# AssemblyAI-Community/MinImagen

Hardware: AMD Instinct MI355X
Metric: denoising-steps/sec (images/sec x T), base 64^2 + SR 64->256 cascade (higher is better)
Workload: dtype f32; 1 GPU; cascade64_256: unet_0 params @64x64 + unet_1 params (lowres_cond) @256x256, T=100/stage, cond_scale=3.0 (2 U-Net evals/step), dynamic thresholding 0.9, fp32 storage / accumulate / softmax / statistics, contractions as 3-term fp16-split (hi*hi + hi*lo + lo*hi) MFMA products; per_gpu_batch=32, global_batch=32, parallelism=dp1

## Files before the change

### include/minimagen_hip.h

```cpp
#ifndef MINIMAGEN_HIP_H
#define MINIMAGEN_HIP_H

#include <stdint.h>

#ifdef __cplusplus
extern "C" {
#endif

#define MI_ABI_VERSION 12

enum mi_status {
    MI_OK = 0,
    MI_ERR_INVALID = -1,
    MI_ERR_LAUNCH = -2,
    MI_ERR_UNSUPPORTED = -3
};

int mi_abi_version(void);
const char* mi_last_error(void);
const char* mi_backend(void);
int mi_struct_size(int which);

typedef struct mi_act {
    const float* data;
    int C;
    const double* stats;
    int nt;
    float scale;
    int bmod;
    int st;
} mi_act;

typedef struct mi_conv_params {
    int B, H, W;
    mi_act in0, in1;
    int Cout;
    int ksize, stride, up2;
    const float* w;
    const float* bias;
    int gn_groups;
    const float* gn_gamma;
    const float* gn_beta;
    float gn_eps;
    const float* scale_shift;
    int ss_stride, ss_off;
    mi_act res0, res1;
    const float* res_w;
    const float* res_b;
    float* out;
    int out_st;
    double* out_stats;
    int tile_cfg;
    const void* w_rp;
    const void* res_w_rp;
    int w_rp_exp, res_w_rp_exp;
    float* gn_coef;
    int* gn_exps;
    void* act_prep; long long act_prep_bytes;
} mi_conv_params;
#define MI_CONV_SPLIT16 0x100
#define MI_CONV_SPLIT8  0x800
#define MI_CONV_HALF    0x400
#define MI_CONV_REVERSE 0x200
#define MI_CONV_RP_FIRST 6

int mi_conv_tile_shape(int tile_cfg, int* th, int* tw);
int mi_conv_stripe_rows(const mi_conv_params* p);
int mi_conv_prep_fwd(const mi_conv_params* p, void* stream);
long long mi_conv_prep_bytes(int B, int Cin, int Cres, int H, int W);
int mi_conv_cout_tile(int Cout);
int mi_conv_fwd(const mi_conv_params* p, void* stream);
int mi_gn_coef_fwd(const mi_conv_params* p, void* stream);

typedef struct mi_crossembed_params {
    int B, H, W;
    const float* in0; int C0;
    const float* in1; int C1;
    int in1_batch_mod;
    int in0_batch_mod;
    int n_kernels;
    int ksize[3];
    int cout[3];
    const float* w[3];
    const float* bias[3];
    float* out; double* out_stats;
    int out_st;
    int tile_cfg;
    const float* addend;
    const void* w_mfma;
    int w_mfma_exp[3];
} mi_crossembed_params;
int mi_crossembed_fwd(const mi_crossembed_params* p, void* stream);

typedef struct mi_init_down_params {
    int B, H, W;
    const float* in0; int C0;
    const float* in1; int C1;
    int in0_batch_mod;
    int n_kernels;
    int ksize[3];
    int cout[3];
    int Cout;
    const void* w_tab;
    int w_exp;
    const float* bias9;
    float* out; double* out_stats;
    int out_st;
    int tile_cfg;
    const float* addend;
} mi_init_down_params;
int mi_init_down_tiles(int tile_cfg, int H, int W);
int mi_init_down_fwd(const mi_init_down_params* p, void* stream);

typedef struct mi_linear {
    const float* w; const float* b; int in, out;
} mi_linear;

typedef struct mi_text_cond_params {
    int B2, B, L, E, cd, tcd, max_len;
    const float* text_embeds;
    const uint8_t* text_mask;
    const uint8_t* keep;
    mi_linear text_to_cond;
    const float* null_text_embed;
    const float* ln_w; const float* ln_b;
    mi_linear h1, h2;
    const float* null_text_hidden;
    const float* norm_w; const float* norm_b;
    float* c_text;
    float* text_hiddens;
} mi_text_cond_params;
int mi_text_cond_fwd(const mi_text_cond_params* p, void* stream);

typedef struct mi_cond_step_params {
    int B2, B, dim, cd, tcd, ntok;
    const int64_t* time;
    const int64_t* lowres_time;
    const float* freq;
    mi_linear th, tc, tt;
    mi_linear lth, ltc, ltt;
    const float* text_hiddens;
    const float* norm_w; const float* norm_b;
    mi_linear time_mlps;
    float* ss;
    float* c_time;
    float* t_out;
    float* silu_out;
} mi_cond_step_params;
int mi_cond_step_fwd(const mi_cond_step_params* p, void* stream);

#define MI_ATTN_MAX_BLOCKS 8
typedef struct mi_attn_fold_params {
    int B2, C, cd, heads, JT;
    const float* c_rows;
    int c_stride_b;
    int row0, nrows;
    int write_null;
    int frag_f16;
    int n_blocks;
    struct {
        const float* mg;
        const float* mv;
        const float* g0;
        const float* v0;
        float* gv;
        float* table;
        int g_exp, v_exp;
    } blk[MI_ATTN_MAX_BLOCKS];
    int mode;
    const int* t_state;
    int t_off;
    const float* ss_all; float* ss; int ss_n;
} mi_attn_fold_params;
int mi_attn_fold_rows(const mi_attn_fold_params* p, void* stream);
int mi_attn_fragment_floats(int C);

typedef struct mi_cross_attn_params {
    int B2, C, HW, heads, J;
    mi_act x;
    const float* gv;
    const float* n1_g; const float* n1_b;
    const float* n2_g; const float* n2_b;
    float* out; double* out_stats;
    int out_st;
    int x_exp, g_exp, v_exp;
    int variant;
} mi_cross_attn_params;
int mi_cross_attn_fwd(const mi_cross_attn_params* p, void* stream);
#define MI_ATTN_TOKENS_PER_WG 128

typedef struct mi_cfg_x0_params {
    int B, n;
    const float* pred2;
    int two;
    float cond_scale;
    const float* x_t;
    const float* coef; const int* t_state;
    float* pred_out;
    float* x0;
    unsigned* hist0;
    int t_off;
} mi_cfg_x0_params;
int mi_cfg_x0_fwd(const mi_cfg_x0_params* p, void* stream);

#define MI_Q_BINS 2048
typedef struct mi_quantile_params {
    int B, n;
    const float* x0;
    int k_lo, k_hi; float w;
    unsigned* hist;
    float* s_out;
    float* v_out;
    int pass0_done;
    int self_cleaning;
} mi_quantile_params;
int mi_quantile_fwd(const mi_quantile_params* p, void* stream);

typedef struct mi_posterior_params {
    int B, n, T;
    const float* x0; const float* s_q;
    float* x;
    const float* coef; const int* t_state;
    const float* noise;
    uint64_t seed; int sample0; int stream_base;
    const uint64_t* seed_dev;
    int t_off;
} mi_posterior_params;
int mi_posterior_fwd(const mi_posterior_params* p, void* stream);

#define MI_SAMPLER_SMALL_N 16384
int mi_sampler_step_small_fwd(const mi_cfg_x0_params* c, const mi_quantile_params* q, const mi_posterior_params* pp, void* stream);

int mi_sampler_group_size(int n);
long long mi_sampler_group_sync_bytes(int B, int n);
int mi_sampler_step_group_fwd(const mi_cfg_x0_params* c, const mi_quantile_params* q, const mi_posterior_params* pp, void* sync, void* stream);

int mi_step_advance(int* t_state, int64_t* times, int B, void* stream);
int mi_step_advance_by(int* t_state, int64_t* times, int B, int n, void* stream);
int mi_step_set(int* t_state, int64_t* times, int B, int value, void* stream);

typedef struct mi_sampler_ext_params {
    const int* t_map;
    float* x0_prev;
    long long reserved[2];
} mi_sampler_ext_params;
int mi_posterior_ext_fwd(const mi_posterior_params* p, const mi_sampler_ext_params* e, void* stream);
int mi_sampler_step_small_ext_fwd(const mi_cfg_x0_params* c, const mi_quantile_params* q, const mi_posterior_params* pp, const mi_sampler_ext_params* e, void* stream);
int mi_sampler_step_group_ext_fwd(const mi_cfg_x0_params* c, const mi_quantile_params* q, const mi_posterior_params* pp, const mi_sampler_ext_params* e, void* sync,
                                  void* stream);
int mi_step_set_mapped(int* t_state, int64_t* times, int B, int value, const mi_sampler_ext_params* e, void* stream);
int mi_step_advance_mapped(int* t_state, int64_t* times, int B, const mi_sampler_ext_params* e, void* stream);
int mi_step_advance_by_mapped(int* t_state, int64_t* times, int B, int n, const mi_sampler_ext_params* e, void* stream);

typedef struct mi_inpaint_params {
    const float* known;
    const unsigned char* mask;
    int hw;
    int known_stream;
    const float* known_noise;
    long long reserved[2];
} mi_inpaint_params;
int mi_posterior_inpaint_fwd(const mi_posterior_params* p, const mi_sampler_ext_params* e, const mi_inpaint_params* ip, void* stream);
int mi_sampler_step_small_inpaint_fwd(const mi_cfg_x0_params* c, const mi_quantile_params* q, const mi_posterior_params* pp, const mi_sampler_ext_params* e,
                                      const mi_inpaint_params* ip, void* stream);
int mi_sampler_step_group_inpaint_fwd(const mi_cfg_x0_params* c, const mi_quantile_params* q, const mi_posterior_params* pp, const mi_sampler_ext_params* e,
                                      const mi_inpaint_params* ip, void* sync, void* stream);
int mi_inpaint_blend0_fwd(float* x, int B, int n, const mi_inpaint_params* ip, float a, float b, uint64_t seed, int sample0, void* stream);
int mi_inpaint_prepare_fwd(const float* img, float* known, int B, int n, int normalize, const unsigned char* mask_in, int Hin, int Win, unsigned char* mask_out,
                           int size, void* stream);

int mi_randn_fill(float* out, int B, int n, uint64_t seed, int sample0, int stream_id, void* stream);

int mi_finalize_images(const float* x, float* out, int64_t total, int unnormalize, void* stream);

typedef struct mi_resize_params {
    int planes, Hin, Win, Hout, Wout, KH, KW;
    const float* in; float* out;
    const int* idx_h; const float* w_h;
    const int* idx_w; const float* w_w;
} mi_resize_params;
int mi_resize_fwd(const mi_resize_params* p, void* stream);

int mi_lowres_augment(const float* img, const float* noise, float* out, int64_t total, float a, float b, int normalize, void* stream);

int mi_ln_tokens_fwd(const mi_act* x, int B, int HW, const float* gamma, const float* beta, float* out, void* stream);
typedef struct mi_self_attn_params {
    int B2, C, HW, heads, J;
    mi_act x;
    const float* gv;
    const float* n1_g; const float* n1_b;
    const float* n2_g; const float* n2_b;
    float* out; double* out_stats;
} mi_self_attn_params;
int mi_self_attn_fwd(const mi_self_attn_params* p, void* stream);
typedef struct mi_chan_ff_params {
    int B, C, Chid, HW;
    mi_act x;
    const float* g1; const float* w1;
    const float* g2; const float* w2;
    float* out; double* out_stats;
} mi_chan_ff_params;
int mi_chan_ff_fwd(const mi_chan_ff_params* p, void* stream);

typedef struct mi_flash_attn_params {
    int B, HW, heads, kv_heads;
    const float* q; float q_scale;
    const float* null_k; const float* null_v;
    const float* k0; const float* v0; int n0, ld0; long long bs0;
    const float* k1; const float* v1; int n1, ld1; long long bs1;
    float* out;
    void* kv_prep; long long kv_prep_bytes;
} mi_flash_attn_params;
int mi_flash_attn_fwd(const mi_flash_attn_params* p, void* stream);
long long mi_flash_kv_prep_bytes(int B, int J);
typedef struct mi_tokens_to_nchw_params {
    int B, HW, C;
    const float* tokens;
    const float* gamma; const float* beta; float eps;
    mi_act res;
    float* out; double* out_stats;
} mi_tokens_to_nchw_params;
int mi_tokens_to_nchw_fwd(const mi_tokens_to_nchw_params* p, void* stream);
int mi_ln_rows_fwd(const float* x, const float* gamma, const float* beta, float* y, int rows, int dim, float eps, void* stream);

int mi_gemm_f32(const float* A, const float* W, const float* gate, const float* R, float* Cout, int M, int N, int K, int act, void* stream);
int mi_gemm_rms_f32(const float* A, const float* W, const float* gate, const float* R, float* Cout, int M, int N, int K, int act,
                    const float* rowsq_in, int nparts, float eps, float* rowsq_out, void* stream);
int mi_rmsnorm(const float* x, const float* w, float* y, int rows, int dim, float eps, const uint8_t* zero_mask, void* stream);
int mi_embed_rows(const int64_t* ids, const float* table, float* out, int rows, int dim, void* stream);
int mi_embed_rows_sq(const int64_t* ids, const float* table, float* out, float* rowsq, int nparts, int rows, int dim, void* stream);
int mi_t5_attention(const float* qkv, const float* bias_tab, const uint8_t* key_mask, float* ctx, int B, int L, int heads, void* stream);

typedef struct mi_conv_wgrad_params {
    int B, Cin, Cout, H, W;
    const float* a;
    const float* dy;
    float* dw;
    float* db;
    float* partial; int nwg;
    const double* a_stats; int a_nt;
    const float* gamma; const float* beta; int groups; float eps;
    const float* ss; int ss_stride, ss_off;
} mi_conv_wgrad_params;
long long mi_conv_wgrad_workspace(int Cin, int Cout, int nwg);
int mi_conv_wgrad(const mi_conv_wgrad_params* p, void* stream);

typedef struct mi_block_bwd_params {
    int B, C, HW, groups, nt, nchunk;
    float eps;
    const float* x; const float* da;
    const double* x_stats;
    const float* gamma; const float* beta;
    const float* ss; int ss_stride, ss_off;
    float* uv;
    float* dx;
    float* dgamma; float* dbeta;
    float* dss;
    double* dx_stats;
} mi_block_bwd_params;
int mi_block_bwd(const mi_block_bwd_params* p, void* stream);
int mi_chan_stats_fwd(const float* x, double* stats, int rows, int HW, void* stream);
int mi_layernorm_fwd(const float* x, const float* gamma, const float* beta, float* y, float* stat, int rows, int dim, float eps, void* stream);
int mi_layernorm_bwd_nwg(int rows, int dim);
int mi_layernorm_bwd(const float* dy, const float* x, const float* gamma, const float* stat, float* dx, float* partial, float* dgamma, float* dbeta,
                     int rows, int dim, void* stream);
long long mi_pack_conv3_floats(int Cout, int Cin, int adjoint, int cout_pad, int which);
int mi_pack_conv3(const float* w, int Cout, int Cin, int adjoint, int exp, void* frag, float* generic, int cout_pad, void* stream);
typedef struct mi_pack_conv3_desc {
    const float* w; void* frag; float* generic;
    int Cout, Cin, adjoint, exp, cout_pad, reserved;
} mi_pack_conv3_desc;
int mi_pack_conv3_multi(const mi_pack_conv3_desc* descs, int n, int blocks, void* stream);

typedef struct mi_crossembed_wgrad_params {
    int B, Cin, H, W;
    const float* x;
    const float* dy;
    int n_kernels; int ksize[3]; int cout[3];
    float* dw[3];
    float* db[3];
    float* partial; int nwg;
} mi_crossembed_wgrad_params;
long long mi_crossembed_wgrad_workspace(int Cin, int kmax, int nwg);
int mi_crossembed_wgrad(const mi_crossembed_wgrad_params* p, void* stream);

typedef struct mi_folded_attn_params {
    int B, n, H, J, C, nchunk;
    const float* q;
    const float* kf; const float* vf;
    const uint8_t* mask;
    float* out;
    float* lse;
    const float* dout;
    float* dsum;
    float* dq;
    float* dkf; float* dvf;
    float* oh;
} mi_folded_attn_params;
int mi_folded_attn_fwd(const mi_folded_attn_params* p, void* stream);
int mi_folded_attn_bwd(const mi_folded_attn_params* p, void* stream);

typedef struct mi_flash_attn_train_params {
    int B, n, heads, kv_heads, J;
    const float* q; float q_scale;
    const float* k; const float* v;
    const uint8_t* mask;
    float* out;
    float* lse;
    const float* dout;
    float* dq;
    float* dk; float* dv;
    void* work; long long work_bytes;
} mi_flash_attn_train_params;
int mi_flash_attn_train_fwd(const mi_flash_attn_train_params* p, void* stream);
int mi_flash_attn_train_bwd(const mi_flash_attn_train_params* p, void* stream);
long long mi_flash_attn_train_workspace(int B, int n, int heads, int kv_heads, int J, int backward);

typedef struct { float* p; const float* g; float* m; float* v; long long n; } mi_adam_tensor;
typedef struct {
    const mi_adam_tensor* tensors;
    const int* chunk_tensor; const int* chunk_off;
    int nchunks, chunk;
    float lr, beta1, beta2, eps, weight_decay, bias_correction1, bias_correction2;
    float one_minus_beta1, one_minus_beta2;
    const float* grad_scale;
} mi_adam_params;
int mi_adam_step(const mi_adam_params* p, void* stream);

int mi_graph_begin(void* stream);
int mi_graph_end(void* stream, void** graph_exec);
int mi_graph_launch(void* graph_exec, void* stream);
int mi_graph_destroy(void* graph_exec);

#ifdef __cplusplus
}
#endif
#endif
```

### minimagen_amd/_lib.py

```python
from __future__ import annotations

import ctypes as C
import os

import torch

_HERE = os.path.dirname(os.path.abspath(__file__))
DEFAULT_LIB = os.environ.get("MINIMAGEN_HIP_LIB") or os.path.join(_HERE, "libminimagen_hip.so")

c_float_p = C.c_void_p


class MiAct(C.Structure):
    _fields_ = [("data", C.c_void_p), ("C", C.c_int), ("stats", C.c_void_p), ("nt", C.c_int), ("scale", C.c_float), ("bmod", C.c_int),
                ("st", C.c_int)]


class MiConvParams(C.Structure):
    _fields_ = [
        ("B", C.c_int), ("H", C.c_int), ("W", C.c_int),
        ("in0", MiAct), ("in1", MiAct),
        ("Cout", C.c_int), ("ksize", C.c_int), ("stride", C.c_int), ("up2", C.c_int),
        ("w", C.c_void_p), ("bias", C.c_void_p),
        ("gn_groups", C.c_int), ("gn_gamma", C.c_void_p), ("gn_beta", C.c_void_p), ("gn_eps", C.c_float),
        ("scale_shift", C.c_void_p), ("ss_stride", C.c_int), ("ss_off", C.c_int),
        ("res0", MiAct), ("res1", MiAct), ("res_w", C.c_void_p), ("res_b", C.c_void_p),
        ("out", C.c_void_p), ("out_st", C.c_int), ("out_stats", C.c_void_p), ("tile_cfg", C.c_int),
        ("w_rp", C.c_void_p), ("res_w_rp", C.c_void_p), ("w_rp_exp", C.c_int), ("res_w_rp_exp", C.c_int),
        ("gn_coef", C.c_void_p), ("gn_exps", C.c_void_p),
        ("act_prep", C.c_void_p), ("act_prep_bytes", C.c_longlong),
    ]


class MiCrossEmbedParams(C.Structure):
    _fields_ = [
        ("B", C.c_int), ("H", C.c_int), ("W", C.c_int),
        ("in0", C.c_void_p), ("C0", C.c_int), ("in1", C.c_void_p), ("C1", C.c_int),
        ("in1_batch_mod", C.c_int), ("in0_batch_mod", C.c_int), ("n_kernels", C.c_int),
        ("ksize", C.c_int * 3), ("cout", C.c_int * 3), ("w", C.c_void_p * 3), ("bias", C.c_void_p * 3),
        ("out", C.c_void_p), ("out_stats", C.c_void_p), ("out_st", C.c_int), ("tile_cfg", C.c_int), ("addend", C.c_void_p),
        ("w_mfma", C.c_void_p), ("w_mfma_exp", C.c_int * 3),
    ]


class MiInitDownParams(C.Structure):
    _fields_ = [
        ("B", C.c_int), ("H", C.c_int), ("W", C.c_int),
        ("in0", C.c_void_p), ("C0", C.c_int), ("in1", C.c_void_p), ("C1", C.c_int),
        ("in0_batch_mod", C.c_int), ("n_kernels", C.c_int), ("ksize", C.c_int * 3), ("cout", C.c_int * 3), ("Cout", C.c_int),
        ("w_tab", C.c_void_p), ("w_exp", C.c_int), ("bias9", C.c_void_p),
        ("out", C.c_void_p), ("out_stats", C.c_void_p), ("out_st", C.c_int), ("tile_cfg", C.c_int), ("addend", C.c_void_p),
    ]


class MiLinear(C.Structure):
    _fields_ = [("w", C.c_void_p), ("b", C.c_void_p), ("in_", C.c_int), ("out", C.c_int)]


class MiTextCondParams(C.Structure):
    _fields_ = [
        ("B2", C.c_int), ("B", C.c_int), ("L", C.c_int), ("E", C.c_int), ("cd", C.c_int), ("tcd", C.c_int), ("max_len", C.c_int),
        ("text_embeds", C.c_void_p), ("text_mask", C.c_void_p), ("keep", C.c_void_p),
        ("text_to_cond", MiLinear), ("null_text_embed", C.c_void_p), ("ln_w", C.c_void_p), ("ln_b", C.c_void_p),
        ("h1", MiLinear), ("h2", MiLinear), ("null_text_hidden", C.c_void_p), ("norm_w", C.c_void_p), ("norm_b", C.c_void_p),
        ("c_text", C.c_void_p), ("text_hiddens", C.c_void_p),
    ]


class MiCondStepParams(C.Structure):
    _fields_ = [
        ("B2", C.c_int), ("B", C.c_int), ("dim", C.c_int), ("cd", C.c_int), ("tcd", C.c_int), ("ntok", C.c_int),
        ("time", C.c_void_p), ("lowres_time", C.c_void_p), ("freq", C.c_void_p),
        ("th", MiLinear), ("tc", MiLinear), ("tt", MiLinear), ("lth", MiLinear), ("ltc", MiLinear), ("ltt", MiLinear),
        ("text_hiddens", C.c_void_p), ("norm_w", C.c_void_p), ("norm_b", C.c_void_p), ("time_mlps", MiLinear),
        ("ss", C.c_void_p), ("c_time", C.c_void_p), ("t_out", C.c_void_p), ("silu_out", C.c_void_p),
    ]


class MiAttnFoldBlk(C.Structure):
    _fields_ = [("mg", C.c_void_p), ("mv", C.c_void_p), ("g0", C.c_void_p), ("v0", C.c_void_p), ("gv", C.c_void_p), ("table", C.c_void_p),
                ("g_exp", C.c_int), ("v_exp", C.c_int)]


class MiAttnFoldParams(C.Structure):
    _fields_ = [
        ("B2", C.c_int), ("C", C.c_int), ("cd", C.c_int), ("heads", C.c_int), ("JT", C.c_int),
        ("c_rows", C.c_void_p), ("c_stride_b", C.c_int), ("row0", C.c_int), ("nrows", C.c_int), ("write_null", C.c_int), ("frag_f16", C.c_int),
        ("n_blocks", C.c_int), ("blk", MiAttnFoldBlk * 8),
        ("mode", C.c_int), ("t_state", C.c_void_p), ("t_off", C.c_int), ("ss_all", C.c_void_p), ("ss", C.c_void_p), ("ss_n", C.c_int),
    ]


class MiCrossAttnParams(C.Structure):
    _fields_ = [
        ("B2", C.c_int), ("C", C.c_int), ("HW", C.c_int), ("heads", C.c_int), ("J", C.c_int),
        ("x", MiAct), ("gv", C.c_void_p), ("n1_g", C.c_void_p), ("n1_b", C.c_void_p), ("n2_g", C.c_void_p), ("n2_b", C.c_void_p),
        ("out", C.c_void_p), ("out_stats", C.c_void_p), ("out_st", C.c_int), ("x_exp", C.c_int), ("g_exp", C.c_int), ("v_exp", C.c_int), ("variant", C.c_int),
    ]


class MiSelfAttnParams(C.Structure):
    _fields_ = [("B2", C.c_int), ("C", C.c_int), ("HW", C.c_int), ("heads", C.c_int), ("J", C.c_int), ("x", MiAct), ("gv", C.c_void_p),
                ("n1_g", C.c_void_p), ("n1_b", C.c_void_p), ("n2_g", C.c_void_p), ("n2_b", C.c_void_p), ("out", C.c_void_p), ("out_stats", C.c_void_p)]


class MiChanFFParams(C.Structure):
    _fields_ = [("B", C.c_int), ("C", C.c_int), ("Chid", C.c_int), ("HW", C.c_int), ("x", MiAct), ("g1", C.c_void_p), ("w1", C.c_void_p),
                ("g2", C.c_void_p), ("w2", C.c_void_p), ("out", C.c_void_p), ("out_stats", C.c_void_p)]


class MiFlashAttnParams(C.Structure):
    _fields_ = [("B", C.c_int), ("HW", C.c_int), ("heads", C.c_int), ("kv_heads", C.c_int), ("q", C.c_void_p), ("q_scale", C.c_float),
                ("null_k", C.c_void_p), ("null_v", C.c_void_p),
                ("k0", C.c_void_p), ("v0", C.c_void_p), ("n0", C.c_int), ("ld0", C.c_int), ("bs0", C.c_longlong),
                ("k1", C.c_void_p), ("v1", C.c_void_p), ("n1", C.c_int), ("ld1", C.c_int), ("bs1", C.c_longlong), ("out", C.c_void_p),
                ("kv_prep", C.c_void_p), ("kv_prep_bytes", C.c_longlong)]


class MiTokensToNchwParams(C.Structure):
    _fields_ = [("B", C.c_int), ("HW", C.c_int), ("C", C.c_int), ("tokens", C.c_void_p), ("gamma", C.c_void_p), ("beta", C.c_void_p),
                ("eps", C.c_float), ("res", MiAct), ("out", C.c_void_p), ("out_stats", C.c_void_p)]


class MiCfgX0Params(C.Structure):
    _fields_ = [("B", C.c_int), ("n", C.c_int), ("pred2", C.c_void_p), ("two", C.c_int), ("cond_scale", C.c_float),
                ("x_t", C.c_void_p), ("coef", C.c_void_p), ("t_state", C.c_void_p), ("pred_out", C.c_void_p), ("x0", C.c_void_p),
                ("hist0", C.c_void_p), ("t_off", C.c_int)]


class MiQuantileParams(C.Structure):
    _fields_ = [("B", C.c_int), ("n", C.c_int), ("x0", C.c_void_p), ("k_lo", C.c_int), ("k_hi", C.c_int), ("w", C.c_float),
                ("hist", C.c_void_p), ("s_out", C.c_void_p), ("v_out", C.c_void_p), ("pass0_done", C.c_int), ("self_cleaning", C.c_int)]


class MiPosteriorParams(C.Structure):
    _fields_ = [("B", C.c_int), ("n", C.c_int), ("T", C.c_int), ("x0", C.c_void_p), ("s_q", C.c_void_p), ("x", C.c_void_p),
                ("coef", C.c_void_p), ("t_state", C.c_void_p), ("noise", C.c_void_p),
                ("seed", C.c_uint64), ("sample0", C.c_int), ("stream_base", C.c_int), ("seed_dev", C.c_void_p), ("t_off", C.c_int)]


class MiSamplerExtParams(C.Structure):
    _fields_ = [("t_map", C.c_void_p), ("x0_prev", C.c_void_p), ("reserved", C.c_longlong * 2)]


class MiInpaintParams(C.Structure):
    _fields_ = [("known", C.c_void_p), ("mask", C.c_void_p), ("hw", C.c_int), ("known_stream", C.c_int), ("known_noise", C.c_void_p),
                ("reserved", C.c_longlong * 2)]


class MiResizeParams(C.Structure):
    _fields_ = [("planes", C.c_int), ("Hin", C.c_int), ("Win", C.c_int), ("Hout", C.c_int), ("Wout", C.c_int), ("KH", C.c_int), ("KW", C.c_int),
                ("in_", C.c_void_p), ("out", C.c_void_p), ("idx_h", C.c_void_p), ("w_h", C.c_void_p), ("idx_w", C.c_void_p), ("w_w", C.c_void_p)]


class MiConvWgradParams(C.Structure):
    _fields_ = [("B", C.c_int), ("Cin", C.c_int), ("Cout", C.c_int), ("H", C.c_int), ("W", C.c_int), ("a", C.c_void_p), ("dy", C.c_void_p),
                ("dw", C.c_void_p), ("db", C.c_void_p), ("partial", C.c_void_p), ("nwg", C.c_int),
                ("a_stats", C.c_void_p), ("a_nt", C.c_int), ("gamma", C.c_void_p), ("beta", C.c_void_p), ("groups", C.c_int), ("eps", C.c_float),
                ("ss", C.c_void_p), ("ss_stride", C.c_int), ("ss_off", C.c_int)]


class MiBlockBwdParams(C.Structure):
    _fields_ = [("B", C.c_int), ("C", C.c_int), ("HW", C.c_int), ("groups", C.c_int), ("nt", C.c_int), ("nchunk", C.c_int), ("eps", C.c_float),
                ("x", C.c_void_p), ("da", C.c_void_p), ("x_stats", C.c_void_p), ("gamma", C.c_void_p), ("beta", C.c_void_p),
                ("ss", C.c_void_p), ("ss_stride", C.c_int), ("ss_off", C.c_int), ("uv", C.c_void_p), ("dx", C.c_void_p),
                ("dgamma", C.c_void_p), ("dbeta", C.c_void_p), ("dss", C.c_void_p), ("dx_stats", C.c_void_p)]


class MiCrossEmbedWgradParams(C.Structure):
    _fields_ = [("B", C.c_int), ("Cin", C.c_int), ("H", C.c_int), ("W", C.c_int), ("x", C.c_void_p), ("dy", C.c_void_p),
                ("n_kernels", C.c_int), ("ksize", C.c_int * 3), ("cout", C.c_int * 3), ("dw", C.c_void_p * 3), ("db", C.c_void_p * 3),
                ("partial", C.c_void_p), ("nwg", C.c_int)]


class MiFoldedAttnParams(C.Structure):
    _fields_ = [("B", C.c_int), ("n", C.c_int), ("H", C.c_int), ("J", C.c_int), ("C", C.c_int), ("nchunk", C.c_int), ("q", C.c_void_p),
                ("kf", C.c_void_p), ("vf", C.c_void_p), ("mask", C.c_void_p), ("out", C.c_void_p), ("lse", C.c_void_p), ("dout", C.c_void_p),
                ("dsum", C.c_void_p), ("dq", C.c_void_p), ("dkf", C.c_void_p), ("dvf", C.c_void_p), ("oh", C.c_void_p)]


class MiFlashAttnTrainParams(C.Structure):
    _fields_ = [("B", C.c_int), ("n", C.c_int), ("heads", C.c_int), ("kv_heads", C.c_int), ("J", C.c_int), ("q", C.c_void_p), ("q_scale", C.c_float),
                ("k", C.c_void_p), ("v", C.c_void_p), ("mask", C.c_void_p), ("out", C.c_void_p), ("lse", C.c_void_p), ("dout", C.c_void_p),
                ("dq", C.c_void_p), ("dk", C.c_void_p), ("dv", C.c_void_p), ("work", C.c_void_p), ("work_bytes", C.c_longlong)]


class MiAdamTensor(C.Structure):
    _fields_ = [("p", C.c_void_p), ("g", C.c_void_p), ("m", C.c_void_p), ("v", C.c_void_p), ("n", C.c_longlong)]


class MiAdamParams(C.Structure):
    _fields_ = [("tensors", C.c_void_p), ("chunk_tensor", C.c_void_p), ("chunk_off", C.c_void_p), ("nchunks", C.c_int), ("chunk", C.c_int),
                ("lr", C.c_float), ("beta1", C.c_float), ("beta2", C.c_float), ("eps", C.c_float), ("weight_decay", C.c_float),
                ("bias_correction1", C.c_float), ("bias_correction2", C.c_float), ("one_minus_beta1", C.c_float), ("one_minus_beta2", C.c_float),
                ("grad_scale", C.c_void_p)]


class MiPackConv3Desc(C.Structure):
    _fields_ = [("w", C.c_void_p), ("frag", C.c_void_p), ("generic", C.c_void_p), ("Cout", C.c_int), ("Cin", C.c_int), ("adjoint", C.c_int),
                ("exp", C.c_int), ("cout_pad", C.c_int), ("reserved", C.c_int)]


_STRUCTS = {0: MiAct, 1: MiConvParams, 2: MiCrossEmbedParams, 3: MiLinear, 4: MiTextCondParams, 5: MiCondStepParams,
            6: MiAttnFoldParams, 7: MiCrossAttnParams, 8: MiCfgX0Params, 9: MiQuantileParams, 10: MiPosteriorParams,
            11: MiResizeParams, 12: MiSelfAttnParams, 13: MiChanFFParams, 14: MiFlashAttnParams, 15: MiTokensToNchwParams, 16: MiConvWgradParams, 17: MiBlockBwdParams, 18: MiCrossEmbedWgradParams, 19: MiFoldedAttnParams, 20: MiAdamTensor, 21: MiAdamParams, 22: MiPackConv3Desc,
            23: MiFlashAttnTrainParams, 24: MiSamplerExtParams, 25: MiInpaintParams, 26: MiInitDownParams}

_lib = None
_backend = None


class MinImagenHipError(RuntimeError):
    pass


def _bind(lib):
    lib.mi_abi_version.restype = C.c_int
    lib.mi_last_error.restype = C.c_char_p
    lib.mi_backend.restype = C.c_char_p
    lib.mi_struct_size.argtypes = [C.c_int]
    vp, i32, i64, u64, f32 = C.c_void_p, C.c_int, C.c_int64, C.c_uint64, C.c_float
    for name in ("mi_conv_fwd", "mi_gn_coef_fwd", "mi_crossembed_fwd", "mi_text_cond_fwd", "mi_cond_step_fwd", "mi_attn_fold_rows", "mi_cross_attn_fwd",
                 "mi_cfg_x0_fwd", "mi_quantile_fwd", "mi_posterior_fwd", "mi_resize_fwd", "mi_self_attn_fwd", "mi_chan_ff_fwd",
                 "mi_flash_attn_fwd", "mi_conv_prep_fwd", "mi_tokens_to_nchw_fwd", "mi_conv_wgrad", "mi_block_bwd", "mi_crossembed_wgrad", "mi_folded_attn_fwd", "mi_folded_attn_bwd", "mi_adam_step",
                 "mi_flash_attn_train_fwd", "mi_flash_attn_train_bwd", "mi_init_down_fwd"):
        getattr(lib, name).argtypes = [vp, vp]
        getattr(lib, name).restype = i32
    lib.mi_conv_prep_bytes.argtypes = [i32, i32, i32, i32, i32]
    lib.mi_conv_prep_bytes.restype = C.c_longlong
    lib.mi_flash_kv_prep_bytes.argtypes = [i32, i32]
    lib.mi_flash_kv_prep_bytes.restype = C.c_longlong
    lib.mi_flash_attn_train_workspace.argtypes = [i32, i32, i32, i32, i32, i32]
    lib.mi_flash_attn_train_workspace.restype = C.c_longlong
    lib.mi_step_advance.argtypes = [vp, vp, i32, vp]
    lib.mi_step_advance_by.argtypes = [vp, vp, i32, i32, vp]
    lib.mi_sampler_step_small_fwd.argtypes = [vp, vp, vp, vp]
    lib.mi_sampler_step_small_fwd.restype = i32
    lib.mi_sampler_step_group_fwd.argtypes = [vp, vp, vp, vp, vp]
    lib.mi_sampler_step_group_fwd.restype = i32
    lib.mi_sampler_group_size.argtypes = [i32]
    lib.mi_sampler_group_sync_bytes.argtypes = [i32, i32]
    lib.mi_sampler_group_sync_bytes.restype = C.c_longlong
    lib.mi_step_set.argtypes = [vp, vp, i32, i32, vp]
    lib.mi_posterior_ext_fwd.argtypes = [vp, vp, vp]
    lib.mi_sampler_step_small_ext_fwd.argtypes = [vp, vp, vp, vp, vp]
    lib.mi_sampler_step_group_ext_fwd.argtypes = [vp, vp, vp, vp, vp, vp]
    lib.mi_step_set_mapped.argtypes = [vp, vp, i32, i32, vp, vp]
    lib.mi_step_advance_mapped.argtypes = [vp, vp, i32, vp, vp]
    lib.mi_step_advance_by_mapped.argtypes = [vp, vp, i32, i32, vp, vp]
    lib.mi_posterior_inpaint_fwd.argtypes = [vp, vp, vp, vp]
    lib.mi_sampler_step_small_inpaint_fwd.argtypes = [vp, vp, vp, vp, vp, vp]
    lib.mi_sampler_step_group_inpaint_fwd.argtypes = [vp, vp, vp, vp, vp, vp, vp]
    lib.mi_inpaint_blend0_fwd.argtypes = [vp, i32, i32, vp, f32, f32, u64, i32, vp]
    lib.mi_inpaint_prepare_fwd.argtypes = [vp, vp, i32, i32, i32, vp, i32, i32, vp, i32, vp]
    lib.mi_randn_fill.argtypes = [vp, i32, i32, u64, i32, i32, vp]
    lib.mi_finalize_images.argtypes = [vp, vp, i64, i32, vp]
    lib.mi_lowres_augment.argtypes = [vp, vp, vp, i64, f32, f32, i32, vp]
    lib.mi_gemm_f32.argtypes = [vp, vp, vp, vp, vp, i32, i32, i32, i32, vp]
    lib.mi_rmsnorm.argtypes = [vp, vp, vp, i32, i32, f32, vp, vp]
    lib.mi_embed_rows.argtypes = [vp, vp, vp, i32, i32, vp]
    lib.mi_embed_rows_sq.argtypes = [vp, vp, vp, vp, i32, i32, i32, vp]
    lib.mi_gemm_rms_f32.argtypes = [vp, vp, vp, vp, vp, i32, i32, i32, i32, vp, i32, f32, vp, vp]
    lib.mi_t5_attention.argtypes = [vp, vp, vp, vp, i32, i32, i32, vp]
    lib.mi_ln_tokens_fwd.argtypes = [vp, i32, i32, vp, vp, vp, vp]
    lib.mi_ln_rows_fwd.argtypes = [vp, vp, vp, vp, i32, i32, f32, vp]
    lib.mi_graph_begin.argtypes = [vp]
    lib.mi_graph_end.argtypes = [vp, C.POINTER(vp)]
    lib.mi_graph_launch.argtypes = [vp, vp]
    lib.mi_graph_destroy.argtypes = [vp]
    lib.mi_conv_tile_shape.argtypes = [i32, C.POINTER(i32), C.POINTER(i32)]
    lib.mi_conv_stripe_rows.argtypes = [vp]
    lib.mi_conv_stripe_rows.restype = i32
    lib.mi_conv_cout_tile.argtypes = [i32]
    lib.mi_init_down_tiles.argtypes = [i32, i32, i32]
    lib.mi_init_down_tiles.restype = i32
    lib.mi_conv_wgrad_workspace.argtypes = [i32, i32, i32]
    lib.mi_conv_wgrad_workspace.restype = C.c_longlong
    lib.mi_crossembed_wgrad_workspace.argtypes = [i32, i32, i32]
    lib.mi_crossembed_wgrad_workspace.restype = C.c_longlong
    lib.mi_chan_stats_fwd.argtypes = [vp, vp, i32, i32, vp]
    lib.mi_layernorm_fwd.argtypes = [vp, vp, vp, vp, vp, i32, i32, C.c_float, vp]
    lib.mi_layernorm_bwd_nwg.argtypes = [i32, i32]
    lib.mi_layernorm_bwd_nwg.restype = i32
    lib.mi_layernorm_bwd.argtypes = [vp, vp, vp, vp, vp, vp, vp, vp, i32, i32, vp]
    lib.mi_pack_conv3_floats.argtypes = [i32, i32, i32, i32, i32]
    lib.mi_pack_conv3_floats.restype = C.c_longlong
    lib.mi_pack_conv3.argtypes = [vp, i32, i32, i32, i32, vp, vp, i32, vp]
    lib.mi_pack_conv3_multi.argtypes = [vp, i32, i32, vp]
    lib.mi_attn_fragment_floats.argtypes = [i32]
    for which, st in _STRUCTS.items():
        n = lib.mi_struct_size(which)
        if n != C.sizeof(st):
            raise MinImagenHipError(f"ABI mismatch: struct {st.__name__} is {n} bytes in the library, {C.sizeof(st)} in the binding")
    return lib


def use_library(path: str):
    global _lib, _backend
    if not os.path.exists(path):
        raise MinImagenHipError(f"{path} not found -- build it first (python -c 'import __graft_entry__ as g; g.build()')")
    _lib = _bind(C.CDLL(path))
    _backend = _lib.mi_backend().decode()
    return _lib


def lib():
    global _lib
    if _lib is None:
        use_library(DEFAULT_LIB)
    return _lib


def backend() -> str:
    lib()
    return _backend


def require_device(*tensors):
    be = backend()
    for t in tensors:
        if t is None:
            continue
        if t.dtype not in (torch.float32, torch.int64, torch.int32, torch.uint8, torch.bool, torch.float64):
            raise MinImagenHipError(f"unsupported dtype {t.dtype}")
        if not t.is_contiguous():
            raise MinImagenHipError("tensor must be contiguous")
        if be == "hip-gfx950" and not t.is_cuda:
            raise MinImagenHipError("minimagen_amd has no CPU path: tensor is not on the GPU")
        if be == "hipemu" and t.is_cuda:
            raise MinImagenHipError("emulator build needs host tensors")


def ptr(t) -> int:
    return 0 if t is None else t.data_ptr()


_RAW_STREAM = getattr(torch._C, "_cuda_getCurrentRawStream", None)


def current_stream() -> int:
    if backend() == "hip-gfx950":
        if _RAW_STREAM is not None:
            return _RAW_STREAM(torch.cuda.current_device())
        return torch.cuda.current_stream().cuda_stream
    return 0


def check(rc: int, what: str = ""):
    if rc != 0:
        raise MinImagenHipError(f"{what} failed ({rc}): {lib().mi_last_error().decode()}")
```

### minimagen_amd/csrc/attention.hip

```cpp
#include "common.hip.h"

namespace {

typedef _Float16 f16x4 __attribute__((ext_vector_type(4)));
typedef _Float16 f16x8 __attribute__((ext_vector_type(8)));
#ifndef ATTN_QPF
#define ATTN_QPF 1
#endif
#ifndef ATTN_QK32
#define ATTN_QK32 2
#endif

__device__ __forceinline__ void split_f16(const float (&x)[4], f16x4& hi, f16x4& lo) { mi_split_f16(x, hi, lo); }

template <int C, int JT, int WPS, bool HALF, int NWV>
__global__ __launch_bounds__(64 * NWV, WPS) void cross_attn_f16x3_kernel(const mi_cross_attn_params p) {
    constexpr int KC = (C + 15) / 16, MT = (C + 15) / 16, FRH = 8 * KC + 8 * MT, TOK_WG = 16 * NWV;
    constexpr int JP = (JT + 1) / 2;
    __shared__ double red[NWV][2 * 16 * MT];
    constexpr int QC = KC + MT, JTS = (JT + 1) & ~1, ROWS = JTS * QC;
    __shared__ __attribute__((aligned(16))) uint4 frag[2][ROWS * 64];
    const int tid = threadIdx.x, wave = tid >> 6, lane = tid & 63, lq = lane & 15, lg = lane >> 4;
    const int tiles = (p.HW + TOK_WG - 1) / TOK_WG;
    int b, tile;
    if ((p.B2 & 7) == 0) {
        const int L = blockIdx.x, k = L >> 3;
        b = (L & 7) + 8 * (k / tiles);
        tile = k % tiles;
    } else {
        b = blockIdx.x / tiles;
        tile = blockIdx.x % tiles;
    }
    const int bx = mi_row_of(b, p.x.bmod);
    const int i = (tile * NWV + wave) * 16 + lq;
    const bool ok = i < p.HW;
    const float* xb = p.x.data + (size_t)bx * C * p.HW;
    const bool x16 = HALF && p.x.st != 0, o16 = HALF && p.out_st != 0;
    auto ldx = [&](int a) -> float {
        if (x16) return mi_bf16_to_f32(reinterpret_cast<const unsigned short*>(p.x.data)[((size_t)bx * C + a) * p.HW + i]);
        return xb[(size_t)a * p.HW + i];
    };

    f16x4 xhi[KC], xlo[KC];
    {
        float xf[KC][4];
        float s = 0.0f;
#pragma unroll
        for (int kc = 0; kc < KC; ++kc)
#pragma unroll
            for (int e = 0; e < 4; ++e) {
                const int a = 16 * kc + 4 * lg + e;
                xf[kc][e] = (ok && a < C) ? ldx(a) * p.x.scale : 0.0f;
                s += xf[kc][e];
            }
        s += __shfl_xor(s, 16); s += __shfl_xor(s, 32);
        const float mean = s / (float)C;
        float v = 0.0f;
#pragma unroll
        for (int kc = 0; kc < KC; ++kc)
#pragma unroll
            for (int e = 0; e < 4; ++e) { const float d = (16 * kc + 4 * lg + e < C) ? xf[kc][e] - mean : 0.0f; v = fmaf(d, d, v); }
        v += __shfl_xor(v, 16); v += __shfl_xor(v, 32);
        const float rstd = 1.0f / sqrtf(v / (float)C + 1e-5f);
#pragma unroll
        for (int kc = 0; kc < KC; ++kc) {
            float xn[4];
#pragma unroll
            for (int e = 0; e < 4; ++e) {
                const int a = 16 * kc + 4 * lg + e;
                xn[e] = (a < C) ? ldexpf((xf[kc][e] - mean) * rstd * p.n1_g[a] + p.n1_b[a], p.x_exp) : 0.0f;
            }
            split_f16(xn, xhi[kc], xlo[kc]);
        }
    }
    f32x4 oacc[MT];
#pragma unroll
    for (int mt = 0; mt < MT; ++mt) oacc[mt] = (f32x4){0.f, 0.f, 0.f, 0.f};
    const _Float16* gvb = reinterpret_cast<const _Float16*>(p.gv) + (size_t)b * p.heads * JTS * 64 * FRH;
    const int jlast = p.J - 1;
    auto issue_head = [&](int h, int buf) {
        const _Float16* gvh = gvb + (size_t)h * JTS * 64 * FRH;
        for (int r = wave; r < ROWS; r += NWV) {
            const int jt = r / QC, q = r % QC;
            const _Float16* src = gvh + ((size_t)(jt * 64 + lane) * QC + q) * 8;
#if defined(HIPEMU)
            frag[buf][r * 64 + lane] = *reinterpret_cast<const uint4*>(src);
#else
            __builtin_amdgcn_global_load_lds((const __attribute__((address_space(1))) void*)src,
                                             (__attribute__((address_space(3))) void*)&frag[buf][r * 64], 16, 0, 0);
#endif
        }
    };
    issue_head(0, 0);

    for (int h = 0; h < p.heads; ++h) {
        const int hb = h & 1;
#if !defined(HIPEMU)
        asm volatile("s_waitcnt vmcnt(0)" ::: "memory");
#endif
        __syncthreads();
        if (h + 1 < p.heads) issue_head(h + 1, hb ^ 1);
        f32x4 s[JT];
        uint4 gq[2];
        constexpr bool QPF = !HALF && KC == 1 && ATTN_QPF;
        if constexpr (QPF) gq[0] = frag[hb][lane];
#pragma unroll
        for (int jt = 0; jt < JT; ++jt) {
            f32x4 acc = (f32x4){0.f, 0.f, 0.f, 0.f};
            if constexpr (QPF) {
                if (jt + 1 < JT) gq[(jt + 1) & 1] = frag[hb][((jt + 1) * QC) * 64 + lane];
                __builtin_amdgcn_sched_barrier(0);
            }
#pragma unroll
            for (int kc = 0; kc < KC; ++kc) {
                union { uint4 u; f16x4 h2[2]; uint2 u2; } g;
                if constexpr (HALF) g.u2 = reinterpret_cast<const uint2*>(&frag[hb][0])[2 * ((jt * QC + kc) * 64 + lane)];
                else if constexpr (QPF) g.u = gq[jt & 1];
                else g.u = frag[hb][(jt * QC + kc) * 64 + lane];
                const f16x4 ghi = g.h2[0];
                if constexpr (!HALF) {
#if ATTN_QK32 == 2
                    const f16x4 z4 = {(_Float16)0, (_Float16)0, (_Float16)0, (_Float16)0};
                    const f16x8 xhh = __builtin_shufflevector(xhi[kc], xhi[kc], 0, 1, 2, 3, 4, 5, 6, 7);
                    const f16x8 xl0 = __builtin_shufflevector(xlo[kc], z4, 0, 1, 2, 3, 4, 5, 6, 7);
                    acc = __builtin_amdgcn_mfma_f32_16x16x32_f16(__builtin_bit_cast(f16x8, g.u), xl0, acc, 0, 0, 0);
                    acc = __builtin_amdgcn_mfma_f32_16x16x32_f16(__builtin_bit_cast(f16x8, g.u), xhh, acc, 0, 0, 0);
#elif ATTN_QK32
                    const f16x8 xhh = __builtin_shufflevector(xhi[kc], xhi[kc], 0, 1, 2, 3, 4, 5, 6, 7);
                    acc = __builtin_amdgcn_mfma_f32_16x16x16f16(ghi, xlo[kc], acc, 0, 0, 0);
                    acc = __builtin_amdgcn_mfma_f32_16x16x32_f16(__builtin_bit_cast(f16x8, g.u), xhh, acc, 0, 0, 0);
#else
                    acc = __builtin_amdgcn_mfma_f32_16x16x16f16(g.h2[1], xhi[kc], acc, 0, 0, 0);
                    acc = __builtin_amdgcn_mfma_f32_16x16x16f16(ghi, xlo[kc], acc, 0, 0, 0);
                    acc = __builtin_amdgcn_mfma_f32_16x16x16f16(ghi, xhi[kc], acc, 0, 0, 0);
#endif
                } else {
                    acc = __builtin_amdgcn_mfma_f32_16x16x16f16(ghi, xhi[kc], acc, 0, 0, 0);
                }
            }
            s[jt] = acc;
            if constexpr (HALF) { if ((jt & 3) == 3) __builtin_amdgcn_sched_barrier(0); }
        }
        float m = -INFINITY;
#pragma unroll
        for (int jt = 0; jt < JT; ++jt)
#pragma unroll
            for (int r = 0; r < 4; ++r) {
                if (jt == JT - 1 && (16 * jt + 4 * lg + r) > jlast) s[jt][r] = -INFINITY;
                m = fmaxf(m, s[jt][r]);
            }
        m = fmaxf(m, __shfl_xor(m, 16));
        m = fmaxf(m, __shfl_xor(m, 32));
        const float sc = ldexpf(1.0f, -(p.x_exp + p.g_exp)), msc = -m * sc;
        mi_f32x2 l2 = {0.0f, 0.0f};
        const mi_f32x2 sc2 = {sc, sc}, msc2 = {msc, msc};
        f32x4 oh[MT];
#pragma unroll
        for (int mt = 0; mt < MT; ++mt) oh[mt] = (f32x4){0.f, 0.f, 0.f, 0.f};
#pragma unroll
        for (int jp = 0; jp < JP; ++jp) {
            f16x4 ph[2], pl[2];
#pragma unroll
            for (int ts = 0; ts < 2; ++ts) {
                const int jt = 2 * jp + ts;
                float pe[4] = {0.f, 0.f, 0.f, 0.f};
                if (jt < JT) {
                    const f32x4 sv = s[jt < JT ? jt : 0];
                    const mi_f32x2 a01 = mi_pk_fma((mi_f32x2){sv[0], sv[1]}, sc2, msc2), a23 = mi_pk_fma((mi_f32x2){sv[2], sv[3]}, sc2, msc2);
                    pe[0] = __builtin_amdgcn_exp2f(a01[0]); pe[1] = __builtin_amdgcn_exp2f(a01[1]);
                    pe[2] = __builtin_amdgcn_exp2f(a23[0]); pe[3] = __builtin_amdgcn_exp2f(a23[1]);
                    l2 = mi_pk_add(l2, (mi_f32x2){pe[0], pe[1]});
                    l2 = mi_pk_add(l2, (mi_f32x2){pe[2], pe[3]});
                }
                if constexpr (HALF) {
#pragma unroll
                    for (int r = 0; r < 4; ++r) ph[ts][r] = (_Float16)pe[r];
                } else {
                    split_f16(pe, ph[ts], pl[ts]);
                }
            }
            const f16x8 phi = __builtin_shufflevector(ph[0], ph[1], 0, 1, 2, 3, 4, 5, 6, 7);
#pragma unroll
            for (int mt = 0; mt < MT; ++mt) {
                const f16x8 vhi = __builtin_bit_cast(f16x8, frag[hb][((2 * jp) * QC + KC + mt) * 64 + lane]);
                if constexpr (!HALF) {
                    const f16x8 plo = __builtin_shufflevector(pl[0], pl[1], 0, 1, 2, 3, 4, 5, 6, 7);
                    const f16x8 vlo = __builtin_bit_cast(f16x8, frag[hb][((2 * jp + 1) * QC + KC + mt) * 64 + lane]);
                    oh[mt] = __builtin_amdgcn_mfma_f32_16x16x32_f16(vlo, phi, oh[mt], 0, 0, 0);
                    oh[mt] = __builtin_amdgcn_mfma_f32_16x16x32_f16(vhi, plo, oh[mt], 0, 0, 0);
                }
                oh[mt] = __builtin_amdgcn_mfma_f32_16x16x32_f16(vhi, phi, oh[mt], 0, 0, 0);
            }
        }
        float l = l2[0] + l2[1];
        l += __shfl_xor(l, 16);
        l += __shfl_xor(l, 32);
        const float linv = ldexpf(1.0f / l, -p.v_exp);
#pragma unroll
        for (int mt = 0; mt < MT; ++mt)
#pragma unroll
            for (int r = 0; r < 4; ++r) oacc[mt][r] = fmaf(oh[mt][r], linv, oacc[mt][r]);
    }

    float yv[4 * MT];
#pragma unroll
    for (int e = 0; e < 4 * MT; ++e) yv[e] = 0.0f;
    {
        float s1 = 0.0f;
#pragma unroll
        for (int mt = 0; mt < MT; ++mt)
#pragma unroll
            for (int r = 0; r < 4; ++r) s1 += oacc[mt][r];
        s1 += __shfl_xor(s1, 16); s1 += __shfl_xor(s1, 32);
        const float mean = s1 / (float)C;
        float v = 0.0f;
#pragma unroll
        for (int mt = 0; mt < MT; ++mt)
#pragma unroll
            for (int r = 0; r < 4; ++r) { const int a = 16 * mt + 4 * lg + r; const float d = (a < C) ? oacc[mt][r] - mean : 0.0f; v = fmaf(d, d, v); }
        v += __shfl_xor(v, 16); v += __shfl_xor(v, 32);
        const float rstd = 1.0f / sqrtf(v / (float)C + 1e-5f);
#pragma unroll
        for (int mt = 0; mt < MT; ++mt)
#pragma unroll
            for (int r = 0; r < 4; ++r) {
                const int a = 16 * mt + 4 * lg + r;
                if (a < C && ok) {
                    const float y = (oacc[mt][r] - mean) * rstd * p.n2_g[a] + p.n2_b[a] + ldx(a) * p.x.scale;
                    if (o16) reinterpret_cast<unsigned short*>(p.out)[((size_t)b * C + a) * p.HW + i] = (unsigned short)(mi_f32_to_bf16x2(y, 0.0f) & 0xffffu);
                    else p.out[((size_t)b * C + a) * p.HW + i] = y;
                    yv[4 * mt + r] = y;
                }
            }
    }
    if (p.out_stats) {
#pragma unroll
        for (int mt = 0; mt < MT; ++mt)
#pragma unroll
            for (int r = 0; r < 4; ++r) {
                const int a = 16 * mt + 4 * lg + r;
                double S, Q;
                mi_stat_reduce16(yv[4 * mt + r], a < C && ok, lane, S, Q);
                if (lq == 0) { red[wave][2 * a] = S; red[wave][2 * a + 1] = Q; }
            }
        __syncthreads();
        const int nt64 = (p.HW + 63) / 64;
        for (int sub = 0; sub < NWV / 4; ++sub) {
            const int st = tile * (NWV / 4) + sub;
            if (tid < 2 * C && st < nt64)
                p.out_stats[((size_t)(b * C + (tid >> 1)) * nt64 + st) * 2 + (tid & 1)] =
                    red[4 * sub][tid] + red[4 * sub + 1][tid] + red[4 * sub + 2][tid] + red[4 * sub + 3][tid];
        }
    }
}

}

extern "C" int mi_cross_attn_fwd(const mi_cross_attn_params* pp, void* stream) {
    const mi_cross_attn_params& p = *pp;
    hipStream_t st = (hipStream_t)stream;
    const int JT = (p.J + 15) / 16;
    if (JT != 17 && JT != 1) { mi_set_error("mi_cross_attn_fwd: context of %d rows (%d tiles) not instantiated (MinImagen: 1 + time tokens [+ 256])", p.J, JT); return MI_ERR_UNSUPPORTED; }
    if (p.B2 <= 0 || p.HW <= 0) { mi_set_error("mi_cross_attn_fwd: empty problem"); return MI_ERR_INVALID; }
    if ((p.x.st || p.out_st) && p.variant != 7) { mi_set_error("mi_cross_attn_fwd: bf16 activation storage is variant 7 only"); return MI_ERR_UNSUPPORTED; }
    if (p.variant == 6 || p.variant == 7) {
        static const int force_nwv = getenv("MI_ATTN_WAVES") ? atoi(getenv("MI_ATTN_WAVES")) : 0;
        const int nwv = (force_nwv == 8 || force_nwv == 16) ? force_nwv : (p.HW <= 1024 ? 16 : 8);
        const dim3 g6(((p.HW + 16 * nwv - 1) / (16 * nwv)) * p.B2);
#define MI_ATTN16_LAUNCH(CC) \
        if (JT == 1) { \
            if (p.variant == 6) hipLaunchKernelGGL(HIP_KERNEL_NAME(cross_attn_f16x3_kernel<CC, 1, (CC <= 16 ? 4 : 2), false, 8>), dim3(((p.HW + 127) / 128) * p.B2), dim3(512), 0, st, p); \
            else hipLaunchKernelGGL(HIP_KERNEL_NAME(cross_attn_f16x3_kernel<CC, 1, (CC <= 16 ? 4 : 2), true, 8>), dim3(((p.HW + 127) / 128) * p.B2), dim3(512), 0, st, p); \
        } else \
        if (p.variant == 6 && nwv == 8) hipLaunchKernelGGL(HIP_KERNEL_NAME(cross_attn_f16x3_kernel<CC, 17, (CC <= 16 ? 4 : 2), false, 8>), g6, dim3(512), 0, st, p); \
        else if (p.variant == 6) hipLaunchKernelGGL(HIP_KERNEL_NAME(cross_attn_f16x3_kernel<CC, 17, (CC <= 16 ? 4 : 2), false, 16>), g6, dim3(1024), 0, st, p); \
        else if (nwv == 8) hipLaunchKernelGGL(HIP_KERNEL_NAME(cross_attn_f16x3_kernel<CC, 17, (CC <= 16 ? 4 : 2), true, 8>), g6, dim3(512), 0, st, p); \
        else hipLaunchKernelGGL(HIP_KERNEL_NAME(cross_attn_f16x3_kernel<CC, 17, (CC <= 16 ? 4 : 2), true, 16>), g6, dim3(1024), 0, st, p);
        switch (p.C) {
            case 8: MI_ATTN16_LAUNCH(8) break;
            case 16: MI_ATTN16_LAUNCH(16) break;
            case 32: MI_ATTN16_LAUNCH(32) break;
            default: mi_set_error("mi_cross_attn_fwd: folded path instantiated for C in {8,16,32}, got %d", p.C); return MI_ERR_UNSUPPORTED;
        }
#undef MI_ATTN16_LAUNCH
        return mi_check_launch("cross_attn_f16x3_kernel");
    }
    mi_set_error("mi_cross_attn_fwd: variant %d (6 = 3-term fp16 split, fp32-grade; 7 = single fp16 term: the reduced-precision configuration)", p.variant);
    return MI_ERR_UNSUPPORTED;
}

namespace {

__global__ __launch_bounds__(256) void ln_tokens_kernel(const mi_act x, int HW, const float* gamma, const float* beta, float* out) {
    __shared__ float part[4][64];
    __shared__ float sMean[64], sRstd[64];
    __shared__ float T[64 * 65];
    const int tid = threadIdx.x, tl = tid & 63, cq = tid >> 6;
    const int b = blockIdx.y, C = x.C;
    const int bx = mi_row_of(b, x.bmod);
    const int tok0 = blockIdx.x * 64, tok = tok0 + tl;
    const bool ok = tok < HW;
    const float* xb = x.data + (size_t)bx * C * HW + (ok ? tok : HW - 1);
    float s = 0.0f;
    for (int c = cq; c < C; c += 4) s += xb[(size_t)c * HW] * x.scale;
    part[cq][tl] = s;
    __syncthreads();
    if (cq == 0) sMean[tl] = ((part[0][tl] + part[1][tl]) + (part[2][tl] + part[3][tl])) / (float)C;
    __syncthreads();
    const float mean = sMean[tl];
    float v = 0.0f;
    for (int c = cq; c < C; c += 4) { const float d = xb[(size_t)c * HW] * x.scale - mean; v = fmaf(d, d, v); }
    part[cq][tl] = v;
    __syncthreads();
    if (cq == 0) sRstd[tl] = 1.0f / sqrtf(((part[0][tl] + part[1][tl]) + (part[2][tl] + part[3][tl])) / (float)C + 1e-5f);
    __syncthreads();
    const float rstd = sRstd[tl];
    const int orow = tid >> 2, oseg = (tid & 3) * 16;
    const int nblk = (C + 63) / 64, per = (nblk + (int)gridDim.z - 1) / (int)gridDim.z;
    const int c_lo = (int)blockIdx.z * per * 64, c_hi = c_lo + per * 64 < C ? c_lo + per * 64 : C;
    for (int c0 = c_lo; c0 < c_hi; c0 += 64) {
        for (int cc = cq; cc < 64; cc += 4) {
            const int c = c0 + cc;
            if (c < C) T[tl * 65 + cc] = (xb[(size_t)c * HW] * x.scale - mean) * rstd * gamma[c] + beta[c];
        }
        __syncthreads();
        if (tok0 + orow < HW) {
            float* o = out + ((size_t)b * HW + tok0 + orow) * C + c0 + oseg;
            if (c0 + oseg + 16 <= C && (C & 3) == 0) {
#pragma unroll
                for (int i = 0; i < 16; i += 4)
                    *reinterpret_cast<float4*>(o + i) = make_float4(T[orow * 65 + oseg + i], T[orow * 65 + oseg + i + 1], T[orow * 65 + oseg + i + 2], T[orow * 65 + oseg + i + 3]);
            } else {
                for (int i = 0; i < 16; ++i) if (c0 + oseg + i < C) o[i] = T[orow * 65 + oseg + i];
            }
        }
        __syncthreads();
    }
}

template <int C, int JTC>
__global__ __launch_bounds__(256) void self_attn_folded_kernel(const mi_self_attn_params p, const int JT) {
    constexpr int KK = C / 4, NGP = KK < 4 ? 4 : KK, MT = (C + 15) / 16, FR = NGP + 4 * MT;
    __shared__ double red[4][2 * 16 * MT];
    const int tid = threadIdx.x, wave = tid >> 6, lane = tid & 63, lq = lane & 15, lg = lane >> 4;
    const int tiles = (p.HW + 63) / 64;
    const int b = blockIdx.x / tiles, tile = blockIdx.x % tiles;
    const int bx = mi_row_of(b, p.x.bmod);
    const int i = (tile * 4 + wave) * 16 + lq;
    const bool ok = i < p.HW;
    const float* xb = p.x.data + (size_t)bx * C * p.HW;
    float xh[KK];
    {
        float s = 0.0f;
#pragma unroll
        for (int kk = 0; kk < KK; ++kk) { xh[kk] = ok ? xb[(size_t)(4 * kk + lg) * p.HW + i] * p.x.scale : 0.0f; s += xh[kk]; }
        s += __shfl_xor(s, 16); s += __shfl_xor(s, 32);
        const float mean = s / (float)C;
        float v = 0.0f;
#pragma unroll
        for (int kk = 0; kk < KK; ++kk) { const float d = xh[kk] - mean; v = fmaf(d, d, v); }
        v += __shfl_xor(v, 16); v += __shfl_xor(v, 32);
        const float rstd = 1.0f / sqrtf(v / (float)C + 1e-5f);
#pragma unroll
        for (int kk = 0; kk < KK; ++kk) { const int a = 4 * kk + lg; xh[kk] = (xh[kk] - mean) * rstd * p.n1_g[a] + p.n1_b[a]; }
    }
    f32x4 oacc[MT];
#pragma unroll
    for (int mt = 0; mt < MT; ++mt) oacc[mt] = (f32x4){0.f, 0.f, 0.f, 0.f};
    const float* gvb = p.gv + (size_t)b * p.heads * JT * 64 * FR + (size_t)lane * FR;
    const int jlast = p.J - 1;
    for (int h = 0; h < p.heads; ++h) {
        const float* gvh = gvb + (size_t)h * JT * 64 * FR;
        f32x4 oh[MT];
#pragma unroll
        for (int mt = 0; mt < MT; ++mt) oh[mt] = (f32x4){0.f, 0.f, 0.f, 0.f};
        float m = -INFINITY, l = 0.0f;
        for (int jt0 = 0; jt0 < JT; jt0 += JTC) {
            f32x4 s[JTC];
#pragma unroll
            for (int t = 0; t < JTC; ++t) {
                f32x4 acc = (f32x4){0.f, 0.f, 0.f, 0.f};
                if (jt0 + t < JT) {
                    float g[NGP];
#pragma unroll
                    for (int v4 = 0; v4 < NGP / 4; ++v4) {
                        const float4 q4 = *reinterpret_cast<const float4*>(gvh + (size_t)(jt0 + t) * 64 * FR + 4 * v4);
                        g[4 * v4] = q4.x; g[4 * v4 + 1] = q4.y; g[4 * v4 + 2] = q4.z; g[4 * v4 + 3] = q4.w;
                    }
#pragma unroll
                    for (int kk = 0; kk < KK; ++kk) acc = __builtin_amdgcn_mfma_f32_16x16x4f32(g[kk], xh[kk], acc, 0, 0, 0);
                }
                s[t] = acc;
            }
            float cm = -INFINITY;
#pragma unroll
            for (int t = 0; t < JTC; ++t)
#pragma unroll
                for (int r = 0; r < 4; ++r) {
                    if (16 * (jt0 + t) + 4 * lg + r > jlast) s[t][r] = -INFINITY;
                    cm = fmaxf(cm, s[t][r]);
                }
            cm = fmaxf(cm, __shfl_xor(cm, 16));
            cm = fmaxf(cm, __shfl_xor(cm, 32));
            const float mn = fmaxf(m, cm);
            const float alpha = __builtin_amdgcn_exp2f(m - mn);
            float cl = 0.0f;
#pragma unroll
            for (int t = 0; t < JTC; ++t)
#pragma unroll
                for (int r = 0; r < 4; ++r) { const float e = __builtin_amdgcn_exp2f(s[t][r] - mn); s[t][r] = e; cl += e; }
            cl += __shfl_xor(cl, 16);
            cl += __shfl_xor(cl, 32);
            l = l * alpha + cl;
            m = mn;
#pragma unroll
            for (int mt = 0; mt < MT; ++mt)
#pragma unroll
                for (int r = 0; r < 4; ++r) oh[mt][r] *= alpha;
#pragma unroll
            for (int t = 0; t < JTC; ++t) {
                if (jt0 + t < JT) {
                    float vw[4 * MT];
#pragma unroll
                    for (int mt = 0; mt < MT; ++mt) {
                        const float4 q4 = *reinterpret_cast<const float4*>(gvh + (size_t)(jt0 + t) * 64 * FR + NGP + 4 * mt);
                        vw[4 * mt] = q4.x; vw[4 * mt + 1] = q4.y; vw[4 * mt + 2] = q4.z; vw[4 * mt + 3] = q4.w;
                    }
#pragma unroll
                    for (int mt = 0; mt < MT; ++mt)
#pragma unroll
                        for (int r = 0; r < 4; ++r) oh[mt] = __builtin_amdgcn_mfma_f32_16x16x4f32(vw[4 * mt + r], s[t][r], oh[mt], 0, 0, 0);
                }
            }
        }
        const float linv = 1.0f / l;
#pragma unroll
        for (int mt = 0; mt < MT; ++mt)
#pragma unroll
            for (int r = 0; r < 4; ++r) oacc[mt][r] = fmaf(oh[mt][r], linv, oacc[mt][r]);
    }
    float yv[4 * MT];
#pragma unroll
    for (int e = 0; e < 4 * MT; ++e) yv[e] = 0.0f;
    {
        float s1 = 0.0f;
#pragma unroll
        for (int mt = 0; mt < MT; ++mt)
#pragma unroll
            for (int r = 0; r < 4; ++r) s1 += oacc[mt][r];
        s1 += __shfl_xor(s1, 16); s1 += __shfl_xor(s1, 32);
        const float mean = s1 / (float)C;
        float v = 0.0f;
#pragma unroll
        for (int mt = 0; mt < MT; ++mt)
#pragma unroll
            for (int r = 0; r < 4; ++r) { const int a = 16 * mt + 4 * lg + r; const float d = (a < C) ? oacc[mt][r] - mean : 0.0f; v = fmaf(d, d, v); }
        v += __shfl_xor(v, 16); v += __shfl_xor(v, 32);
        const float rstd = 1.0f / sqrtf(v / (float)C + 1e-5f);
#pragma unroll
        for (int mt = 0; mt < MT; ++mt)
#pragma unroll
            for (int r = 0; r < 4; ++r) {
                const int a = 16 * mt + 4 * lg + r;
                if (a < C && ok) {
                    const float y = (oacc[mt][r] - mean) * rstd * p.n2_g[a] + p.n2_b[a] + xb[(size_t)a * p.HW + i] * p.x.scale;
                    p.out[((size_t)b * C + a) * p.HW + i] = y;
                    yv[4 * mt + r] = y;
                }
            }
    }
    if (p.out_stats) {
#pragma unroll
        for (int mt = 0; mt < MT; ++mt)
#pragma unroll
            for (int r = 0; r < 4; ++r) {
                const int a = 16 * mt + 4 * lg + r;
                double S, Q;
                mi_stat_reduce16(yv[4 * mt + r], a < C && ok, lane, S, Q);
                if (lq == 0) { red[wave][2 * a] = S; red[wave][2 * a + 1] = Q; }
            }
        __syncthreads();
        if (tid < 2 * C) p.out_stats[((size_t)(b * C + (tid >> 1)) * tiles + tile) * 2 + (tid & 1)] = red[0][tid] + red[1][tid] + red[2][tid] + red[3][tid];
    }
}

__device__ __forceinline__ float gelu_erf(float x) { return 0.5f * x * (1.0f + erff(x * 0.70710678118654752440f)); }

template <int C, int CH>
__global__ __launch_bounds__(256) void chan_ff_kernel(const mi_chan_ff_params p, const float* __restrict__ w1, const float* __restrict__ w2,
                                                      const float* __restrict__ g1, const float* __restrict__ g2) {
    __shared__ double red[2 * C][4];
    const int b = blockIdx.y, tid = threadIdx.x;
    const int bx = mi_row_of(b, p.x.bmod);
    const int i = blockIdx.x * 256 + tid;
    const bool ok = i < p.HW;
    const float* xb = p.x.data + (size_t)bx * C * p.HW + (ok ? i : 0);
    float x[C], hdn[CH];
    float s = 0.0f;
#pragma unroll
    for (int c = 0; c < C; ++c) { x[c] = xb[(size_t)c * p.HW] * p.x.scale; s += x[c]; }
    float mean = s / (float)C, v = 0.0f;
#pragma unroll
    for (int c = 0; c < C; ++c) { const float d = x[c] - mean; v = fmaf(d, d, v); }
    float rs = 1.0f / sqrtf(v / (float)C + 1e-5f);
    float xn[C];
#pragma unroll
    for (int c = 0; c < C; ++c) xn[c] = (x[c] - mean) * rs * g1[c];
    s = 0.0f;
#pragma unroll
    for (int o = 0; o < CH; ++o) {
        float a = 0.0f;
#pragma unroll
        for (int c = 0; c < C; ++c) a = fmaf(w1[o * C + c], xn[c], a);
        hdn[o] = gelu_erf(a);
        s += hdn[o];
    }
    mean = s / (float)CH; v = 0.0f;
#pragma unroll
    for (int o = 0; o < CH; ++o) { const float d = hdn[o] - mean; v = fmaf(d, d, v); }
    rs = 1.0f / sqrtf(v / (float)CH + 1e-5f);
#pragma unroll
    for (int o = 0; o < CH; ++o) hdn[o] = (hdn[o] - mean) * rs * g2[o];
#pragma unroll
    for (int c = 0; c < C; ++c) {
        float a = 0.0f;
#pragma unroll
        for (int o = 0; o < CH; ++o) a = fmaf(w2[c * CH + o], hdn[o], a);
        const float y = a + x[c];
        if (ok) p.out[((size_t)b * C + c) * p.HW + i] = y;
        if (p.out_stats) {
            double ys, yq;
            mi_stat_reduce64(ok ? y : 0.0f, ok, ys, yq);
            if ((tid & 63) == 0) { red[2 * c][tid >> 6] = ys; red[2 * c + 1][tid >> 6] = yq; }
        }
    }
    if (p.out_stats) {
        __syncthreads();
        if (tid < 2 * C) p.out_stats[((size_t)(b * C + (tid >> 1)) * gridDim.x + blockIdx.x) * 2 + (tid & 1)] = red[tid][0] + red[tid][1] + red[tid][2] + red[tid][3];
    }
}

}

extern "C" int mi_ln_tokens_fwd(const mi_act* x, int B, int HW, const float* gamma, const float* beta, float* out, void* stream) {
    if (B <= 0 || HW <= 0) { mi_set_error("mi_ln_tokens_fwd: empty"); return MI_ERR_INVALID; }
    const int nt = (HW + 63) / 64, nblk = (x->C + 63) / 64;
    int split = 1;
    while (split < nblk && (long long)nt * B * split < 512) split *= 2;
    hipLaunchKernelGGL(ln_tokens_kernel, dim3(nt, B, split), dim3(256), 0, (hipStream_t)stream, *x, HW, gamma, beta, out);
    return mi_check_launch("ln_tokens_kernel");
}

extern "C" int mi_self_attn_fwd(const mi_self_attn_params* pp, void* stream) {
    const mi_self_attn_params& p = *pp;
    hipStream_t st = (hipStream_t)stream;
    if (p.B2 <= 0 || p.HW <= 0 || p.J != p.HW + 1) { mi_set_error("mi_self_attn_fwd: bad sizes (J must be HW+1)"); return MI_ERR_INVALID; }
    const int JT = (p.J + 15) / 16;
    const dim3 grid(((p.HW + 63) / 64) * p.B2);
    switch (p.C) {
        case 8: hipLaunchKernelGGL(HIP_KERNEL_NAME(self_attn_folded_kernel<8, 16>), grid, dim3(256), 0, st, p, JT); break;
        case 16: hipLaunchKernelGGL(HIP_KERNEL_NAME(self_attn_folded_kernel<16, 16>), grid, dim3(256), 0, st, p, JT); break;
        case 32: hipLaunchKernelGGL(HIP_KERNEL_NAME(self_attn_folded_kernel<32, 16>), grid, dim3(256), 0, st, p, JT); break;
        default: mi_set_error("mi_self_attn_fwd: folded path instantiated for C in {8,16,32}, got %d", p.C); return MI_ERR_UNSUPPORTED;
    }
    return mi_check_launch("self_attn_folded_kernel");
}

extern "C" int mi_chan_ff_fwd(const mi_chan_ff_params* pp, void* stream) {
    const mi_chan_ff_params& p = *pp;
    hipStream_t st = (hipStream_t)stream;
    if (p.B <= 0 || p.HW <= 0 || p.Chid != 2 * p.C) { mi_set_error("mi_chan_ff_fwd: bad sizes (hidden must be 2*C)"); return MI_ERR_INVALID; }
    const dim3 grid((p.HW + 255) / 256, p.B);
    switch (p.C) {
        case 8: hipLaunchKernelGGL(HIP_KERNEL_NAME(chan_ff_kernel<8, 16>), grid, dim3(256), 0, st, p, p.w1, p.w2, p.g1, p.g2); break;
        case 16: hipLaunchKernelGGL(HIP_KERNEL_NAME(chan_ff_kernel<16, 32>), grid, dim3(256), 0, st, p, p.w1, p.w2, p.g1, p.g2); break;
        case 32: hipLaunchKernelGGL(HIP_KERNEL_NAME(chan_ff_kernel<32, 64>), grid, dim3(256), 0, st, p, p.w1, p.w2, p.g1, p.g2); break;
        default: mi_set_error("mi_chan_ff_fwd: instantiated for C in {8,16,32}, got %d", p.C); return MI_ERR_UNSUPPORTED;
    }
    return mi_check_launch("chan_ff_kernel");
}
```

### minimagen_amd/csrc/capi.hip

```cpp
#include "common.hip.h"
#include <cstdarg>
#include <cstdio>

static thread_local char g_err[512] = "";

void mi_set_error(const char* fmt, ...) {
    va_list ap;
    va_start(ap, fmt);
    vsnprintf(g_err, sizeof(g_err), fmt, ap);
    va_end(ap);
}

int mi_check_launch(const char* what) {
    hipError_t e = hipGetLastError();
    if (e != hipSuccess) {
        mi_set_error("%s: %s", what, hipGetErrorString(e));
        return MI_ERR_LAUNCH;
    }
    return MI_OK;
}

extern "C" int mi_abi_version(void) { return MI_ABI_VERSION; }
extern "C" const char* mi_last_error(void) { return g_err; }
extern "C" const char* mi_backend(void) { return MI_BACKEND_STRING; }
extern "C" int mi_struct_size(int which) {
    switch (which) {
        case 0: return (int)sizeof(mi_act);
        case 1: return (int)sizeof(mi_conv_params);
        case 2: return (int)sizeof(mi_crossembed_params);
        case 3: return (int)sizeof(mi_linear);
        case 4: return (int)sizeof(mi_text_cond_params);
        case 5: return (int)sizeof(mi_cond_step_params);
        case 6: return (int)sizeof(mi_attn_fold_params);
        case 7: return (int)sizeof(mi_cross_attn_params);
        case 8: return (int)sizeof(mi_cfg_x0_params);
        case 9: return (int)sizeof(mi_quantile_params);
        case 10: return (int)sizeof(mi_posterior_params);
        case 11: return (int)sizeof(mi_resize_params);
        case 12: return (int)sizeof(mi_self_attn_params);
        case 13: return (int)sizeof(mi_chan_ff_params);
        case 14: return (int)sizeof(mi_flash_attn_params);
        case 15: return (int)sizeof(mi_tokens_to_nchw_params);
        case 16: return (int)sizeof(mi_conv_wgrad_params);
        case 17: return (int)sizeof(mi_block_bwd_params);
        case 18: return (int)sizeof(mi_crossembed_wgrad_params);
        case 19: return (int)sizeof(mi_folded_attn_params);
        case 20: return (int)sizeof(mi_adam_tensor);
        case 21: return (int)sizeof(mi_adam_params);
        case 22: return (int)sizeof(mi_pack_conv3_desc);
        case 23: return (int)sizeof(mi_flash_attn_train_params);
        case 24: return (int)sizeof(mi_sampler_ext_params);
        case 25: return (int)sizeof(mi_inpaint_params);
        case 26: return (int)sizeof(mi_init_down_params);
    }
    return -1;
}
```

### minimagen_amd/csrc/cond.hip

```cpp
#include "common.hip.h"

#define MI_MAX_TCD 4096
#define MI_MAX_CD 1024

namespace {

__device__ __forceinline__ float dot_row(const float* __restrict__ w, const float* __restrict__ x, int n) {
    float a0 = 0.0f, a1 = 0.0f, a2 = 0.0f, a3 = 0.0f;
    int k = 0;
    if ((n & 3) == 0 && ((reinterpret_cast<size_t>(w) | reinterpret_cast<size_t>(x)) & 15) == 0) {
        for (; k + 4 <= n; k += 4) {
            const float4 wv = *reinterpret_cast<const float4*>(w + k), xv = *reinterpret_cast<const float4*>(x + k);
            a0 = fmaf(wv.x, xv.x, a0);
            a1 = fmaf(wv.y, xv.y, a1);
            a2 = fmaf(wv.z, xv.z, a2);
            a3 = fmaf(wv.w, xv.w, a3);
        }
    }
    for (; k < n; ++k) a0 = fmaf(w[k], x[k], a0);
    return (a0 + a1) + (a2 + a3);
}

__device__ __forceinline__ void ln_stats(const float* v, int n, float& mean, float& rstd) {
    float s = 0.0f;
    for (int k = 0; k < n; ++k) s += v[k];
    mean = s / (float)n;
    float q = 0.0f;
    for (int k = 0; k < n; ++k) { const float d = v[k] - mean; q = fmaf(d, d, q); }
    rstd = 1.0f / sqrtf(q / (float)n + 1e-5f);
}

__global__ __launch_bounds__(256) void text_cond_kernel(const mi_text_cond_params p) {
    __shared__ __attribute__((aligned(16))) float pooled[MI_MAX_CD];
    __shared__ __attribute__((aligned(16))) float hid[MI_MAX_TCD];
    const int tid = threadIdx.x, NT = 256;
    const int bb = blockIdx.x, b = bb % p.B;
    const bool keep = p.keep[bb] != 0;
    float* crow = p.c_text + (size_t)bb * p.max_len * p.cd;
    for (int j = tid; j < p.max_len; j += NT) {
        const bool in_caption = j < p.L;
        const bool valid = keep && (p.text_mask == nullptr || (in_caption && p.text_mask[(size_t)b * p.L + j] != 0));
        const float* e = p.text_embeds + ((size_t)b * p.L + (in_caption ? j : 0)) * p.E;
        for (int o = 0; o < p.cd; ++o) {
            float v;
            if (valid) v = in_caption ? dot_row(p.text_to_cond.w + (size_t)o * p.E, e, p.E) + (p.text_to_cond.b ? p.text_to_cond.b[o] : 0.0f) : 0.0f;
            else v = p.null_text_embed[(size_t)j * p.cd + o];
            crow[(size_t)j * p.cd + o] = v;
        }
    }
    __syncthreads();
    for (int o = tid; o < p.cd; o += NT) {
        float s = 0.0f;
        for (int j = 0; j < p.max_len; ++j) s += crow[(size_t)j * p.cd + o];
        pooled[o] = s / (float)p.max_len;
    }
    __syncthreads();
    float mean, rstd;
    ln_stats(pooled, p.cd, mean, rstd);
    __syncthreads();
    for (int o = tid; o < p.cd; o += NT) pooled[o] = (pooled[o] - mean) * rstd * p.ln_w[o] + p.ln_b[o];
    __syncthreads();
    for (int o = tid; o < p.tcd; o += NT) hid[o] = mi_silu(dot_row(p.h1.w + (size_t)o * p.cd, pooled, p.cd) + p.h1.b[o]);
    __syncthreads();
    for (int o = tid; o < p.tcd; o += NT) {
        const float v = dot_row(p.h2.w + (size_t)o * p.tcd, hid, p.tcd) + p.h2.b[o];
        p.text_hiddens[(size_t)bb * p.tcd + o] = keep ? v : p.null_text_hidden[o];
    }
    for (int j = tid; j < p.max_len; j += NT) {
        float* r = crow + (size_t)j * p.cd;
        float s = 0.0f;
        for (int k = 0; k < p.cd; ++k) s += r[k];
        const float m = s / (float)p.cd;
        float q = 0.0f;
        for (int k = 0; k < p.cd; ++k) { const float d = r[k] - m; q = fmaf(d, d, q); }
        const float rs = 1.0f / sqrtf(q / (float)p.cd + 1e-5f);
        for (int k = 0; k < p.cd; ++k) r[k] = (r[k] - m) * rs * p.norm_w[k] + p.norm_b[k];
    }
}

__device__ void time_trio(const mi_linear& th, const mi_linear& tc, const mi_linear& tt, const float* freq, long long tval, int dim,
                          float* emb, float* hid, float* t_acc, float* tok, bool accumulate, int tid, int NT) {
    const int half = dim / 2;
    for (int j = tid; j < half; j += NT) {
        const float arg = (float)tval * freq[j];
        emb[j] = sinf(arg);
        emb[half + j] = cosf(arg);
    }
    __syncthreads();
    for (int o = tid; o < th.out; o += NT) hid[o] = mi_silu(dot_row(th.w + (size_t)o * th.in, emb, th.in) + th.b[o]);
    __syncthreads();
    for (int o = tid; o < tc.out; o += NT) {
        const float v = dot_row(tc.w + (size_t)o * tc.in, hid, tc.in) + tc.b[o];
        t_acc[o] = accumulate ? t_acc[o] + v : v;
    }
    for (int o = tid; o < tt.out; o += NT) tok[o] = dot_row(tt.w + (size_t)o * tt.in, hid, tt.in) + tt.b[o];
    __syncthreads();
}

__global__ __launch_bounds__(256) void cond_step_kernel(const mi_cond_step_params p) {
    __shared__ __attribute__((aligned(16))) float emb[MI_MAX_CD];
    __shared__ __attribute__((aligned(16))) float hid[MI_MAX_TCD];
    __shared__ __attribute__((aligned(16))) float tvec[MI_MAX_TCD];
    __shared__ __attribute__((aligned(16))) float tok[4 * MI_MAX_CD];
    const int tid = threadIdx.x, NT = 256;
    const int bb = blockIdx.x, b = bb % p.B;
    const bool lowres = p.lth.w != nullptr;
    time_trio(p.th, p.tc, p.tt, p.freq, (long long)p.time[b], p.dim, emb, hid, tvec, tok, false, tid, NT);
    if (lowres)
        time_trio(p.lth, p.ltc, p.ltt, p.freq, (long long)p.lowres_time[b], p.dim, emb, hid, tvec, tok + p.ntok * p.cd, true, tid, NT);
    const int ntot = p.ntok * (lowres ? 2 : 1);
    for (int o = tid; o < p.tcd; o += NT) {
        float v = tvec[o];
        if (p.text_hiddens) v += p.text_hiddens[(size_t)bb * p.tcd + o];
        if (p.t_out) p.t_out[(size_t)bb * p.tcd + o] = v;
        hid[o] = mi_silu(v);
        if (p.silu_out) p.silu_out[(size_t)bb * p.tcd + o] = hid[o];
    }
    for (int r = tid; r < ntot; r += NT) {
        const float* row = tok + r * p.cd;
        float s = 0.0f;
        for (int k = 0; k < p.cd; ++k) s += row[k];
        const float m = s / (float)p.cd;
        float q = 0.0f;
        for (int k = 0; k < p.cd; ++k) { const float d = row[k] - m; q = fmaf(d, d, q); }
        const float rs = 1.0f / sqrtf(q / (float)p.cd + 1e-5f);
        if (p.c_time)
            for (int k = 0; k < p.cd; ++k)
                p.c_time[((size_t)bb * ntot + r) * p.cd + k] = (row[k] - m) * rs * p.norm_w[k] + p.norm_b[k];
    }
    __syncthreads();
    if (p.ss)
        for (int r = tid; r < p.time_mlps.out; r += NT)
            p.ss[(size_t)bb * p.time_mlps.out + r] = dot_row(p.time_mlps.w + (size_t)r * p.tcd, hid, p.tcd) + p.time_mlps.b[r];
}

__global__ __launch_bounds__(256) void attn_fold_rows_kernel(const mi_attn_fold_params p) {
    const int bb = blockIdx.x, blk = blockIdx.y;
    if (blk == p.n_blocks) {
        const float* src = p.ss_all + ((size_t)(*p.t_state - p.t_off) * gridDim.x + bb) * p.ss_n;
        for (int i = threadIdx.x; i < p.ss_n; i += 256) p.ss[(size_t)bb * p.ss_n + i] = src[i];
        return;
    }
    const int C = p.C, NGP = (C / 4) < 4 ? 4 : (C / 4), MT = (C + 15) / 16, FR = NGP + 4 * MT;
    const float* mg = p.blk[blk].mg;
    const float* mv = p.blk[blk].mv;
    float* gv = p.blk[blk].gv + (size_t)bb * p.heads * p.JT * 64 * FR;
    const int first = p.write_null ? -1 : 0;
    const int total = (p.nrows - first) * p.heads * C;
    const size_t trow = p.mode == 2 ? (size_t)(*p.t_state - p.t_off) * gridDim.x + bb : (p.mode == 3 ? (size_t)(*p.t_state - p.t_off) : (size_t)bb);
    for (int idx = threadIdx.x; idx < total; idx += 256) {
        const int a = idx % C, h = (idx / C) % p.heads, r = idx / (C * p.heads) + first;
        float g, v;
        int j;
        if (r < 0) {
            j = 0;
            g = p.blk[blk].g0[h * C + a];
            v = p.blk[blk].v0[h * C + a];
        } else {
            j = p.row0 + r;
            float* tab = p.mode ? p.blk[blk].table + (((trow * p.nrows + r) * p.heads + h) * C + a) * 2 : nullptr;
            if (p.mode >= 2) {
                g = tab[0];
                v = tab[1];
            } else {
                const float* c = p.c_rows + (size_t)bb * p.c_stride_b + (size_t)r * p.cd;
                g = dot_row(mg + ((size_t)h * C + a) * p.cd, c, p.cd);
                v = dot_row(mv + ((size_t)h * C + a) * p.cd, c, p.cd);
                if (p.mode == 1) { tab[0] = g; tab[1] = v; continue; }
            }
        }
        const int jt = j >> 4, jm = j & 15;
        if (p.frag_f16) {
            const int KC = (C + 15) / 16, MTh = (C + 15) / 16, FRH = 8 * KC + 8 * MTh;
            const int JTS = (p.JT + 1) & ~1;
            _Float16* th = reinterpret_cast<_Float16*>(p.blk[blk].gv) + (((size_t)bb * p.heads + h) * JTS + jt) * 64 * FRH;
            g = ldexpf(g, p.blk[blk].g_exp);
            v = ldexpf(v, p.blk[blk].v_exp);
            const _Float16 ghi = (_Float16)g, glo = (_Float16)(g - (float)ghi);
            const _Float16 vhi = (_Float16)v, vlo = (_Float16)(v - (float)vhi);
            _Float16* lg = th + (size_t)(jm + 16 * ((a & 15) >> 2)) * FRH + 8 * (a >> 4);
            lg[a & 3] = ghi;
            lg[4 + (a & 3)] = glo;
            _Float16* tv = th - (size_t)(jt & 1) * 64 * FRH;
            _Float16* lv = tv + (size_t)((a & 15) + 16 * (jm >> 2)) * FRH + 8 * KC + 8 * (a >> 4) + 4 * (jt & 1);
            lv[jm & 3] = vhi;
            lv[(size_t)64 * FRH + (jm & 3)] = vlo;
            continue;
        }
        float* tilep = gv + ((size_t)h * p.JT + jt) * 64 * FR;
        tilep[(size_t)(jm + 16 * (a & 3)) * FR + (a >> 2)] = g;
        tilep[(size_t)((a & 15) + 16 * (jm >> 2)) * FR + NGP + 4 * (a >> 4) + (jm & 3)] = v;
    }
}

}

extern "C" int mi_attn_fragment_floats(int C) { return ((C / 4) < 4 ? 4 : (C / 4)) + 4 * ((C + 15) / 16); }

extern "C" int mi_text_cond_fwd(const mi_text_cond_params* p, void* stream) {
    if (p->cd > MI_MAX_CD || p->tcd > MI_MAX_TCD || p->B2 <= 0 || p->B <= 0) { mi_set_error("mi_text_cond_fwd: cd/tcd too large or empty batch"); return MI_ERR_INVALID; }
    hipLaunchKernelGGL(text_cond_kernel, dim3(p->B2), dim3(256), 0, (hipStream_t)stream, *p);
    return mi_check_launch("text_cond_kernel");
}

extern "C" int mi_cond_step_fwd(const mi_cond_step_params* p, void* stream) {
    if (p->cd > MI_MAX_CD || p->tcd > MI_MAX_TCD || p->dim > MI_MAX_CD || p->B2 <= 0 || p->ntok * p->cd > 2 * MI_MAX_CD) { mi_set_error("mi_cond_step_fwd: dims too large"); return MI_ERR_INVALID; }
    if ((p->lth.w != nullptr) && p->lowres_time == nullptr) { mi_set_error("mi_cond_step_fwd: lowres U-Net needs lowres_time"); return MI_ERR_INVALID; }
    hipLaunchKernelGGL(cond_step_kernel, dim3(p->B2), dim3(256), 0, (hipStream_t)stream, *p);
    return mi_check_launch("cond_step_kernel");
}

extern "C" int mi_attn_fold_rows(const mi_attn_fold_params* p, void* stream) {
    const bool stage = p->mode == 2 || p->mode == 3;
    if (p->n_blocks < (stage ? 0 : 1) || p->n_blocks > MI_ATTN_MAX_BLOCKS || (p->n_blocks && (p->C % 4) != 0) || p->B2 <= 0) { mi_set_error("mi_attn_fold_rows: bad n_blocks / C"); return MI_ERR_INVALID; }
    if (p->n_blocks && p->mode != 1 && p->row0 + p->nrows > p->JT * 16) { mi_set_error("mi_attn_fold_rows: rows beyond the padded context"); return MI_ERR_INVALID; }
    if (p->mode < 0 || p->mode > 3 || (p->mode && p->write_null) || (stage && (!p->t_state || (p->ss_n > 0 && (!p->ss_all || !p->ss))))) { mi_set_error("mi_attn_fold_rows: bad mode / table arguments"); return MI_ERR_INVALID; }
    for (int k = 0; k < p->n_blocks; ++k) if (p->mode && !p->blk[k].table) { mi_set_error("mi_attn_fold_rows: mode %d needs blk[].table", p->mode); return MI_ERR_INVALID; }
    hipLaunchKernelGGL(attn_fold_rows_kernel, dim3(p->B2, p->n_blocks + ((stage && p->ss_n > 0) ? 1 : 0)), dim3(256), 0, (hipStream_t)stream, *p);
    return mi_check_launch("attn_fold_rows_kernel");
}
```

### minimagen_amd/engine.py

```python
from __future__ import annotations

import ctypes as C
import os
from types import SimpleNamespace
from typing import List, Optional

import torch
from torch import nn

from . import _lib as L
from . import packing as P
from .layers import Attention, CrossAttention, EinopsToAndFrom, Identity, Parallel, ResnetBlock, TransformerBlock

MAX_TEXT_LEN = 256
CONV_SPLIT8 = int(os.environ.get("MINIMAGEN_CONV_SPLIT8", "64"))
CONV_RP = int(os.environ.get("MINIMAGEN_CONV_RP", "2"))
CONV_WIDE_GEMM = os.environ.get("MINIMAGEN_CONV_WIDE_GEMM", "1") != "0"
COND_GEMM = int(os.environ.get("MINIMAGEN_COND_GEMM", "2048"))
FLASH_KV_PREP = os.environ.get("MINIMAGEN_FLASH_KV_PREP", "1") != "0"
CE_MFMA = os.environ.get("MINIMAGEN_CE_MFMA", "1") != "0"
INIT_DOWN = os.environ.get("MINIMAGEN_INIT_DOWN", "1") != "0"
CONV_REVERSE = int(os.environ.get("MINIMAGEN_CONV_REVERSE", "1"))
RP_NTILE = int(os.environ.get("MINIMAGEN_RP_NTILE", "0"))
RP_NTILE_BY = {k: int(os.environ.get("MINIMAGEN_RP_NTILE_" + k, "0")) for k in ("L", "M", "S")}
RP_NTILE_PIPE = {k: int(os.environ.get("MINIMAGEN_RP_NTILE_PIPE_" + k, d)) for k, d in (("L", "0"), ("M", "4"), ("S", "2"))}
CONV_STRIPE = os.environ.get("MINIMAGEN_CONV_STRIPE", "LMS").upper().replace("0", "").replace("1", "LMS")
ST_NBLK = {k: int(os.environ.get("MINIMAGEN_ST_NBLK_" + k, "0")) for k in ("L", "M", "S")}
ST_NBLK_PIPE = {k: int(os.environ.get("MINIMAGEN_ST_NBLK_PIPE_" + k, d)) for k, d in (("L", "0"), ("M", "0"), ("S", "4"))}
WEIGHT_FINGERPRINT = os.environ.get("MINIMAGEN_WEIGHT_FINGERPRINT", "1") != "0"
JT = 17


class Act:
    __slots__ = ("t", "stats", "nt", "C", "H", "W", "batch", "uses", "rev")

    def __init__(self, t, stats, nt, C_, H, W, batch):
        self.t, self.stats, self.nt, self.C, self.H, self.W, self.batch = t, stats, nt, C_, H, W, batch
        self.uses = 0
        self.rev = False

    @property
    def st(self) -> int:
        return 1 if self.t.dtype == torch.bfloat16 else 0

    def c(self, consumer_batch: int, scale: float = 1.0) -> L.MiAct:
        bmod = self.batch if self.batch != consumer_batch else 0
        self.uses += 1
        return L.MiAct(L.ptr(self.t), self.C, L.ptr(self.stats), self.nt, scale, bmod, self.st)


class _Store16Unsupported(Exception):
    """raised while a launch plan is built with bf16 activation storage and a layer needs a kernel that only reads fp32"""


def _lin(m: Optional[nn.Linear]) -> L.MiLinear:
    if m is None:
        return L.MiLinear(0, 0, 0, 0)
    return L.MiLinear(L.ptr(m.weight), L.ptr(m.bias) if m.bias is not None else 0, m.in_features, m.out_features)


class Workspace:

    def __init__(self):
        self.sampler_state = {}
        self.step_tables = {}
        self.prog_stage = None
        self.prog_stage_off = {}
        self.resize_tabs = {}


def _close_workspace(ws):
    for st in ws.sampler_state.values():
        st.close(ws.dev)


class UnetEngine:
    def __init__(self, unet):
        self.unet = unet
        self._pack = None
        self._pack_key = None
        self._pack_fp = None
        self._ws = {}
        self.precision = os.environ.get("MINIMAGEN_PRECISION", "fp32")

    def _param_key(self):
        ts = self._tensors()
        return (str(ts[0].device), tuple(t.data_ptr() for t in ts), sum(t._version for t in ts))

    def _tensors(self):
        ts = self.__dict__.get("_tensor_list")
        if ts is None:
            ts = self._tensor_list = list(self.unet.parameters()) + list(self.unet.buffers())
        return ts

    def _fingerprint(self):
        ts = [t.detach() for t in self._tensors() if t.is_floating_point()]
        return torch.stack(torch._foreach_norm(ts, 1) + torch._foreach_norm(ts, 2))

    def invalidate(self):
        for ws in self._ws.values():
            _close_workspace(ws)
        self._ws = {}
        self._pack = self._pack_key = self._pack_fp = None
        self.__dict__.pop("_tensor_list", None)

    def _check_params(self):
        for name, t in list(self.unet.named_parameters()) + list(self.unet.named_buffers()):
            if t.dtype != torch.float32:
                raise L.MinImagenHipError(f"parameter {name} is {t.dtype}; the HIP path computes in fp32 like the reference")
            if not t.is_contiguous():
                raise L.MinImagenHipError(f"parameter {name} is not contiguous")
        L.require_device(next(self.unet.parameters()))

    def pack(self):
        key = self._param_key()
        if not WEIGHT_FINGERPRINT:
            if self._pack is not None and key == self._pack_key:
                return self._pack
            fp = None
        else:
            fp = self._fingerprint()
            if self._pack is not None and key == self._pack_key and torch.equal(fp, self._pack_fp):
                return self._pack
        return self._repack(key, fp)

    def pack_identity(self):
        if self._pack is None or self._param_key() != self._pack_key:
            self.pack()

    def pack_begin(self):
        fresh = list(self.unet.parameters()) + list(self.unet.buffers())
        cached = self._tensors()
        if len(fresh) != len(cached) or any(a is not b for a, b in zip(fresh, cached)):
            self.__dict__.pop("_tensor_list", None)
            return (None, None, None)
        if not WEIGHT_FINGERPRINT or self._pack is None or self._pack_fp is None:
            return None
        fp = self._fingerprint()
        flag = self.__dict__.get("_fp_flag")
        if flag is None or flag.device != torch.device("cpu"):
            flag = self._fp_flag = torch.zeros(1, dtype=torch.int32).pin_memory() if fp.is_cuda else torch.zeros(1, dtype=torch.int32)
        flag.copy_((fp != self._pack_fp).any().to(torch.int32).reshape(1), non_blocking=True)
        ev = torch.cuda.current_stream(fp.device).record_event() if fp.is_cuda else None
        return (flag, ev, fp)

    def pack_changed(self, token) -> bool:
        if token is None:
            return False
        flag, ev, _ = token
        if flag is None:
            return True
        if ev is not None:
            ev.synchronize()
        return bool(flag.item())

    def _repack(self, key, fp):
        self.invalidate()
        self._pack_fp = fp
        self._check_params()
        u = self.unet
        dev = next(u.parameters()).device
        lib = L.lib()
        pk = SimpleNamespace()
        pk.keep = []
        pk.freq = P.sinusoid_freq(u.dim, dev)
        pk.conv = {}
        pk.conv_rp = {}
        pk.conv_ig = {}
        pk.attn = {}
        pk.attn_exp = {}

        def conv_pack(mod: nn.Conv2d, w=None, b=None):
            w = mod.weight if w is None else w
            ct = lib.mi_conv_cout_tile(w.shape[0])
            wp = P.pack_conv_weight(w.to(dev), ct)
            pk.keep.append(wp)
            if w.shape[-1] in (3, 4) and w.shape[1] % 8 == 0:
                pk.conv_rp[id(wp)] = P.pack_conv_weight_rp(w.to(dev))
            if CONV_WIDE_GEMM and w.shape[-1] == 3 and w.shape[1] % 32 == 0 and w.shape[0] % 64 == 0:
                pk.conv_ig[id(wp)] = P.pack_conv_weight_ig(w.to(dev))
            return wp

        resblocks: List[ResnetBlock] = [m for m in u.modules() if isinstance(m, ResnetBlock)]
        rows, biases, off = [], [], 0
        pk.ss_off = {}
        for rb in resblocks:
            if rb.time_mlp is not None:
                lin = rb.time_mlp[1]
                pk.ss_off[id(rb)] = off
                rows.append(lin.weight.detach())
                biases.append(lin.bias.detach())
                off += lin.out_features
        pk.R = off
        pk.tm_w = torch.cat(rows, 0).contiguous() if rows else torch.zeros(1, u.time_cond_dim, device=dev)
        pk.tm_b = torch.cat(biases, 0).contiguous() if rows else torch.zeros(1, device=dev)
        for rb in resblocks:
            pk.conv[id(rb.block1.project)] = conv_pack(rb.block1.project)
            pk.conv[id(rb.block2.project)] = conv_pack(rb.block2.project)
            if isinstance(rb.res_conv, nn.Conv2d):
                ct = lib.mi_conv_cout_tile(rb.res_conv.weight.shape[0])
                rw = P.pack_conv_weight(rb.res_conv.weight, ct).reshape(rb.res_conv.weight.shape[1], -1).contiguous()
                pk.keep.append(rw)
                if rb.res_conv.weight.shape[1] % 8 == 0:
                    pk.conv_rp[id(rw)] = P.pack_conv_weight_rp(rb.res_conv.weight)
                if CONV_WIDE_GEMM and rb.res_conv.weight.shape[1] % 32 == 0 and rb.res_conv.weight.shape[0] % 64 == 0:
                    pk.conv_ig[id(rw)] = P.pack_conv_weight_ig(rb.res_conv.weight)
                pk.conv[id(rb.res_conv)] = rw
            if rb.cross_attn is not None:
                ca: CrossAttention = rb.cross_attn.fn
                Cc = ca.to_q.in_features
                if ca.dim_head != 64:
                    raise NotImplementedError("cross-attention with dim_head != 64")
                if Cc not in (8, 16, 32):
                    if Cc % 16 or u.cond_dim % 16:
                        raise NotImplementedError(f"cross-attention over {Cc} channels / {u.cond_dim}-wide context: the wide path needs multiples of 16")
                    continue
                if not isinstance(ca.norm_context, Identity):
                    raise NotImplementedError("norm_context=True cross-attention is not on the MinImagen hot path")
                mg, mv, g0, v0 = P.fold_cross_attention(ca.to_q.weight, ca.to_kv.weight, ca.to_out[0].weight, ca.null_kv, ca.heads, ca.dim_head)
                pk.attn[id(ca)] = (mg, mv, g0, v0)
                pk.attn_exp[id(ca)] = P.attn_f16_exponents(mg, mv, g0, v0, cmax=P.layernorm_bound(u.norm_cond.weight, u.norm_cond.bias, u.cond_dim),
                                                           xmax=P.layernorm_bound(ca.norm.gamma, ca.norm.beta, Cc))
        for m in u.modules():
            if isinstance(m, Attention):
                Cc = m.to_q.in_features
                dh = m.to_kv.out_features // 2
                if dh != 64:
                    raise NotImplementedError("self-attention with dim_head != 64")
                if Cc not in (8, 16, 32):
                    if Cc % 16:
                        raise NotImplementedError(f"self-attention over {Cc} channels: the wide path needs a multiple of 16")
                    continue
                kv = m.to_kv.weight.detach()
                kv_full = torch.cat((kv[:dh].repeat(m.heads, 1), kv[dh:].repeat(m.heads, 1)), 0)
                pk.attn[id(m)] = P.fold_cross_attention(m.to_q.weight, kv_full, m.to_out[0].weight, m.null_kv, m.heads, dh)
        for level in u.downs:
            pre, _, _, _, post = level
            if isinstance(pre, nn.Conv2d):
                pk.conv[id(pre)] = conv_pack(pre)
            if isinstance(post, nn.Conv2d):
                pk.conv[id(post)] = conv_pack(post)
            elif isinstance(post, Parallel):
                w, b = P.fold_parallel_1x1(post.fns[0].weight, post.fns[0].bias, post.fns[1].weight, post.fns[1].bias)
                b = b.contiguous()
                pk.keep.append(b)
                pk.conv[id(post)] = (conv_pack(None, w=w), b)
        for level in u.ups:
            up = level[3]
            if isinstance(up, nn.Sequential):
                pk.conv[id(up[1])] = conv_pack(up[1])
        pk.conv[id(u.final_conv)] = conv_pack(u.final_conv)
        pk.ce_w = [c.weight.detach().permute(1, 2, 3, 0).contiguous() for c in u.init_conv.convs]
        pk.ce_mfma = {}
        cvs = u.init_conv.convs
        if CE_MFMA and [c.kernel_size[0] for c in cvs] == [3, 7, 15] and [c.out_channels for c in cvs] == [4, 2, 2] and u.channels <= 4:
            for chan0 in range(0, cvs[0].in_channels, u.channels):
                pk.ce_mfma[chan0] = P.pack_crossembed_mfma([c.weight for c in cvs], chan0, u.channels)
        pk.init_down = {}
        pre0 = u.downs[0][0]
        pk.init_down_ok = INIT_DOWN and CE_MFMA and isinstance(pre0, nn.Conv2d) and pre0.kernel_size == (4, 4) and pre0.stride == (2, 2) \
            and pre0.padding == (1, 1) and pre0.out_channels == 8 and len(cvs) <= 3 and all(c.kernel_size[0] % 2 == 1 and c.kernel_size[0] <= 15 for c in cvs) \
            and sum(c.out_channels for c in cvs) <= 16 and u.channels <= 4 and not u.init_conv_to_final_conv_residual
        self._pack, self._pack_key = pk, key
        return pk

    def _init_down_tables(self, pk):
        if not pk.init_down:
            u = self.unet
            cvs, pre0 = u.init_conv.convs, u.downs[0][0]
            dev = pre0.weight.device
            for chan0 in range(0, cvs[0].in_channels, u.channels):
                x_half = chan0 == 0
                w9, b9 = P.compose_init_down([c.weight for c in cvs], [c.bias for c in cvs] if x_half else None, pre0.weight, pre0.bias, chan0, u.channels)
                tab, exp, b32 = P.pack_init_down_mfma(w9, b9)
                pk.init_down[chan0] = (tab.to(dev), exp, b32.to(dev) if x_half else None)
        return pk.init_down

    def packed(self):
        return self._pack if self._pack is not None else self.pack()

    def workspace(self, B: int, B2: int, H: int, W: int, precision: Optional[str] = None, has_text: bool = True, lane: int = 0,
                  pipelined: bool = False) -> Workspace:
        pk = self.packed()
        dev = next(self.unet.parameters()).device
        precision = self.precision if precision is None else precision
        assert precision in ("fp32", "half"), precision
        key = (B, B2, H, W, str(dev), precision, has_text) + ((lane,) if lane else ()) + (("pipe",) if pipelined else ())
        ws = self._ws.get(key)
        if ws is not None:
            return ws
        u = self.unet
        ws = Workspace()
        ws.B, ws.B2, ws.H, ws.W, ws.dev = B, B2, H, W, dev
        ws.pipelined = pipelined
        ws.half = precision == "half"
        f = lambda *shape: torch.zeros(*shape, dtype=torch.float32, device=dev)
        ws.x = f(B, u.channels, H, W)
        ws.lowres = f(B, u.channels, H, W) if u.lowres_cond else None
        ws.times = torch.zeros(B, dtype=torch.int64, device=dev)
        ws.lowres_times = torch.zeros(B, dtype=torch.int64, device=dev) if u.lowres_cond else None
        ws.keep = torch.ones(B2, dtype=torch.uint8, device=dev)
        ws.c_text = f(B2, MAX_TEXT_LEN, u.cond_dim)
        ws.text_hiddens = f(B2, u.time_cond_dim)
        ws.ntot = u.num_time_tokens * (2 if u.lowres_cond else 1)
        ws.has_text = has_text
        ws.J = 1 + ws.ntot + (MAX_TEXT_LEN if has_text else 0)
        ws.JT = -(-ws.J // 16)
        ws.ss = f(B2, max(pk.R, 1))
        ws.c_time = f(B2, ws.ntot, u.cond_dim)
        ws.t_out = f(B2, u.time_cond_dim)
        ws.gv = {}
        ws.tensors = []
        ws.text_L = None
        for store16 in ((True, False) if ws.half else (False,)):
            ws.store16 = store16
            ws.gv, ws.tensors, ws.prog, ws.prog_text, ws.wide_attn = {}, [], [], [], False
            ws.ig_convs = []
            try:
                self._build_program(ws, pk)
                break
            except _Store16Unsupported:
                continue
        if ws.ig_convs:
            nbytes = max(n for _, n in ws.ig_convs)
            ws.ig_prep = torch.empty((nbytes + 3) // 4, dtype=torch.float32, device=dev)
            for p_, _ in ws.ig_convs:
                p_.act_prep, p_.act_prep_bytes = L.ptr(ws.ig_prep), nbytes
        self._ws[key] = ws
        return ws

    def _tile_cfg(self, H, W, batch=None, cz=1):
        lib = L.lib()
        best = 0 if (W >= 64 and H * W > 64 * 64) else 2
        th, tw = C.c_int(), C.c_int()
        lib.mi_conv_tile_shape(best, C.byref(th), C.byref(tw))
        return best, -(-H // th.value) * -(-W // tw.value)

    def _stripe_rows(self, batch, Ho, Wo, in0, in1, Cout, gn, res, up2=0, ksize=3, stride=1) -> int:
        q = L.MiConvParams()
        q.B, q.H, q.W, q.Cout, q.ksize, q.stride, q.up2 = batch, Ho, Wo, Cout, ksize, stride, int(bool(up2))
        q.in0 = L.MiAct(1, in0.C, 1 if in0.stats is not None else 0, in0.nt, 1.0, 0)
        if in1 is not None:
            q.in1 = L.MiAct(1, in1.C, 1 if in1.stats is not None else 0, in1.nt, 1.0, 0)
        q.w_rp = 1
        if gn is not None:
            q.gn_groups = gn.num_groups
        if res is not None:
            r0, r1, rw, _ = res
            q.res0 = L.MiAct(1, r0.C, 1 if r0.stats is not None else 0, r0.nt, 1.0, 0)
            if r1 is not None:
                q.res1 = L.MiAct(1, r1.C, 1 if r1.stats is not None else 0, r1.nt, 1.0, 0)
            if rw is not None:
                q.res_w, q.res_w_rp = 1, 1
        return int(L.lib().mi_conv_stripe_rows(C.byref(q)))

    def _new_act(self, ws, batch, Cc, H, W, nt, fp32: bool = False) -> Act:
        t = torch.empty(batch, Cc, H, W, dtype=torch.float32 if (fp32 or not ws.store16) else torch.bfloat16, device=ws.dev)
        st = torch.zeros(batch, Cc, max(nt, 1), 2, dtype=torch.float64, device=ws.dev) if nt else None
        ws.tensors += [t, st]
        return Act(t, st, nt, Cc, H, W, batch)

    def _emit_conv(self, ws, pk, in0: Act, in1: Optional[Act], *, wpack, bias, Cout, ksize=3, stride=1, up2=0,
                   gn: Optional[nn.GroupNorm] = None, ss_off: Optional[int] = None, res=None, conditioned=False,
                   want_stats=True, skip_scale=1.0, out_fp32=False) -> Act:
        lib = L.lib()
        Ho = in0.H * 2 if up2 else in0.H // stride
        Wo = in0.W * 2 if up2 else in0.W // stride
        if stride == 2 and ((in0.H | in0.W) & 1):
            raise NotImplementedError("stride-2 conv on an odd-sized image")
        ins = [a for a in (in0, in1) if a is not None] + ([r for r in res[:2] if r is not None] if res else [])
        batch = ws.B2 if (conditioned or any(a.batch == ws.B2 for a in ins)) else ws.B
        ct = lib.mi_conv_cout_tile(Cout)
        cfg, nt = self._tile_cfg(Ho, Wo, batch, -(-Cout // ct))
        cin_tot = in0.C + (in1.C if in1 is not None else 0)
        cres = 0 if (res is None or res[2] is None) else res[0].C + (res[1].C if res[1] is not None else 0)
        rp = bool(CONV_RP) and ((ksize == 3 and stride == 1) or (ksize == 4 and stride == 2 and not up2 and CONV_RP >= 2)) \
            and (not up2 or CONV_RP >= 2) and Wo % 4 == 0 and id(wpack) in pk.conv_rp \
            and in0.C % 8 == 0 and (in1 is None or in1.C % 8 == 0) \
            and (res is None or res[2] is None or (id(res[2]) in pk.conv_rp and res[0].C % 8 == 0 and (res[1] is None or res[1].C % 8 == 0)))
        narrow = cin_tot <= 64 and cres <= 64 and Cout <= (16 if stride == 2 else (8 if up2 else 32))
        wide = rp and not narrow
        stripe = False
        if rp:
            cfg = 6
            if Ho * Wo <= 64 * 64 and (Wo <= 32 or Cout <= 8):
                cfg = 7
            if Cout > 16:
                cfg = 7
            if up2:
                cfg = 6
            if stride == 2 or wide:
                cfg = 7
            if wide and stride == 1 and not up2 and Wo % 64 == 0 and Cout >= 32 and not ws.half:
                cfg = 6
            if wide and stride == 1 and not up2 and Wo <= 16 and Ho > 8 and Cout >= 32 and not ws.half:
                cfg = 10
            gemm = wide and ksize == 3 and stride == 1 and (not up2 or res is None) and not ws.half and cin_tot % 32 == 0 and cres % 32 == 0 and Cout % 64 == 0 \
                and id(wpack) in pk.conv_ig and (cres == 0 or id(res[2]) in pk.conv_ig)
            if gemm:
                cfg = 11
            th, tw = {6: (8, 64), 7: (8, 32), 10: (16, 16), 11: (8, 16)}[cfg]
            nt = -(-Ho // th) * -(-Wo // tw)
            cls = "L" if Ho * Wo > 128 * 128 else ("M" if Ho * Wo > 64 * 64 else "S")
            if narrow and ((ksize == 3 and stride == 1) or (ksize == 4 and stride == 2)) and not ws.half and cls in CONV_STRIPE:
                rows = self._stripe_rows(batch, Ho, Wo, in0, in1, Cout, gn, res, up2, ksize, stride)
                if rows:
                    cfg, nt, stripe = 12, Ho // rows, True
        if ws.store16 and (not rp or wide):
            raise _Store16Unsupported()
        out = self._new_act(ws, batch, Cout, Ho, Wo, nt if want_stats else 0, fp32=out_fp32)
        p = L.MiConvParams()
        p.B, p.H, p.W = batch, Ho, Wo
        p.in0 = in0.c(batch)
        if in1 is not None:
            p.in1 = in1.c(batch, skip_scale)
        p.Cout, p.ksize, p.stride, p.up2 = Cout, ksize, stride, up2
        p.w, p.bias = L.ptr(wpack), L.ptr(bias)
        if gn is not None:
            p.gn_groups, p.gn_gamma, p.gn_beta, p.gn_eps = gn.num_groups, L.ptr(gn.weight), L.ptr(gn.bias), gn.eps
            if ss_off is not None:
                p.scale_shift, p.ss_stride, p.ss_off = L.ptr(ws.ss), ws.ss.shape[1], ss_off
        if res is not None:
            r0, r1, rw, rb = res
            p.res0 = r0.c(batch)
            if r1 is not None:
                p.res1 = r1.c(batch, skip_scale)
            p.res_w, p.res_b = L.ptr(rw), L.ptr(rb)
        p.out_st = out.st
        p.out, p.out_stats, p.tile_cfg = L.ptr(out.t), L.ptr(out.stats), cfg | 0x100 | (0x400 if ws.half else 0) | (0x800 if (CONV_SPLIT8 and Ho * Wo <= CONV_SPLIT8 * CONV_SPLIT8) else 0)
        if wide:
            coef = torch.zeros(batch, cin_tot, 4, dtype=torch.float32, device=ws.dev)
            exps = torch.zeros(batch, 2, dtype=torch.int32, device=ws.dev)
            ws.tensors += [coef, exps]
            p.gn_coef, p.gn_exps = L.ptr(coef), L.ptr(exps)
        if rp:
            out.rev = bool(CONV_REVERSE) and batch % 8 == 0 and not in0.rev
            if out.rev:
                p.tile_cfg |= 0x200
            cls = "L" if Ho * Wo > 128 * 128 else ("M" if Ho * Wo > 64 * 64 else "S")
            nt_knob = RP_NTILE_BY[cls] or RP_NTILE
            if not nt_knob and ws.pipelined and RP_NTILE_PIPE[cls] and batch * nt // RP_NTILE_PIPE[cls] >= 256:
                nt_knob = RP_NTILE_PIPE[cls]
            if stripe:
                nt_knob = ST_NBLK[cls]
                if ws.pipelined and ST_NBLK_PIPE[cls] and nt % ST_NBLK_PIPE[cls] == 0 and batch * nt // ST_NBLK_PIPE[cls] >= 128 \
                        and self.unet.lowres_cond:
                    nt_knob = ST_NBLK_PIPE[cls]
                if nt_knob and (nt % nt_knob or nt_knob > 15):
                    nt_knob = 0
            p.tile_cfg |= (nt_knob & 0xf) << 12
            frags = pk.conv_ig if gemm else pk.conv_rp
            frag, p.w_rp_exp = frags[id(wpack)]
            p.w_rp = L.ptr(frag)
            if res is not None and res[2] is not None:
                rfrag, p.res_w_rp_exp = frags[id(res[2])]
                p.res_w_rp = L.ptr(rfrag)
        if wide:
            ws.prog.append((lib.mi_gn_coef_fwd, p, "gn_coef"))
            if gemm:
                ws.ig_convs.append((p, lib.mi_conv_prep_bytes(batch, cin_tot, cres, Ho, Wo)))
                ws.prog.append((lib.mi_conv_prep_fwd, p, "conv_prep"))
        ws.prog.append((lib.mi_conv_fwd, p, "conv"))
        return out

    def _emit_resnet(self, ws, pk, rb: ResnetBlock, in0: Act, in1: Optional[Act]) -> Act:
        u = self.unet
        s = u.skip_connect_scale
        Cout = rb.block1.project.out_channels
        has_cross = rb.cross_attn is not None
        h = self._emit_conv(ws, pk, in0, in1, wpack=pk.conv[id(rb.block1.project)], bias=rb.block1.project.bias, Cout=Cout,
                            gn=rb.block1.groupnorm, want_stats=not has_cross, skip_scale=s)
        if has_cross:
            h = self._emit_cross_attn(ws, pk, rb.cross_attn.fn, h)
        ss_off = pk.ss_off.get(id(rb))
        if isinstance(rb.res_conv, nn.Conv2d):
            res = (in0, in1, pk.conv[id(rb.res_conv)], rb.res_conv.bias)
        else:
            assert in1 is None
            res = (in0, None, None, None)
        return self._emit_conv(ws, pk, h, None, wpack=pk.conv[id(rb.block2.project)], bias=rb.block2.project.bias, Cout=Cout,
                               gn=rb.block2.groupnorm, ss_off=ss_off, res=res, conditioned=ss_off is not None, skip_scale=s)

    @staticmethod
    def _call(fn, name, *args):
        return (lambda _p, st, fn=fn, args=args: fn(*args, st)), None, name

    def _buf(self, ws, *shape):
        t = torch.empty(*shape, dtype=torch.float32, device=ws.dev)
        ws.tensors.append(t)
        return t

    def _emit_tokens_out(self, ws, tokens, batch, Cc, H, W, ln, res: Act, want_stats: bool) -> Act:
        if ws.store16:
            raise _Store16Unsupported()
        lib = L.lib()
        HW = H * W
        out = self._new_act(ws, batch, Cc, H, W, -(-HW // 64) if want_stats else 0)
        p = L.MiTokensToNchwParams()
        p.B, p.HW, p.C, p.tokens = batch, HW, Cc, L.ptr(tokens)
        if ln is not None:
            p.gamma, p.beta, p.eps = L.ptr(ln.gamma), L.ptr(ln.beta), 1e-5
        p.res = res.c(batch)
        p.out, p.out_stats = L.ptr(out.t), L.ptr(out.stats)
        ws.prog.append((lib.mi_tokens_to_nchw_fwd, p, "tokens_to_nchw"))
        return out

    def _emit_cross_attn_wide(self, ws, ca: CrossAttention, h: Act) -> Act:
        if ws.store16:
            raise _Store16Unsupported()
        lib, u = L.lib(), self.unet
        Cc, HW, B2, inner = h.C, h.H * h.W, ws.B2, ca.heads * 64
        xh, q, o, t = self._buf(ws, B2, HW, Cc), self._buf(ws, B2, HW, inner), self._buf(ws, B2, HW, inner), self._buf(ws, B2, HW, Cc)
        kv_time = self._buf(ws, B2, ws.ntot, 2 * inner)
        kv_text = self._buf(ws, B2, MAX_TEXT_LEN, 2 * inner) if ws.has_text else None
        xa = h.c(B2)
        ws.tensors.append(xa)
        ws.prog.append(self._call(lib.mi_ln_tokens_fwd, "ln_tokens", C.byref(xa), B2, HW, L.ptr(ca.norm.gamma), L.ptr(ca.norm.beta), L.ptr(xh)))
        ws.prog.append(self._call(lib.mi_gemm_f32, "gemm_q", L.ptr(xh), L.ptr(ca.to_q.weight), 0, 0, L.ptr(q), B2 * HW, inner, Cc, 0))
        ws.prog.append(self._call(lib.mi_gemm_f32, "gemm_kv_time", L.ptr(ws.c_time), L.ptr(ca.to_kv.weight), 0, 0, L.ptr(kv_time), B2 * ws.ntot, 2 * inner, u.cond_dim, 0))
        if ws.has_text:
            ws.prog_text.append(self._call(lib.mi_gemm_f32, "gemm_kv_text", L.ptr(ws.c_text), L.ptr(ca.to_kv.weight), 0, 0, L.ptr(kv_text), B2 * MAX_TEXT_LEN, 2 * inner, u.cond_dim, 0))
        p = L.MiFlashAttnParams()
        p.B, p.HW, p.heads, p.kv_heads, p.q, p.q_scale = B2, HW, ca.heads, ca.heads, L.ptr(q), 64 ** -0.5 * P.LOG2E
        p.null_k, p.null_v = L.ptr(ca.null_kv), L.ptr(ca.null_kv) + 4 * 64
        p.k0, p.v0, p.n0, p.ld0, p.bs0 = L.ptr(kv_time), L.ptr(kv_time) + 4 * inner, ws.ntot, 2 * inner, ws.ntot * 2 * inner
        if ws.has_text:
            p.k1, p.v1, p.n1, p.ld1, p.bs1 = L.ptr(kv_text), L.ptr(kv_text) + 4 * inner, MAX_TEXT_LEN, 2 * inner, MAX_TEXT_LEN * 2 * inner
        p.out = L.ptr(o)
        if FLASH_KV_PREP:
            nbytes = lib.mi_flash_kv_prep_bytes(B2 * ca.heads, 1 + ws.ntot + (MAX_TEXT_LEN if ws.has_text else 0))
            prep = self._buf(ws, (nbytes + 3) // 4)
            p.kv_prep, p.kv_prep_bytes = L.ptr(prep), nbytes
        ws.prog.append((lib.mi_flash_attn_fwd, p, "flash_attn"))
        ws.prog.append(self._call(lib.mi_gemm_f32, "gemm_out", L.ptr(o), L.ptr(ca.to_out[0].weight), 0, 0, L.ptr(t), B2 * HW, Cc, inner, 0))
        ws.wide_attn = True
        return self._emit_tokens_out(ws, t, B2, Cc, h.H, h.W, ca.to_out[1], h, True)

    def _emit_self_attn_wide(self, ws, at: Attention, x: Act, want_stats: bool) -> Act:
        if ws.store16:
            raise _Store16Unsupported()
        lib = L.lib()
        Cc, HW, batch, inner = x.C, x.H * x.W, x.batch, at.heads * 64
        xh, q, kv = self._buf(ws, batch, HW, Cc), self._buf(ws, batch, HW, inner), self._buf(ws, batch, HW, 128)
        o, t = self._buf(ws, batch, HW, inner), self._buf(ws, batch, HW, Cc)
        xa = x.c(batch)
        ws.tensors.append(xa)
        ws.prog.append(self._call(lib.mi_ln_tokens_fwd, "ln_tokens", C.byref(xa), batch, HW, L.ptr(at.norm.gamma), L.ptr(at.norm.beta), L.ptr(xh)))
        ws.prog.append(self._call(lib.mi_gemm_f32, "gemm_q", L.ptr(xh), L.ptr(at.to_q.weight), 0, 0, L.ptr(q), batch * HW, inner, Cc, 0))
        ws.prog.append(self._call(lib.mi_gemm_f32, "gemm_kv", L.ptr(xh), L.ptr(at.to_kv.weight), 0, 0, L.ptr(kv), batch * HW, 128, Cc, 0))
        p = L.MiFlashAttnParams()
        p.B, p.HW, p.heads, p.kv_heads, p.q, p.q_scale = batch, HW, at.heads, 1, L.ptr(q), 64 ** -0.5 * P.LOG2E
        p.null_k, p.null_v = L.ptr(at.null_kv), L.ptr(at.null_kv) + 4 * 64
        p.k0, p.v0, p.n0, p.ld0, p.bs0 = L.ptr(kv), L.ptr(kv) + 4 * 64, HW, 128, HW * 128
        p.out = L.ptr(o)
        if FLASH_KV_PREP and at.heads % 4 == 0:
            nbytes = lib.mi_flash_kv_prep_bytes(batch, HW + 1)
            prep = self._buf(ws, (nbytes + 3) // 4)
            p.kv_prep, p.kv_prep_bytes = L.ptr(prep), nbytes
        ws.prog.append((lib.mi_flash_attn_fwd, p, "flash_attn"))
        ws.prog.append(self._call(lib.mi_gemm_f32, "gemm_out", L.ptr(o), L.ptr(at.to_out[0].weight), 0, 0, L.ptr(t), batch * HW, Cc, inner, 0))
        return self._emit_tokens_out(ws, t, batch, Cc, x.H, x.W, at.to_out[1], x, want_stats)

    def _emit_chan_ff_wide(self, ws, tb: TransformerBlock, y: Act) -> Act:
        if ws.store16:
            raise _Store16Unsupported()
        lib = L.lib()
        Cc, HW, batch, Chid = y.C, y.H * y.W, y.batch, tb.ff[1].out_channels
        t0, h1, h2, t = self._buf(ws, batch, HW, Cc), self._buf(ws, batch, HW, Chid), self._buf(ws, batch, HW, Chid), self._buf(ws, batch, HW, Cc)
        zeros = torch.zeros(Cc, dtype=torch.float32, device=ws.dev)
        ya = y.c(batch)
        ws.tensors += [zeros, ya]
        ws.prog.append(self._call(lib.mi_ln_tokens_fwd, "ln_tokens", C.byref(ya), batch, HW, L.ptr(tb.ff[0].g), L.ptr(zeros), L.ptr(t0)))
        ws.prog.append(self._call(lib.mi_gemm_f32, "gemm_ff1", L.ptr(t0), L.ptr(tb.ff[1].weight), 0, 0, L.ptr(h1), batch * HW, Chid, Cc, 3))
        ws.prog.append(self._call(lib.mi_ln_rows_fwd, "ln_rows", L.ptr(h1), L.ptr(tb.ff[3].g), 0, L.ptr(h2), batch * HW, Chid, 1e-5))
        ws.prog.append(self._call(lib.mi_gemm_f32, "gemm_ff2", L.ptr(h2), L.ptr(tb.ff[4].weight), 0, 0, L.ptr(t), batch * HW, Cc, Chid, 0))
        return self._emit_tokens_out(ws, t, batch, Cc, y.H, y.W, None, y, True)

    def _emit_cross_attn(self, ws, pk, ca: CrossAttention, h: Act) -> Act:
        lib = L.lib()
        Cc, HW = h.C, h.H * h.W
        if Cc not in (8, 16, 32):
            return self._emit_cross_attn_wide(ws, ca, h)
        FR = lib.mi_attn_fragment_floats(Cc)
        jts = ws.JT + (ws.JT & 1)
        gv = torch.zeros(ws.B2, ca.heads, jts, 64, FR, dtype=torch.float32, device=ws.dev)
        ws.gv[id(ca)] = gv
        nt = -(-HW // 64)
        out = self._new_act(ws, ws.B2, Cc, h.H, h.W, nt)
        p = L.MiCrossAttnParams()
        p.B2, p.C, p.HW, p.heads, p.J = ws.B2, Cc, HW, ca.heads, ws.J
        p.x = h.c(ws.B2)
        p.gv = L.ptr(gv)
        p.n1_g, p.n1_b = L.ptr(ca.norm.gamma), L.ptr(ca.norm.beta)
        p.n2_g, p.n2_b = L.ptr(ca.to_out[1].gamma), L.ptr(ca.to_out[1].beta)
        p.out_st = out.st
        p.out, p.out_stats, p.variant = L.ptr(out.t), L.ptr(out.stats), (7 if ws.half else 6)
        p.x_exp, p.g_exp, p.v_exp = pk.attn_exp[id(ca)]
        ws.prog.append((lib.mi_cross_attn_fwd, p, "cross_attn"))
        return out

    def _emit_self_attn(self, ws, pk, at: Attention, x: Act, want_stats: bool) -> Act:
        if ws.store16:
            raise _Store16Unsupported()
        lib = L.lib()
        Cc, HW, batch = x.C, x.H * x.W, x.batch
        if Cc not in (8, 16, 32):
            return self._emit_self_attn_wide(ws, at, x, want_stats)
        xh = torch.empty(batch, HW, Cc, dtype=torch.float32, device=ws.dev)
        J = HW + 1
        jt = -(-J // 16)
        FR = lib.mi_attn_fragment_floats(Cc)
        gv = torch.zeros(batch, at.heads, jt, 64, FR, dtype=torch.float32, device=ws.dev)
        ws.tensors += [xh, gv]
        xa = x.c(batch)
        ws.tensors.append(xa)

        def ln_call(_p, st, xa=xa, xh=xh):
            return lib.mi_ln_tokens_fwd(C.byref(xa), batch, HW, L.ptr(at.norm.gamma), L.ptr(at.norm.beta), L.ptr(xh), st)
        ws.prog.append((lambda p_, st: ln_call(p_, st), None, "ln_tokens"))
        mg, mv, g0, v0 = pk.attn[id(at)]
        fp = L.MiAttnFoldParams()
        fp.B2, fp.C, fp.cd, fp.heads, fp.JT = batch, Cc, Cc, at.heads, jt
        fp.c_rows, fp.c_stride_b, fp.row0, fp.nrows, fp.write_null, fp.n_blocks = L.ptr(xh), HW * Cc, 1, HW, 1, 1
        fp.blk[0].mg, fp.blk[0].mv, fp.blk[0].g0, fp.blk[0].v0, fp.blk[0].gv = L.ptr(mg), L.ptr(mv), L.ptr(g0), L.ptr(v0), L.ptr(gv)
        ws.prog.append((lib.mi_attn_fold_rows, fp, "self_fold"))
        out = self._new_act(ws, batch, Cc, x.H, x.W, -(-HW // 64) if want_stats else 0)
        p = L.MiSelfAttnParams()
        p.B2, p.C, p.HW, p.heads, p.J = batch, Cc, HW, at.heads, J
        p.x, p.gv = xa, L.ptr(gv)
        p.n1_g, p.n1_b = L.ptr(at.norm.gamma), L.ptr(at.norm.beta)
        p.n2_g, p.n2_b = L.ptr(at.to_out[1].gamma), L.ptr(at.to_out[1].beta)
        p.out, p.out_stats = L.ptr(out.t), L.ptr(out.stats)
        ws.prog.append((lib.mi_self_attn_fwd, p, "self_attn"))
        return out

    def _emit_transformer_block(self, ws, pk, tb: TransformerBlock, x: Act) -> Act:
        if ws.store16:
            raise _Store16Unsupported()
        lib = L.lib()
        y = self._emit_self_attn(ws, pk, tb.attn.fn, x, want_stats=False)
        if y.C not in (8, 16, 32):
            return self._emit_chan_ff_wide(ws, tb, y)
        HW = y.H * y.W
        out = self._new_act(ws, y.batch, y.C, y.H, y.W, -(-HW // 256))
        p = L.MiChanFFParams()
        p.B, p.C, p.Chid, p.HW = y.batch, y.C, tb.ff[1].out_channels, HW
        p.x = y.c(y.batch)
        p.g1, p.w1, p.g2, p.w2 = L.ptr(tb.ff[0].g), L.ptr(tb.ff[1].weight), L.ptr(tb.ff[3].g), L.ptr(tb.ff[4].weight)
        p.out, p.out_stats = L.ptr(out.t), L.ptr(out.stats)
        ws.prog.append((lib.mi_chan_ff_fwd, p, "chan_ff"))
        return out

    def _fold_params(self, ws, pk, rows_t, stride_b, row0, nrows, write_null):
        lib = L.lib()
        calls = []
        cas = {id(m): m for m in self.unet.modules() if isinstance(m, CrossAttention)}
        by_c = {}
        for ca_id in ws.gv:
            if ca_id in cas:
                by_c.setdefault(cas[ca_id].to_q.in_features, []).append(ca_id)
        for _, ids in by_c.items():
            for i0 in range(0, len(ids), 8):
                chunk = ids[i0:i0 + 8]
                ca0 = cas[chunk[0]]
                p = L.MiAttnFoldParams()
                p.B2, p.C, p.cd, p.heads, p.JT = ws.B2, ca0.to_q.in_features, self.unet.cond_dim, ca0.heads, ws.JT
                p.c_rows, p.c_stride_b, p.row0, p.nrows, p.write_null = L.ptr(rows_t), stride_b, row0, nrows, write_null
                p.frag_f16 = 1
                p.n_blocks = len(chunk)
                for k, cid in enumerate(chunk):
                    mg, mv, g0, v0 = pk.attn[cid]
                    _, p.blk[k].g_exp, p.blk[k].v_exp = pk.attn_exp[cid]
                    p.blk[k].mg, p.blk[k].mv, p.blk[k].g0, p.blk[k].v0 = L.ptr(mg), L.ptr(mv), L.ptr(g0), L.ptr(v0)
                    p.blk[k].gv = L.ptr(ws.gv[cid])
                calls.append((lib.mi_attn_fold_rows, p, "fold"))
        return calls

    def _build_program(self, ws, pk):
        u = self.unet
        lib = L.lib()
        B, B2, H, W = ws.B, ws.B2, ws.H, ws.W
        cp = L.MiCondStepParams()
        cp.B2, cp.B, cp.dim, cp.cd, cp.tcd, cp.ntok = B2, B, u.dim, u.cond_dim, u.time_cond_dim, u.num_time_tokens
        cp.time, cp.lowres_time, cp.freq = L.ptr(ws.times), L.ptr(ws.lowres_times), L.ptr(pk.freq)
        cp.th, cp.tc, cp.tt = _lin(u.to_time_hiddens[1]), _lin(u.to_time_cond[0]), _lin(u.to_time_tokens[0])
        if u.lowres_cond:
            cp.lth, cp.ltc, cp.ltt = _lin(u.to_lowres_time_hiddens[1]), _lin(u.to_lowres_time_cond[0]), _lin(u.to_lowres_time_tokens[0])
        cp.text_hiddens = L.ptr(ws.text_hiddens) if ws.has_text else 0
        cp.norm_w, cp.norm_b = L.ptr(u.norm_cond.weight), L.ptr(u.norm_cond.bias)
        cp.time_mlps = L.MiLinear(L.ptr(pk.tm_w), L.ptr(pk.tm_b), u.time_cond_dim, pk.R)
        cp.ss, cp.c_time, cp.t_out = L.ptr(ws.ss), L.ptr(ws.c_time), L.ptr(ws.t_out)
        ws.cond_params = cp
        ws.prog_cond = [(lib.mi_cond_step_fwd, cp, "cond_step")]
        if COND_GEMM and pk.R >= COND_GEMM and u.time_cond_dim % 32 == 0:
            cg = L.MiCondStepParams.from_buffer_copy(cp)
            ws.silu_t = self._buf(ws, B2, u.time_cond_dim)
            ws.tm_bias = pk.tm_b.unsqueeze(0).expand(B2, -1).contiguous()
            ws.tensors.append(ws.tm_bias)
            cg.ss, cg.silu_out = 0, L.ptr(ws.silu_t)
            ws.prog_cond = [(lib.mi_cond_step_fwd, cg, "cond_step"),
                            self._call(lib.mi_gemm_f32, "gemm_time_mlps", L.ptr(ws.silu_t), L.ptr(pk.tm_w), 0, L.ptr(ws.tm_bias), L.ptr(ws.ss), B2, pk.R, u.time_cond_dim, 0)]

        cin = u.init_conv.convs[0].in_channels
        assert cin == u.channels * (2 if u.lowres_cond else 1)
        cfg, nt = self._tile_cfg(H, W, B)
        ce_mfma = bool(pk.ce_mfma) and W % 4 == 0
        if ws.store16 and not ce_mfma:
            raise _Store16Unsupported()
        if ce_mfma:
            cfg = 8 if H * W >= 128 * 128 else 9
            th, tw = C.c_int(), C.c_int()
            lib.mi_conv_tile_shape(cfg, C.byref(th), C.byref(tw))
            nt = -(-H // th.value) * -(-W // tw.value)
        ctot = sum(u.init_conv.dim_scales)
        if len(u.init_conv.convs) > 3:
            raise NotImplementedError("CrossEmbedLayer with more than 3 kernel sizes")
        init_down = pk.init_down_ok and not ws.half and not ws.store16 and H >= 4 and W >= 4 and H % 2 == 0 and W % 4 == 0

        def ce_params(src, chan0, with_bias, out_t, out_stats, addend):
            ce = L.MiCrossEmbedParams()
            ce.B, ce.H, ce.W = B, H, W
            ce.in0, ce.C0 = L.ptr(src), u.channels
            ce.n_kernels = len(u.init_conv.convs)
            for i, cv in enumerate(u.init_conv.convs):
                k, co = cv.kernel_size[0], cv.out_channels
                ce.ksize[i], ce.cout[i] = k, co
                ce.w[i] = L.ptr(pk.ce_w[i]) + 4 * chan0 * k * k * co
                ce.bias[i] = L.ptr(cv.bias) if with_bias else 0
            ce.out, ce.out_stats, ce.tile_cfg, ce.addend = L.ptr(out_t), L.ptr(out_stats), cfg, L.ptr(addend)
            ce.out_st = 1 if ws.store16 else 0
            if ce_mfma:
                tab, exps = pk.ce_mfma[chan0]
                ce.w_mfma, ce.tile_cfg = L.ptr(tab), cfg | (0x400 if ws.half else 0)
                for i in range(3):
                    ce.w_mfma_exp[i] = exps[i]
            return ce

        def id_params(src, chan0, out_t, out_stats, addend, id_cfg):
            q = L.MiInitDownParams()
            q.B, q.H, q.W = B, H, W
            q.in0, q.C0 = L.ptr(src), u.channels
            q.n_kernels = len(u.init_conv.convs)
            for i, cv in enumerate(u.init_conv.convs):
                q.ksize[i], q.cout[i] = cv.kernel_size[0], cv.out_channels
            tab, q.w_exp, b9 = pk.init_down[chan0]
            q.Cout, q.w_tab, q.bias9 = 8, L.ptr(tab), L.ptr(b9)
            q.out, q.out_stats, q.tile_cfg, q.addend = L.ptr(out_t), L.ptr(out_stats), id_cfg, L.ptr(addend)
            return q

        ws.prog_pre = []
        if init_down:
            self._init_down_tables(pk)
            id_cfg = 0 if W // 2 >= 64 else 1
            cur = self._new_act(ws, B, 8, H // 2, W // 2, lib.mi_init_down_tiles(id_cfg, H, W))
            fn = lib.mi_init_down_fwd
            if u.lowres_cond:
                ws.ce_lr = torch.zeros(B, 8, H // 2, W // 2, dtype=torch.float32, device=ws.dev)
                ws.prog_pre.append((fn, id_params(ws.lowres, u.channels, ws.ce_lr, None, None, id_cfg), "crossembed_lowres"))
            ws.prog.append((fn, id_params(ws.x, 0, cur.t, cur.stats, ws.ce_lr if u.lowres_cond else None, id_cfg), "crossembed"))
        else:
            cur = self._new_act(ws, B, ctot, H, W, nt)
            if u.lowres_cond:
                ws.ce_lr = torch.zeros(B, ctot, H, W, dtype=torch.bfloat16 if ws.store16 else torch.float32, device=ws.dev)
                ws.prog_pre.append((lib.mi_crossembed_fwd, ce_params(ws.lowres, u.channels, False, ws.ce_lr, None, None), "crossembed_lowres"))
                ws.prog.append((lib.mi_crossembed_fwd, ce_params(ws.x, 0, True, cur.t, cur.stats, ws.ce_lr), "crossembed"))
            else:
                ws.prog.append((lib.mi_crossembed_fwd, ce_params(ws.x, 0, True, cur.t, cur.stats, None), "crossembed"))

        hiddens: List[Act] = []
        for level, (pre, init_block, resnet_blocks, attn_block, post) in enumerate(u.downs):
            if isinstance(pre, nn.Conv2d) and not (init_down and level == 0):
                cur = self._emit_conv(ws, pk, cur, None, wpack=pk.conv[id(pre)], bias=pre.bias, Cout=pre.out_channels, ksize=4, stride=2)
            cur = self._emit_resnet(ws, pk, init_block, cur, None)
            for rb in resnet_blocks:
                cur = self._emit_resnet(ws, pk, rb, cur, None)
                hiddens.append(cur)
            if isinstance(attn_block, TransformerBlock):
                cur = self._emit_transformer_block(ws, pk, attn_block, cur)
            hiddens.append(cur)
            if isinstance(post, nn.Conv2d):
                cur = self._emit_conv(ws, pk, cur, None, wpack=pk.conv[id(post)], bias=post.bias, Cout=post.out_channels, ksize=4, stride=2)
            elif isinstance(post, Parallel):
                wp, bsum = pk.conv[id(post)]
                cur = self._emit_conv(ws, pk, cur, None, wpack=wp, bias=bsum, Cout=post.fns[0].out_channels)
        cur = self._emit_resnet(ws, pk, u.mid_block1, cur, None)
        if u.mid_attn is not None:
            cur = self._emit_self_attn(ws, pk, u.mid_attn.fn.fn, cur, want_stats=True)
        cur = self._emit_resnet(ws, pk, u.mid_block2, cur, None)
        for init_block, resnet_blocks, attn_block, upsample in u.ups:
            cur = self._emit_resnet(ws, pk, init_block, cur, hiddens.pop())
            for rb in resnet_blocks:
                cur = self._emit_resnet(ws, pk, rb, cur, hiddens.pop())
            if isinstance(attn_block, TransformerBlock):
                cur = self._emit_transformer_block(ws, pk, attn_block, cur)
            if isinstance(upsample, nn.Sequential):
                cv = upsample[1]
                cur = self._emit_conv(ws, pk, cur, None, wpack=pk.conv[id(cv)], bias=cv.bias, Cout=cv.out_channels, up2=1)
        cur = self._emit_resnet(ws, pk, u.final_res_block, cur, None)
        out = self._emit_conv(ws, pk, cur, None, wpack=pk.conv[id(u.final_conv)], bias=u.final_conv.bias, Cout=u.channels_out,
                              want_stats=False, conditioned=True, out_fp32=True)
        ws.pred = out.t
        if (out.H, out.W) != (H, W):
            raise L.MinImagenHipError(f"U-Net output is {out.H}x{out.W} for a {H}x{W} input (image size must be divisible by the down-sampling factor)")
        if ws.gv:
            ws.prog_cond += self._fold_params(ws, pk, ws.c_time, ws.ntot * u.cond_dim, 1, ws.ntot, 0)

    def set_text(self, ws, text_embeds: torch.Tensor, text_mask: Optional[torch.Tensor], keep: torch.Tensor):
        u, pk, lib = self.unet, self.packed(), L.lib()
        st = L.current_stream()
        if text_embeds is None:
            assert not ws.has_text, "workspace was built for a text-conditioned call"
            for fn, fp, name in self._fold_params(ws, pk, ws.c_time, ws.ntot * u.cond_dim, 1, 0, 1):
                L.check(fn(C.byref(fp), st), name)
            return
        assert ws.has_text, "workspace was built for a call without text"
        text_embeds = text_embeds.to(device=ws.dev, dtype=torch.float32).contiguous()
        assert text_embeds.shape[0] == ws.B and text_embeds.shape[-1] == u.text_embed_dim
        mask8 = None if text_mask is None else text_mask.to(device=ws.dev).to(torch.uint8).contiguous()
        k8 = keep.to(device='cpu', dtype=torch.uint8)
        if getattr(ws, "keep_host", None) is None or not torch.equal(ws.keep_host, k8):
            ws.keep.copy_(k8)
            ws.keep_host = k8.clone()
        ws.text_keepalive = (text_embeds, mask8)
        L.require_device(text_embeds, mask8)
        p = L.MiTextCondParams()
        p.B2, p.B, p.L, p.E, p.cd, p.tcd, p.max_len = ws.B2, ws.B, text_embeds.shape[1], u.text_embed_dim, u.cond_dim, u.time_cond_dim, MAX_TEXT_LEN
        p.text_embeds, p.text_mask, p.keep = L.ptr(text_embeds), L.ptr(mask8), L.ptr(ws.keep)
        p.text_to_cond = _lin(u.text_to_cond)
        p.null_text_embed = L.ptr(u.null_text_embed)
        ln = u.to_text_non_attn_cond[0]
        p.ln_w, p.ln_b = L.ptr(ln.weight), L.ptr(ln.bias)
        p.h1, p.h2 = _lin(u.to_text_non_attn_cond[1]), _lin(u.to_text_non_attn_cond[3])
        p.null_text_hidden = L.ptr(u.null_text_hidden)
        p.norm_w, p.norm_b = L.ptr(u.norm_cond.weight), L.ptr(u.norm_cond.bias)
        p.c_text, p.text_hiddens = L.ptr(ws.c_text), L.ptr(ws.text_hiddens)
        L.check(lib.mi_text_cond_fwd(C.byref(p), st), "mi_text_cond_fwd")
        for fn, fp, name in self._fold_params(ws, pk, ws.c_text, MAX_TEXT_LEN * u.cond_dim, 1 + ws.ntot, MAX_TEXT_LEN, 1):
            L.check(fn(C.byref(fp), st), name)
        for fn, fp, name in ws.prog_text:
            L.check(fn(None, st), name)

    def prepare_lowres(self, ws, stream=None):
        st = L.current_stream() if stream is None else stream
        for fn, p, name in ws.prog_pre:
            L.check(fn(C.byref(p), st), name)

    def prepare_step_tables(self, ws, T: int, t_state: torch.Tensor, stream=None, t_map=None):
        u, pk, lib = self.unet, self.packed(), L.lib()
        st = L.current_stream() if stream is None else stream
        B2, dev = ws.B2, ws.dev
        if ws.wide_attn:
            ws.prog_stage = ws.prog_cond
            return
        key = (T, t_state.data_ptr()) if t_map is None else (T, t_state.data_ptr(), tuple(int(v) for v in t_map))
        tb = ws.step_tables.get(key)
        if tb is None:
            tb = SimpleNamespace()
            steps_t = torch.arange(T, dtype=torch.int64, device=dev) if t_map is None else t_map.to(dev, torch.int64).contiguous()
            assert steps_t.numel() == T
            n = T * B2
            tb.times = steps_t.repeat_interleave(B2).contiguous()
            tb.lowres_times = torch.zeros(n, dtype=torch.int64, device=dev) if u.lowres_cond else None
            tb.text_hiddens = torch.empty(n, u.time_cond_dim, dtype=torch.float32, device=dev)
            tb.ss = torch.empty(n, max(pk.R, 1), dtype=torch.float32, device=dev)
            cp = L.MiCondStepParams.from_buffer_copy(ws.cond_params)
            cp.B2 = cp.B = n
            cp.time, cp.lowres_time = L.ptr(tb.times), L.ptr(tb.lowres_times)
            cp.text_hiddens, cp.ss, cp.c_time, cp.t_out = (L.ptr(tb.text_hiddens) if ws.has_text else 0), L.ptr(tb.ss), 0, 0
            tb.cond = cp
            tb.times_t = steps_t
            tb.lowres_t = torch.zeros(T, dtype=torch.int64, device=dev) if u.lowres_cond else None
            tb.c_time_t = torch.empty(T, ws.ntot, u.cond_dim, dtype=torch.float32, device=dev)
            ct = L.MiCondStepParams.from_buffer_copy(ws.cond_params)
            ct.B2 = ct.B = T
            ct.time, ct.lowres_time = L.ptr(tb.times_t), L.ptr(tb.lowres_t)
            ct.text_hiddens, ct.ss, ct.c_time, ct.t_out = 0, 0, L.ptr(tb.c_time_t), 0
            tb.cond_t = ct
            tb.fold, tb.tables = [], []
            stage_blocks = []
            for fn, fp, name in self._fold_params(ws, pk, tb.c_time_t, ws.ntot * u.cond_dim, 1, ws.ntot, 0):
                f1 = L.MiAttnFoldParams.from_buffer_copy(fp)
                f1.B2, f1.mode = T, 1
                for k in range(fp.n_blocks):
                    t = torch.empty(T, ws.ntot, fp.heads, fp.C, 2, dtype=torch.float32, device=dev)
                    tb.tables.append(t)
                    f1.blk[k].table = L.ptr(t)
                tb.fold.append(f1)
                f2 = L.MiAttnFoldParams.from_buffer_copy(f1)
                f2.B2, f2.mode, f2.t_state = B2, 3, L.ptr(t_state)
                stage_blocks.append(f2)
            if not stage_blocks:
                f2 = L.MiAttnFoldParams()
                f2.B2, f2.mode, f2.t_state, f2.n_blocks = B2, 3, L.ptr(t_state), 0
                stage_blocks.append(f2)
            stage_blocks[0].ss_all, stage_blocks[0].ss, stage_blocks[0].ss_n = L.ptr(tb.ss), L.ptr(ws.ss), ws.ss.shape[1]
            tb.stage = [(lib.mi_attn_fold_rows, f2, "stage_step") for f2 in stage_blocks]
            tb.keep = t_state
            ws.step_tables[key] = tb
        tb.text_hiddens.view(T, B2, -1).copy_(ws.text_hiddens.unsqueeze(0).expand(T, -1, -1))
        if u.lowres_cond:
            tb.lowres_times.view(T, B2)[:, :ws.B].copy_(ws.lowres_times.unsqueeze(0).expand(T, -1))
            if B2 != ws.B:
                tb.lowres_times.view(T, B2)[:, ws.B:].copy_(ws.lowres_times.unsqueeze(0).expand(T, -1))
            tb.lowres_t.copy_(ws.lowres_times[:1].expand(T))
        L.check(lib.mi_cond_step_fwd(C.byref(tb.cond), st), "mi_cond_step_fwd (all steps: scale/shift rows)")
        L.check(lib.mi_cond_step_fwd(C.byref(tb.cond_t), st), "mi_cond_step_fwd (all steps: time tokens)")
        for f1 in tb.fold:
            L.check(lib.mi_attn_fold_rows(C.byref(f1), st), "mi_attn_fold_rows (all steps)")
        ws.prog_stage = tb.stage

    def drop_step_tables(self, ws, t_state: torch.Tensor):
        for key in [k for k in ws.step_tables if k[1] == t_state.data_ptr()]:
            tb = ws.step_tables.pop(key)
            for k in [k for k in ws.prog_stage_off if k[0] == id(tb.stage)]:
                del ws.prog_stage_off[k]
            if ws.prog_stage is tb.stage:
                ws.prog_stage = ws.prog_cond

    def stage_prog(self, ws, t_off: int = 0):
        if t_off == 0:
            return ws.prog_stage
        assert ws.prog_stage is not ws.prog_cond, "the step-at-a-time conditioning cannot address a timestep offset"
        cache = ws.prog_stage_off
        key = (id(ws.prog_stage), t_off)
        if key not in cache:
            prog = []
            for fn, p, name in ws.prog_stage:
                q = L.MiAttnFoldParams.from_buffer_copy(p)
                q.t_off = t_off
                prog.append((fn, q, name))
            cache[key] = prog
        return cache[key]

    def step_offsets_supported(self, ws) -> bool:
        return ws.prog_stage is not ws.prog_cond

    def run_step(self, ws, stream=None, t_off: int = 0):
        st = L.current_stream() if stream is None else stream
        for fn, p, name in self.stage_prog(ws, t_off) + ws.prog:
            rc = fn(C.byref(p), st) if p is not None else fn(None, st)
            if rc != 0:
                L.check(rc, name)

    def run(self, ws, stream=None):
        st = L.current_stream() if stream is None else stream
        for fn, p, name in ws.prog_cond + ws.prog:
            rc = fn(C.byref(p), st) if p is not None else fn(None, st)
            if rc != 0:
                L.check(rc, name)

    def forward_once(self, x, time, *, lowres_cond_img, lowres_noise_times, text_embeds, text_mask, keep, cond_scale=None):
        u, lib = self.unet, L.lib()
        self.pack()
        L.require_device(x)
        B, Cc, H, W = x.shape
        assert Cc == u.channels
        two = cond_scale is not None
        ws = self.workspace(B, 2 * B if two else B, H, W, has_text=text_embeds is not None)
        ws.x.copy_(x)
        ws.times.copy_(time.to(torch.int64))
        if u.lowres_cond:
            ws.lowres.copy_(lowres_cond_img)
            ws.lowres_times.copy_(lowres_noise_times.to(torch.int64))
            self.prepare_lowres(ws)
        if two:
            keep = torch.cat((torch.ones(B, dtype=torch.bool), torch.zeros(B, dtype=torch.bool)))
        self.set_text(ws, text_embeds, text_mask, keep)
        self.run(ws)
        if not two:
            return ws.pred.clone()
        out = torch.empty(B, u.channels_out, H, W, dtype=torch.float32, device=ws.dev)
        p = L.MiCfgX0Params(B, u.channels_out * H * W, L.ptr(ws.pred), 1, float(cond_scale), 0, 0, 0, L.ptr(out), 0)
        L.check(lib.mi_cfg_x0_fwd(C.byref(p), L.current_stream()), "mi_cfg_x0_fwd")
        return out
```

### minimagen_amd/packing.py

```python
from __future__ import annotations

import math

import torch

LOG2E = 1.4426950408889634


def pack_conv_weight(w: torch.Tensor, cout_tile: int) -> torch.Tensor:
    cout = w.shape[0]
    pad = (cout + cout_tile - 1) // cout_tile * cout_tile
    out = torch.zeros(w.shape[1], w.shape[2], w.shape[3], pad, dtype=torch.float32, device=w.device)
    out[..., :cout] = w.detach().permute(1, 2, 3, 0)
    return out.contiguous()


def fold_parallel_1x1(w3: torch.Tensor, b3, w1: torch.Tensor, b1):
    w = w3.detach().clone()
    w[:, :, 1, 1] += w1.detach()[:, :, 0, 0]
    return w, (b3.detach() + b1.detach())


def fold_cross_attention(to_q, to_kv, to_out, null_kv, heads: int, dim_head: int = 64):
    dev = to_q.device
    H, D = heads, dim_head
    to_q, to_kv, to_out, null_kv = (t.detach().to('cpu') for t in (to_q, to_kv, to_out, null_kv))
    q = to_q.detach().double().reshape(H, D, -1)
    kv = to_kv.detach().double()
    k = kv[:H * D].reshape(H, D, -1)
    v = kv[H * D:].reshape(H, D, -1)
    o = to_out.detach().double().reshape(-1, H, D).permute(1, 0, 2)
    nk, nv = null_kv.detach().double().unbind(0)
    scale = D ** -0.5
    mg = torch.einsum('hda,hdb->hab', q, k) * (scale * LOG2E)
    mv = torch.einsum('had,hdb->hab', o, v)
    g0 = torch.einsum('hda,d->ha', q, nk) * (scale * LOG2E)
    v0 = torch.einsum('had,d->ha', o, nv)
    f = lambda t: t.float().contiguous().to(dev)
    return f(mg), f(mv), f(g0), f(v0)


def sinusoid_freq(dim: int, device) -> torch.Tensor:
    half = dim // 2
    k = math.log(10000) / (half - 1)
    return torch.exp(torch.arange(half) * -k).float().contiguous().to(device)


RP_PERM = (0, 2, 1, 3)


def rp_weight_exponent(mx: float) -> int:
    exp = 0 if (mx == 0.0 or not math.isfinite(mx)) else 7 - math.floor(math.log2(mx))
    return max(-100, min(100, exp))


def pack_conv_weight_rp(w: torch.Tensor, exp=None):
    cout, cin, kh, kw = w.shape
    assert (kh, kw) in ((3, 3), (1, 1), (4, 4))
    if exp is None:
        wd = w.detach().double().cpu()
        exp = rp_weight_exponent(float(wd.abs().max()))
    else:
        wd = w.detach().double()
    dev = wd.device
    ws = wd * (2.0 ** exp)
    if kh == 4:
        nj, ko = -(-cout // 16), -(-cin // 8)
        wp = torch.zeros(nj * 16, ko * 8, 4, 4, dtype=torch.float64, device=dev)
        wp[:cout, :cin] = ws
        lane = torch.arange(64, device=dev)
        lq, lg = lane & 15, lane >> 4
        co = 16 * torch.arange(nj, device=dev)[:, None] + lq[None, :]
        ci = 8 * torch.arange(ko, device=dev)[:, None] + torch.arange(8, device=dev)[None, :]
        out = wp[co[None, None, :, :, None], ci[:, None, None, None, :], lg[None, None, None, :, None], torch.arange(4, device=dev)[None, :, None, None, None]]
        hi = out.float().half()
        lo = (out - hi.double()).float().half()
        return torch.cat((hi, lo), dim=-1).contiguous().to(w.device), exp
    nj, ko, steps = -(-cout // 8), -(-cin // 8), kw
    wp = torch.zeros(nj * 8, ko * 8, 3, kw, dtype=torch.float64, device=dev)
    if kh == 3:
        wp[:cout, :cin] = ws
    else:
        wp[:cout, :cin, 1, :] = ws[:, :, 0, :]
    lane = torch.arange(64, device=dev)
    lq, lg = lane & 15, lane >> 4
    r = torch.tensor(RP_PERM, device=dev)[lg]
    ky = r - (lq >> 3)
    live = ((ky >= 0) & (ky <= 2)).double()
    kyc = ky.clamp(0, 2)
    co = (8 * torch.arange(nj, device=dev)[:, None] + (lq & 7)[None, :])
    ci = (8 * torch.arange(ko, device=dev)[:, None] + torch.arange(8, device=dev)[None, :])
    out = wp[co[None, None, :, :, None], ci[:, None, None, None, :], kyc[None, None, None, :, None], torch.arange(steps, device=dev)[None, :, None, None, None]]
    out = out * live[None, None, None, :, None]
    hi = out.float().half()
    lo = (out - hi.double()).float().half()
    return torch.cat((hi, lo), dim=-1).contiguous().to(w.device), exp


def pack_conv_weight_ig(w: torch.Tensor, exp=None):
    cout, cin, kh, kw = w.shape
    assert (kh, kw) in ((3, 3), (1, 1)) and cin % 32 == 0 and cout % 16 == 0
    wd = w.detach().double()
    if exp is None:
        exp = rp_weight_exponent(float(wd.abs().max()))
    ws = (wd * (2.0 ** exp)).reshape(cout // 16, 16, cin // 32, 4, 8, kh * kw)
    out = ws.permute(2, 5, 0, 3, 1, 4).reshape(cin // 32, kh * kw, cout // 16, 64, 8)
    hi = out.float().half()
    lo = (out - hi.double()).float().half()
    return torch.stack((hi, lo), dim=3).contiguous().to(w.device), exp


def attn_f16_exponents(mg, mv, g0, v0, cmax: float, xmax: float):
    def k(bound):
        bound = float(bound)
        if not math.isfinite(bound) or bound <= 0.0:
            return 0
        return max(-40, min(40, 12 - math.ceil(math.log2(bound))))
    gb = max(float(mg.abs().sum(-1).max()) * cmax, float(g0.abs().max()))
    vb = max(float(mv.abs().sum(-1).max()) * cmax, float(v0.abs().max()))
    return k(xmax), k(gb), k(vb)


def layernorm_bound(weight, bias, n: int) -> float:
    with torch.no_grad():
        if bias is not None:
            w, b = torch.stack((weight.detach().abs().max(), bias.detach().abs().max())).tolist()
        else:
            w, b = float(weight.detach().abs().max()), 0.0
    return w * math.sqrt(max(n - 1, 1)) + b


CE_TILES = ((0, 0), (0, 2), (1, 0), (2, 0))
CE_TABLE_ROWS = 32


def _crossembed_toeplitz(scaled, cin: int):
    tab = torch.zeros(CE_TABLE_ROWS, 2, 2, 2, 4, 8, dtype=torch.float64)
    w3, w7, w15 = scaled
    for lg in range(4):
        for dx in range(2):
            for h in range(2):
                kx = 2 * lg + dx + 8 * h
                if kx < 15:
                    tab[16:31, h, 0, :, lg, 4 * dx:4 * dx + cin] = w15[:, :, :, kx].permute(2, 0, 1)
                kx = 2 * lg + dx + 8 * h - 4
                if 0 <= kx < 7:
                    tab[8:15, h, 0, :, lg, 4 * dx:4 * dx + cin] = w7[:, :, :, kx].permute(2, 0, 1)
            kx = 2 * (lg & 1) + dx
            if kx < 3:
                for t in range(2):
                    for q in range(4):
                        ky = q - 1 + (lg >> 1)
                        if 0 <= ky < 3:
                            tab[4 * t + q, 0, 0, :, lg, 4 * dx:4 * dx + cin] = w3[2 * t:2 * t + 2, :, ky, kx]
    return tab


def pack_crossembed_mfma(ws, chan0: int, cin: int):
    assert cin <= 4 and len(ws) == 3 and [w.shape[-1] for w in ws] == [3, 7, 15] and [w.shape[0] for w in ws] == [4, 2, 2]
    exps, scaled = [], []
    for w in ws:
        wd = w.detach().double().cpu()[:, chan0:chan0 + cin]
        mx = float(wd.abs().max())
        e = 0 if (mx == 0.0 or not math.isfinite(mx)) else 7 - math.floor(math.log2(mx))
        e = max(-100, min(100, e))
        exps.append(e)
        scaled.append(wd * (2.0 ** e))
    tab = _crossembed_toeplitz(scaled, cin)
    hi = tab[:, :, 0].float().half()
    lo = (tab[:, :, 0] - hi.double()).float().half()
    out = torch.stack((hi, lo), dim=2)
    return out.reshape(CE_TABLE_ROWS, 256).contiguous().to(ws[0].device), exps


def crossembed_mfma_gather_index(shapes, chan0: int, cin: int):
    idx_w, off = [], 0
    for sh in shapes:
        n = 1
        for d in sh:
            n *= d
        idx_w.append((torch.arange(n, dtype=torch.float64) + (off + 1)).reshape(sh)[:, chan0:chan0 + cin])
        off += n
    tab = _crossembed_toeplitz(idx_w, cin)[:, :, 0]
    idx = tab.round().long() - 1
    idx[idx < 0] = off
    return idx.reshape(-1).contiguous()


def pack_crossembed_mfma_device(ws, idx: torch.Tensor, exps):
    flat = torch.cat([w.detach().reshape(-1) * (2.0 ** e) for w, e in zip(ws, exps)] + [ws[0].new_zeros(1)])
    t = flat[idx].reshape(CE_TABLE_ROWS, 2, 2, 4, 8)
    hi = t.half()
    lo = (t - hi.float()).half()
    return torch.stack((hi, lo), dim=2).reshape(CE_TABLE_ROWS, 256).contiguous()


ID_TAPS = 18
ID_ROWS = 3 * ID_TAPS + 1
ID_STEPS = 5


def compose_init_down(ce_ws, ce_bs, wd, bd, chan0: int, cin: int):
    ks = [w.shape[-1] for w in ce_ws]
    assert all(k % 2 == 1 and k <= 15 for k in ks) and tuple(wd.shape[2:]) == (4, 4)
    m_tot = sum(w.shape[0] for w in ce_ws)
    assert wd.shape[1] == m_tot
    wc = torch.zeros(m_tot, cin, 15, 15, dtype=torch.float64)
    m0 = 0
    for w, k in zip(ce_ws, ks):
        o = (15 - k) // 2
        wc[m0:m0 + w.shape[0], :, o:o + k, o:o + k] = w.detach().double().cpu()[:, chan0:chan0 + cin]
        m0 += w.shape[0]
    wdd = wd.detach().double().cpu()
    co = wdd.shape[0]
    with_bias = ce_bs is not None
    bc = torch.cat([b.detach().double().cpu() for b in ce_bs]) if with_bias else torch.zeros(m_tot, dtype=torch.float64)
    taps = ((1, 2, 3), (0, 1, 2, 3), (0, 1, 2))
    w9 = torch.zeros(3, 3, co, cin, ID_TAPS, ID_TAPS, dtype=torch.float64)
    b9 = torch.zeros(3, 3, co, dtype=torch.float64)
    for vy in range(3):
        for vx in range(3):
            for a in taps[vy]:
                for b in taps[vx]:
                    w9[vy, vx, :, :, a:a + 15, b:b + 15] += torch.einsum('om,mcyx->ocyx', wdd[:, :, a, b], wc)
                    b9[vy, vx] += wdd[:, :, a, b] @ bc
            if with_bias and bd is not None:
                b9[vy, vx] += bd.detach().double().cpu()
    return w9, b9


def pack_init_down_mfma(w9: torch.Tensor, b9: torch.Tensor):
    co, cin = w9.shape[2], w9.shape[3]
    assert co == 8 and cin <= 4 and tuple(w9.shape[4:]) == (ID_TAPS, ID_TAPS)
    wp = torch.zeros(3, 3, co, 4, ID_TAPS, 24, dtype=torch.float64)
    wp[:, :, :, :cin, :, :ID_TAPS] = w9
    exp = rp_weight_exponent(float(wp.abs().max()))
    wp = wp * (2.0 ** exp)
    tab = torch.zeros(ID_ROWS, ID_STEPS, co, 4, 2, 4, dtype=torch.float64)
    f = lambda t, n: t.reshape(3, co, 4, ID_TAPS, n, 4, 2).permute(0, 3, 4, 1, 5, 6, 2)
    main = tab[:3 * ID_TAPS].reshape(3, ID_TAPS, ID_STEPS, co, 4, 2, 4)
    main[:, :, 0:3] = f(wp[:, 1], 3)
    main[:, :, 3] = f((wp[:, 0] - wp[:, 1])[..., 8:16], 1)[:, :, 0]
    main[:, :, 4] = f((wp[:, 2] - wp[:, 1])[..., 2:10], 1)[:, :, 0]
    t = tab.reshape(ID_ROWS, ID_STEPS, co, 4, 8)
    hi = t.float().half()
    lo = (t - hi.double()).float().half()
    out = torch.stack((hi, lo), dim=2)
    return out.reshape(ID_ROWS, -1).contiguous(), exp, b9.float().contiguous()
```

Measured before the change: 50490 denoising-steps/s.

## Add cond-space cross-attention kernel sharing one context fragment across heads

Adds a cross-attention variant for narrow-channel blocks with 8 heads and small cond_dim. Instead of per-head folded key/value fragments built from the context each step, each token is projected into cond space through a per-head table. Attention then runs against one shared packed context fragment written by a new cond-rows kernel. This removes per-head fragment construction and storage and cuts the context data loaded per block. The cost is extra small MFMAs per head for the projection and new exponent-scaling logic that may hurt accuracy or fall back when bounds are large.

New measurement: 53040 denoising-steps/s, median of 6. 5.0% higher.

```diff
diff --git a/include/minimagen_hip.h b/include/minimagen_hip.h
--- a/include/minimagen_hip.h
+++ b/include/minimagen_hip.h
@@ -185,8 +185,24 @@
     int out_st;
     int x_exp, g_exp, v_exp;
     int variant;
+    const float* head_tab;
 } mi_cross_attn_params;
 int mi_cross_attn_fwd(const mi_cross_attn_params* p, void* stream);
+
+typedef struct mi_attn_cond_params {
+    int B2, cd, JT;
+    const float* c_rows;
+    int c_stride_b;
+    int row0, nrows;
+    int write_null;
+    int c_exp, i_exp;
+    float* frag;
+    const int* t_state; int t_off;
+    const float* ss_all; float* ss; int ss_n;
+} mi_attn_cond_params;
+int mi_attn_cond_rows(const mi_attn_cond_params* p, void* stream);
+int mi_attn_cond_frag_floats(int JT);
+int mi_attn_cond_head_floats(void);
 #define MI_ATTN_TOKENS_PER_WG 128
 
 typedef struct mi_cfg_x0_params {
diff --git a/minimagen_amd/_lib.py b/minimagen_amd/_lib.py
--- a/minimagen_amd/_lib.py
+++ b/minimagen_amd/_lib.py
@@ -96,6 +96,15 @@
         ("B2", C.c_int), ("C", C.c_int), ("HW", C.c_int), ("heads", C.c_int), ("J", C.c_int),
         ("x", MiAct), ("gv", C.c_void_p), ("n1_g", C.c_void_p), ("n1_b", C.c_void_p), ("n2_g", C.c_void_p), ("n2_b", C.c_void_p),
         ("out", C.c_void_p), ("out_stats", C.c_void_p), ("out_st", C.c_int), ("x_exp", C.c_int), ("g_exp", C.c_int), ("v_exp", C.c_int), ("variant", C.c_int),
+        ("head_tab", C.c_void_p),
+    ]
+
+
+class MiAttnCondParams(C.Structure):
+    _fields_ = [
+        ("B2", C.c_int), ("cd", C.c_int), ("JT", C.c_int), ("c_rows", C.c_void_p), ("c_stride_b", C.c_int), ("row0", C.c_int), ("nrows", C.c_int),
+        ("write_null", C.c_int), ("c_exp", C.c_int), ("i_exp", C.c_int), ("frag", C.c_void_p),
+        ("t_state", C.c_void_p), ("t_off", C.c_int), ("ss_all", C.c_void_p), ("ss", C.c_void_p), ("ss_n", C.c_int),
     ]
 
 
@@ -204,7 +213,7 @@
 _STRUCTS = {0: MiAct, 1: MiConvParams, 2: MiCrossEmbedParams, 3: MiLinear, 4: MiTextCondParams, 5: MiCondStepParams,
             6: MiAttnFoldParams, 7: MiCrossAttnParams, 8: MiCfgX0Params, 9: MiQuantileParams, 10: MiPosteriorParams,
             11: MiResizeParams, 12: MiSelfAttnParams, 13: MiChanFFParams, 14: MiFlashAttnParams, 15: MiTokensToNchwParams, 16: MiConvWgradParams, 17: MiBlockBwdParams, 18: MiCrossEmbedWgradParams, 19: MiFoldedAttnParams, 20: MiAdamTensor, 21: MiAdamParams, 22: MiPackConv3Desc,
-            23: MiFlashAttnTrainParams, 24: MiSamplerExtParams, 25: MiInpaintParams, 26: MiInitDownParams}
+            23: MiFlashAttnTrainParams, 24: MiSamplerExtParams, 25: MiInpaintParams, 26: MiInitDownParams, 27: MiAttnCondParams}
 
 _lib = None
 _backend = None
@@ -223,7 +232,7 @@
     for name in ("mi_conv_fwd", "mi_gn_coef_fwd", "mi_crossembed_fwd", "mi_text_cond_fwd", "mi_cond_step_fwd", "mi_attn_fold_rows", "mi_cross_attn_fwd",
                  "mi_cfg_x0_fwd", "mi_quantile_fwd", "mi_posterior_fwd", "mi_resize_fwd", "mi_self_attn_fwd", "mi_chan_ff_fwd",
                  "mi_flash_attn_fwd", "mi_conv_prep_fwd", "mi_tokens_to_nchw_fwd", "mi_conv_wgrad", "mi_block_bwd", "mi_crossembed_wgrad", "mi_folded_attn_fwd", "mi_folded_attn_bwd", "mi_adam_step",
-                 "mi_flash_attn_train_fwd", "mi_flash_attn_train_bwd", "mi_init_down_fwd"):
+                 "mi_flash_attn_train_fwd", "mi_flash_attn_train_bwd", "mi_init_down_fwd", "mi_attn_cond_rows"):
         getattr(lib, name).argtypes = [vp, vp]
         getattr(lib, name).restype = i32
     lib.mi_conv_prep_bytes.argtypes = [i32, i32, i32, i32, i32]
@@ -288,6 +297,8 @@
     lib.mi_pack_conv3.argtypes = [vp, i32, i32, i32, i32, vp, vp, i32, vp]
     lib.mi_pack_conv3_multi.argtypes = [vp, i32, i32, vp]
     lib.mi_attn_fragment_floats.argtypes = [i32]
+    lib.mi_attn_cond_frag_floats.argtypes = [i32]
+    lib.mi_attn_cond_head_floats.argtypes = []
     for which, st in _STRUCTS.items():
         n = lib.mi_struct_size(which)
         if n != C.sizeof(st):
diff --git a/minimagen_amd/csrc/attention.hip b/minimagen_amd/csrc/attention.hip
--- a/minimagen_amd/csrc/attention.hip
+++ b/minimagen_amd/csrc/attention.hip
@@ -254,7 +254,214 @@
     }
 }
 
-}
+#define MI_COND_HEAD_ROWS 5
+template <int C, int NWV>
+__global__ __launch_bounds__(64 * NWV, 4) void cross_attn_cond_f16x3_kernel(const mi_cross_attn_params p) {
+    static_assert(C <= 16, "one channel chunk");
+    constexpr int JT = 17, JP = (JT + 1) / 2, CROWS = JT + JP, HEADS = 8, HROWS = MI_COND_HEAD_ROWS * HEADS, TOK_WG = 16 * NWV;
+    __shared__ double red[NWV][2 * 16];
+    __shared__ __attribute__((aligned(16))) uint4 ctx[CROWS * 64];
+    __shared__ __attribute__((aligned(16))) uint4 htab[HROWS * 64];
+    const int tid = threadIdx.x, wave = tid >> 6, lane = tid & 63, lq = lane & 15, lg = lane >> 4;
+    const int tiles = (p.HW + TOK_WG - 1) / TOK_WG;
+    int b, tile;
+    if ((p.B2 & 7) == 0) {
+        const int L = blockIdx.x, k = L >> 3;
+        b = (L & 7) + 8 * (k / tiles);
+        tile = k % tiles;
+    } else {
+        b = blockIdx.x / tiles;
+        tile = blockIdx.x % tiles;
+    }
+    {
+        const uint4* csrc = reinterpret_cast<const uint4*>(p.gv) + (size_t)b * CROWS * 64;
+        const uint4* hsrc = reinterpret_cast<const uint4*>(p.head_tab);
+        for (int r = wave; r < CROWS + HROWS; r += NWV) {
+            const uint4* src = (r < CROWS ? csrc + (size_t)r * 64 : hsrc + (size_t)(r - CROWS) * 64) + lane;
+            uint4* dst = r < CROWS ? &ctx[r * 64] : &htab[(r - CROWS) * 64];
+#if defined(HIPEMU)
+            dst[lane] = *src;
+#else
+            __builtin_amdgcn_global_load_lds((const __attribute__((address_space(1))) void*)src, (__attribute__((address_space(3))) void*)dst, 16, 0, 0);
+#endif
+        }
+    }
+    const int bx = mi_row_of(b, p.x.bmod);
+    const int i = (tile * NWV + wave) * 16 + lq;
+    const bool ok = i < p.HW;
+    const float* xb = p.x.data + (size_t)bx * C * p.HW;
+    auto ldx = [&](int a) -> float { return xb[(size_t)a * p.HW + i]; };
+
+    f16x4 xhi, xlo;
+    {
+        float xf[4];
+        float s = 0.0f;
+#pragma unroll
+        for (int e = 0; e < 4; ++e) {
+            const int a = 4 * lg + e;
+            xf[e] = (ok && a < C) ? ldx(a) * p.x.scale : 0.0f;
+            s += xf[e];
+        }
+        s += __shfl_xor(s, 16); s += __shfl_xor(s, 32);
+        const float mean = s / (float)C;
+        float v = 0.0f;
+#pragma unroll
+        for (int e = 0; e < 4; ++e) { const float d = (4 * lg + e < C) ? xf[e] - mean : 0.0f; v = fmaf(d, d, v); }
+        v += __shfl_xor(v, 16); v += __shfl_xor(v, 32);
+        const float rstd = 1.0f / sqrtf(v / (float)C + 1e-5f);
+        float xn[4];
+#pragma unroll
+        for (int e = 0; e < 4; ++e) {
+            const int a = 4 * lg + e;
+            xn[e] = (a < C) ? ldexpf((xf[e] - mean) * rstd * p.n1_g[a] + p.n1_b[a], p.x_exp) : 0.0f;
+        }
+        split_f16(xn, xhi, xlo);
+    }
+    const f16x4 z4 = {(_Float16)0, (_Float16)0, (_Float16)0, (_Float16)0};
+    const f16x8 xhh = __builtin_shufflevector(xhi, xhi, 0, 1, 2, 3, 4, 5, 6, 7);
+    const f16x8 xl0 = __builtin_shufflevector(xlo, z4, 0, 1, 2, 3, 4, 5, 6, 7);
+    f32x4 oacc = (f32x4){0.f, 0.f, 0.f, 0.f};
+    float onull[4] = {0.f, 0.f, 0.f, 0.f};
+    const int jlast = p.J - 1;
+#if !defined(HIPEMU)
+    asm volatile("s_waitcnt vmcnt(0)" ::: "memory");
+#endif
+    __syncthreads();
+
+    for (int h = 0; h < HEADS; ++h) {
+        const uint4* ht = &htab[h * MI_COND_HEAD_ROWS * 64];
+        f16x8 yb;
+        {
+            f32x4 y[2];
+#pragma unroll
+            for (int T = 0; T < 2; ++T) {
+                const f16x8 f = __builtin_bit_cast(f16x8, ht[T * 64 + lane]);
+                f32x4 acc = (f32x4){0.f, 0.f, 0.f, 0.f};
+                acc = __builtin_amdgcn_mfma_f32_16x16x32_f16(f, xl0, acc, 0, 0, 0);
+                acc = __builtin_amdgcn_mfma_f32_16x16x32_f16(f, xhh, acc, 0, 0, 0);
+                y[T] = acc;
+            }
+            const float ys[8] = {y[0][0], y[0][1], y[0][2], y[0][3], y[1][0], y[1][1], y[1][2], y[1][3]};
+#pragma unroll
+            for (int e = 0; e < 3; ++e) {
+                const _Float16 hi = (_Float16)ys[e];
+                yb[e] = hi;
+                yb[e + 3] = (_Float16)(ys[e + 3] - (float)hi);
+            }
+            yb[6] = (_Float16)ys[6];
+            yb[7] = (_Float16)ys[7];
+        }
+        f32x4 s[JT];
+        uint4 gq[2];
+        gq[0] = ctx[lane];
+#pragma unroll
+        for (int jt = 0; jt < JT; ++jt) {
+            if (jt + 1 < JT) gq[(jt + 1) & 1] = ctx[(jt + 1) * 64 + lane];
+            __builtin_amdgcn_sched_barrier(0);
+            s[jt] = __builtin_amdgcn_mfma_f32_16x16x32_f16(__builtin_bit_cast(f16x8, gq[jt & 1]), yb, (f32x4){0.f, 0.f, 0.f, 0.f}, 0, 0, 0);
+        }
+        float m = -INFINITY;
+#pragma unroll
+        for (int jt = 0; jt < JT; ++jt)
+#pragma unroll
+            for (int r = 0; r < 4; ++r) {
+                if (jt == JT - 1 && (16 * jt + 4 * lg + r) > jlast) s[jt][r] = -INFINITY;
+                m = fmaxf(m, s[jt][r]);
+            }
+        m = fmaxf(m, __shfl_xor(m, 16));
+        m = fmaxf(m, __shfl_xor(m, 32));
+        const float sc = ldexpf(1.0f, -(p.x_exp + p.g_exp)), msc = -m * sc;
+        mi_f32x2 l2 = {0.0f, 0.0f};
+        const mi_f32x2 sc2 = {sc, sc}, msc2 = {msc, msc};
+        f32x4 u = (f32x4){0.f, 0.f, 0.f, 0.f};
+        float p0 = 0.0f;
+#pragma unroll
+        for (int jp = 0; jp < JP; ++jp) {
+            f16x4 ph[2], pl[2];
+#pragma unroll
+            for (int ts = 0; ts < 2; ++ts) {
+                const int jt = 2 * jp + ts;
+                float pe[4] = {0.f, 0.f, 0.f, 0.f};
+                if (jt < JT) {
+                    const f32x4 sv = s[jt < JT ? jt : 0];
+                    const mi_f32x2 a01 = mi_pk_fma((mi_f32x2){sv[0], sv[1]}, sc2, msc2), a23 = mi_pk_fma((mi_f32x2){sv[2], sv[3]}, sc2, msc2);
+                    pe[0] = __builtin_amdgcn_exp2f(a01[0]); pe[1] = __builtin_amdgcn_exp2f(a01[1]);
+                    pe[2] = __builtin_amdgcn_exp2f(a23[0]); pe[3] = __builtin_amdgcn_exp2f(a23[1]);
+                    l2 = mi_pk_add(l2, (mi_f32x2){pe[0], pe[1]});
+                    l2 = mi_pk_add(l2, (mi_f32x2){pe[2], pe[3]});
+                    if (jt == 0) p0 = pe[0];
+                }
+                split_f16(pe, ph[ts], pl[ts]);
+            }
+            const f16x8 phi = __builtin_shufflevector(ph[0], ph[1], 0, 1, 2, 3, 4, 5, 6, 7);
+            const f16x8 plo = __builtin_shufflevector(pl[0], pl[1], 0, 1, 2, 3, 4, 5, 6, 7);
+            const f16x8 cv = __builtin_bit_cast(f16x8, ctx[(JT + jp) * 64 + lane]);
+            u = __builtin_amdgcn_mfma_f32_16x16x32_f16(cv, plo, u, 0, 0, 0);
+            u = __builtin_amdgcn_mfma_f32_16x16x32_f16(cv, phi, u, 0, 0, 0);
+        }
+        float l = l2[0] + l2[1];
+        l += __shfl_xor(l, 16);
+        l += __shfl_xor(l, 32);
+        const float linv = 1.0f / l;
+        f16x4 uh, ul;
+        {
+            const float un[4] = {u[0] * linv, u[1] * linv, u[2] * linv, u[3] * linv};
+            split_f16(un, uh, ul);
+        }
+        const f16x8 ub = __builtin_shufflevector(uh, ul, 0, 1, 2, 3, 4, 5, 6, 7);
+        oacc = __builtin_amdgcn_mfma_f32_16x16x32_f16(__builtin_bit_cast(f16x8, ht[3 * 64 + lane]), ub, oacc, 0, 0, 0);
+        oacc = __builtin_amdgcn_mfma_f32_16x16x32_f16(__builtin_bit_cast(f16x8, ht[2 * 64 + lane]), ub, oacc, 0, 0, 0);
+        const float w0 = __shfl(p0, lq) * linv;
+        const float4 v0 = __builtin_bit_cast(float4, ht[4 * 64 + lane]);
+        onull[0] = fmaf(w0, v0.x, onull[0]); onull[1] = fmaf(w0, v0.y, onull[1]);
+        onull[2] = fmaf(w0, v0.z, onull[2]); onull[3] = fmaf(w0, v0.w, onull[3]);
+    }
+    float o[4];
+#pragma unroll
+    for (int r = 0; r < 4; ++r) o[r] = ldexpf(oacc[r], -p.v_exp) + onull[r];
+
+    float yv[4] = {0.f, 0.f, 0.f, 0.f};
+    {
+        float s1 = o[0] + o[1] + o[2] + o[3];
+        s1 += __shfl_xor(s1, 16); s1 += __shfl_xor(s1, 32);
+        const float mean = s1 / (float)C;
+        float v = 0.0f;
+#pragma unroll
+        for (int r = 0; r < 4; ++r) { const int a = 4 * lg + r; const float d = (a < C) ? o[r] - mean : 0.0f; v = fmaf(d, d, v); }
+        v += __shfl_xor(v, 16); v += __shfl_xor(v, 32);
+        const float rstd = 1.0f / sqrtf(v / (float)C + 1e-5f);
+#pragma unroll
+        for (int r = 0; r < 4; ++r) {
+            const int a = 4 * lg + r;
+            if (a < C && ok) {
+                const float y = (o[r] - mean) * rstd * p.n2_g[a] + p.n2_b[a] + ldx(a) * p.x.scale;
+                p.out[((size_t)b * C + a) * p.HW + i] = y;
+                yv[r] = y;
+            }
+        }
+    }
+    if (p.out_stats) {
+#pragma unroll
+        for (int r = 0; r < 4; ++r) {
+            const int a = 4 * lg + r;
+            double S, Q;
+            mi_stat_reduce16(yv[r], a < C && ok, lane, S, Q);
+            if (lq == 0) { red[wave][2 * a] = S; red[wave][2 * a + 1] = Q; }
+        }
+        __syncthreads();
+        const int nt64 = (p.HW + 63) / 64;
+        for (int sub = 0; sub < NWV / 4; ++sub) {
+            const int st = tile * (NWV / 4) + sub;
+            if (tid < 2 * C && st < nt64)
+                p.out_stats[((size_t)(b * C + (tid >> 1)) * nt64 + st) * 2 + (tid & 1)] =
+                    red[4 * sub][tid] + red[4 * sub + 1][tid] + red[4 * sub + 2][tid] + red[4 * sub + 3][tid];
+        }
+    }
+}
+
+}
+
+extern "C" int mi_attn_cond_head_floats(void) { return MI_COND_HEAD_ROWS * 64 * 4; }
 
 extern "C" int mi_cross_attn_fwd(const mi_cross_attn_params* pp, void* stream) {
     const mi_cross_attn_params& p = *pp;
@@ -284,6 +491,17 @@
         }
 #undef MI_ATTN16_LAUNCH
         return mi_check_launch("cross_attn_f16x3_kernel");
+    }
+    if (p.variant == 8) {
+        if (JT != 17 || p.heads != 8 || (p.C != 8 && p.C != 16) || !p.head_tab) { mi_set_error("mi_cross_attn_fwd: variant 8 is instantiated for C in {8,16}, 8 heads, a 17-tile context and needs head_tab (C %d, heads %d, J %d)", p.C, p.heads, p.J); return MI_ERR_UNSUPPORTED; }
+        static const int force_nwv = getenv("MI_ATTN_WAVES") ? atoi(getenv("MI_ATTN_WAVES")) : 0;
+        const int nwv = (force_nwv == 8 || force_nwv == 16) ? force_nwv : (p.HW <= 1024 ? 16 : 8);
+        const dim3 g8(((p.HW + 16 * nwv - 1) / (16 * nwv)) * p.B2);
+        if (p.C == 8 && nwv == 8) hipLaunchKernelGGL(HIP_KERNEL_NAME(cross_attn_cond_f16x3_kernel<8, 8>), g8, dim3(512), 0, st, p);
+        else if (p.C == 8) hipLaunchKernelGGL(HIP_KERNEL_NAME(cross_attn_cond_f16x3_kernel<8, 16>), g8, dim3(1024), 0, st, p);
+        else if (nwv == 8) hipLaunchKernelGGL(HIP_KERNEL_NAME(cross_attn_cond_f16x3_kernel<16, 8>), g8, dim3(512), 0, st, p);
+        else hipLaunchKernelGGL(HIP_KERNEL_NAME(cross_attn_cond_f16x3_kernel<16, 16>), g8, dim3(1024), 0, st, p);
+        return mi_check_launch("cross_attn_cond_f16x3_kernel");
     }
     mi_set_error("mi_cross_attn_fwd: variant %d (6 = 3-term fp16 split, fp32-grade; 7 = single fp16 term: the reduced-precision configuration)", p.variant);
     return MI_ERR_UNSUPPORTED;
diff --git a/minimagen_amd/csrc/capi.hip b/minimagen_amd/csrc/capi.hip
--- a/minimagen_amd/csrc/capi.hip
+++ b/minimagen_amd/csrc/capi.hip
@@ -52,6 +52,7 @@
         case 24: return (int)sizeof(mi_sampler_ext_params);
         case 25: return (int)sizeof(mi_inpaint_params);
         case 26: return (int)sizeof(mi_init_down_params);
+        case 27: return (int)sizeof(mi_attn_cond_params);
     }
     return -1;
 }
diff --git a/minimagen_amd/csrc/cond.hip b/minimagen_amd/csrc/cond.hip
--- a/minimagen_amd/csrc/cond.hip
+++ b/minimagen_amd/csrc/cond.hip
@@ -193,6 +193,54 @@
     }
 }
 
+__global__ __launch_bounds__(256) void attn_cond_rows_kernel(const mi_attn_cond_params p) {
+    const int bb = blockIdx.x;
+    const int step = p.t_state ? *p.t_state - p.t_off : 0;
+    if (blockIdx.y == 1) {
+        const float* src = p.ss_all + ((size_t)step * gridDim.x + bb) * p.ss_n;
+        for (int i = threadIdx.x; i < p.ss_n; i += 256) p.ss[(size_t)bb * p.ss_n + i] = src[i];
+        return;
+    }
+    const int JP = (p.JT + 1) / 2;
+    _Float16* fb = reinterpret_cast<_Float16*>(p.frag) + (size_t)bb * (p.JT + JP) * 64 * 8;
+    const float* rows = p.c_rows + (size_t)(p.t_state ? step : bb) * p.c_stride_b;
+    const int first = p.write_null ? -1 : 0;
+    const int total = (p.nrows - first) * 9;
+    for (int idx = threadIdx.x; idx < total; idx += 256) {
+        const int d = idx % 9, r = idx / 9 + first;
+        const int j = r < 0 ? 0 : p.row0 + r;
+        const int jt = j >> 4, jm = j & 15;
+        _Float16* ts = fb + (size_t)jt * 64 * 8;
+        if (d == 8) {
+            const _Float16 ind = (_Float16)(r < 0 ? ldexpf(1.0f, p.i_exp) : 0.0f);
+            _Float16* l8 = ts + (size_t)(jm + 32) * 8;
+            l8[2] = ind;
+            l8[5] = ind;
+            continue;
+        }
+        const float c = (r < 0 || d >= p.cd) ? 0.0f : ldexpf(rows[(size_t)r * p.cd + d], p.c_exp);
+        const _Float16 hi = (_Float16)c, lo = (_Float16)(c - (float)hi);
+        _Float16* lh = ts + (size_t)(jm + 16 * (d / 3)) * 8;
+        lh[d % 3] = hi;
+        lh[3 + d % 3] = hi;
+        ts[(size_t)(jm + 16 * (d >> 1)) * 8 + 6 + (d & 1)] = lo;
+        _Float16* tv = fb + (size_t)(p.JT + (jt >> 1)) * 64 * 8 + (size_t)(16 * (jm >> 2)) * 8 + 4 * (jt & 1) + (jm & 3);
+        tv[(size_t)d * 8] = hi;
+        tv[(size_t)(d + 8) * 8] = lo;
+    }
+}
+
+}
+
+extern "C" int mi_attn_cond_frag_floats(int JT) { return (JT + (JT + 1) / 2) * 64 * 4; }
+
+extern "C" int mi_attn_cond_rows(const mi_attn_cond_params* p, void* stream) {
+    if (p->B2 <= 0 || p->cd <= 0 || p->cd > 8 || p->JT <= 0 || !p->frag) { mi_set_error("mi_attn_cond_rows: cd %d (1 .. 8) / JT %d / empty batch", p->cd, p->JT); return MI_ERR_INVALID; }
+    if (p->row0 < 0 || p->nrows < 0 || p->row0 + p->nrows > p->JT * 16 || (p->nrows && (p->row0 < 1 || !p->c_rows))) { mi_set_error("mi_attn_cond_rows: rows beyond the padded context (row 0 is the null row)"); return MI_ERR_INVALID; }
+    if (p->i_exp < -14 || p->i_exp > 15) { mi_set_error("mi_attn_cond_rows: the indicator 2^%d is no normal fp16 number", p->i_exp); return MI_ERR_INVALID; }
+    if (p->ss_n > 0 && (!p->t_state || !p->ss_all || !p->ss)) { mi_set_error("mi_attn_cond_rows: the scale/shift copy needs t_state, ss_all and ss"); return MI_ERR_INVALID; }
+    hipLaunchKernelGGL(attn_cond_rows_kernel, dim3(p->B2, p->ss_n > 0 ? 2 : 1), dim3(256), 0, (hipStream_t)stream, *p);
+    return mi_check_launch("attn_cond_rows_kernel");
 }
 
 extern "C" int mi_attn_fragment_floats(int C) { return ((C / 4) < 4 ? 4 : (C / 4)) + 4 * ((C + 15) / 16); }
diff --git a/minimagen_amd/engine.py b/minimagen_amd/engine.py
--- a/minimagen_amd/engine.py
+++ b/minimagen_amd/engine.py
@@ -19,6 +19,7 @@
 COND_GEMM = int(os.environ.get("MINIMAGEN_COND_GEMM", "2048"))
 FLASH_KV_PREP = os.environ.get("MINIMAGEN_FLASH_KV_PREP", "1") != "0"
 CE_MFMA = os.environ.get("MINIMAGEN_CE_MFMA", "1") != "0"
+ATTN_COND = os.environ.get("MINIMAGEN_ATTN_COND", "1") != "0"
 INIT_DOWN = os.environ.get("MINIMAGEN_INIT_DOWN", "1") != "0"
 CONV_REVERSE = int(os.environ.get("MINIMAGEN_CONV_REVERSE", "1"))
 RP_NTILE = int(os.environ.get("MINIMAGEN_RP_NTILE", "0"))
@@ -169,6 +170,7 @@
         pk.conv_ig = {}
         pk.attn = {}
         pk.attn_exp = {}
+        pk.attn_cond = {}
 
         def conv_pack(mod: nn.Conv2d, w=None, b=None):
             w = mod.weight if w is None else w
@@ -221,6 +223,11 @@
                 pk.attn[id(ca)] = (mg, mv, g0, v0)
                 pk.attn_exp[id(ca)] = P.attn_f16_exponents(mg, mv, g0, v0, cmax=P.layernorm_bound(u.norm_cond.weight, u.norm_cond.bias, u.cond_dim),
                                                            xmax=P.layernorm_bound(ca.norm.gamma, ca.norm.beta, Cc))
+                if ATTN_COND and Cc in (8, 16) and u.cond_dim <= 8 and ca.heads == 8:
+                    ex = P.attn_cond_exponents(mg, mv, g0, v0, cmax=P.layernorm_bound(u.norm_cond.weight, u.norm_cond.bias, u.cond_dim),
+                                               xmax=P.layernorm_bound(ca.norm.gamma, ca.norm.beta, Cc))
+                    if ex is not None:
+                        pk.attn_cond[id(ca)] = (ex, P.pack_cross_attn_cond(mg, mv, g0, v0, ex["f_exp"], ex["g0_exp"], ex["mv_exp"]))
         for m in u.modules():
             if isinstance(m, Attention):
                 Cc = m.to_q.in_features
@@ -314,6 +321,7 @@
         ws.text_L = None
         for store16 in ((True, False) if ws.half else (False,)):
             ws.store16 = store16
+            ws.cfrag = None
             ws.gv, ws.tensors, ws.prog, ws.prog_text, ws.wide_attn = {}, [], [], [], False
             ws.ig_convs = []
             try:
@@ -581,10 +589,18 @@
         Cc, HW = h.C, h.H * h.W
         if Cc not in (8, 16, 32):
             return self._emit_cross_attn_wide(ws, ca, h)
-        FR = lib.mi_attn_fragment_floats(Cc)
-        jts = ws.JT + (ws.JT & 1)
-        gv = torch.zeros(ws.B2, ca.heads, jts, 64, FR, dtype=torch.float32, device=ws.dev)
-        ws.gv[id(ca)] = gv
+        cond = pk.attn_cond.get(id(ca)) if (not ws.half and ws.JT == 17) else None
+        if cond is not None:
+            if ws.cfrag is None:
+                ws.cfrag = torch.zeros(ws.B2, lib.mi_attn_cond_frag_floats(ws.JT), dtype=torch.float32, device=ws.dev)
+                ws.cfrag_exp = (cond[0]["c_exp"], cond[0]["i_exp"])
+            assert ws.cfrag_exp == (cond[0]["c_exp"], cond[0]["i_exp"])
+            gv = ws.cfrag
+        else:
+            FR = lib.mi_attn_fragment_floats(Cc)
+            jts = ws.JT + (ws.JT & 1)
+            gv = torch.zeros(ws.B2, ca.heads, jts, 64, FR, dtype=torch.float32, device=ws.dev)
+            ws.gv[id(ca)] = gv
         nt = -(-HW // 64)
         out = self._new_act(ws, ws.B2, Cc, h.H, h.W, nt)
         p = L.MiCrossAttnParams()
@@ -596,6 +612,10 @@
         p.out_st = out.st
         p.out, p.out_stats, p.variant = L.ptr(out.t), L.ptr(out.stats), (7 if ws.half else 6)
         p.x_exp, p.g_exp, p.v_exp = pk.attn_exp[id(ca)]
+        if cond is not None:
+            ex, tab = cond
+            p.variant, p.head_tab = 8, L.ptr(tab)
+            p.x_exp, p.g_exp, p.v_exp = ex["x_exp"], ex["f_exp"] + ex["c_exp"], ex["c_exp"] + ex["mv_exp"]
         ws.prog.append((lib.mi_cross_attn_fwd, p, "cross_attn"))
         return out
 
@@ -674,6 +694,13 @@
                     p.blk[k].mg, p.blk[k].mv, p.blk[k].g0, p.blk[k].v0 = L.ptr(mg), L.ptr(mv), L.ptr(g0), L.ptr(v0)
                     p.blk[k].gv = L.ptr(ws.gv[cid])
                 calls.append((lib.mi_attn_fold_rows, p, "fold"))
+        if ws.cfrag is not None:
+            p = L.MiAttnCondParams()
+            p.B2, p.cd, p.JT = ws.B2, self.unet.cond_dim, ws.JT
+            p.c_rows, p.c_stride_b, p.row0, p.nrows, p.write_null = L.ptr(rows_t), stride_b, row0, nrows, write_null
+            p.c_exp, p.i_exp = ws.cfrag_exp
+            p.frag = L.ptr(ws.cfrag)
+            calls.append((lib.mi_attn_cond_rows, p, "fold_cond"))
         return calls
 
     def _build_program(self, ws, pk):
@@ -802,7 +829,7 @@
         ws.pred = out.t
         if (out.H, out.W) != (H, W):
             raise L.MinImagenHipError(f"U-Net output is {out.H}x{out.W} for a {H}x{W} input (image size must be divisible by the down-sampling factor)")
-        if ws.gv:
+        if ws.gv or ws.cfrag is not None:
             ws.prog_cond += self._fold_params(ws, pk, ws.c_time, ws.ntot * u.cond_dim, 1, ws.ntot, 0)
 
     def set_text(self, ws, text_embeds: torch.Tensor, text_mask: Optional[torch.Tensor], keep: torch.Tensor):
@@ -879,6 +906,11 @@
             tb.fold, tb.tables = [], []
             stage_blocks = []
             for fn, fp, name in self._fold_params(ws, pk, tb.c_time_t, ws.ntot * u.cond_dim, 1, ws.ntot, 0):
+                if isinstance(fp, L.MiAttnCondParams):
+                    f2 = L.MiAttnCondParams.from_buffer_copy(fp)
+                    f2.t_state = L.ptr(t_state)
+                    stage_blocks.append(f2)
+                    continue
                 f1 = L.MiAttnFoldParams.from_buffer_copy(fp)
                 f1.B2, f1.mode = T, 1
                 for k in range(fp.n_blocks):
@@ -894,7 +926,7 @@
                 f2.B2, f2.mode, f2.t_state, f2.n_blocks = B2, 3, L.ptr(t_state), 0
                 stage_blocks.append(f2)
             stage_blocks[0].ss_all, stage_blocks[0].ss, stage_blocks[0].ss_n = L.ptr(tb.ss), L.ptr(ws.ss), ws.ss.shape[1]
-            tb.stage = [(lib.mi_attn_fold_rows, f2, "stage_step") for f2 in stage_blocks]
+            tb.stage = [(lib.mi_attn_cond_rows if isinstance(f2, L.MiAttnCondParams) else lib.mi_attn_fold_rows, f2, "stage_step") for f2 in stage_blocks]
             tb.keep = t_state
             ws.step_tables[key] = tb
         tb.text_hiddens.view(T, B2, -1).copy_(ws.text_hiddens.unsqueeze(0).expand(T, -1, -1))
@@ -926,7 +958,7 @@
         if key not in cache:
             prog = []
             for fn, p, name in ws.prog_stage:
-                q = L.MiAttnFoldParams.from_buffer_copy(p)
+                q = type(p).from_buffer_copy(p)
                 q.t_off = t_off
                 prog.append((fn, q, name))
             cache[key] = prog
diff --git a/minimagen_amd/packing.py b/minimagen_amd/packing.py
--- a/minimagen_amd/packing.py
+++ b/minimagen_amd/packing.py
@@ -121,6 +121,57 @@
     return k(xmax), k(gb), k(vb)
 
 
+def attn_cond_exponents(mg, mv, g0, v0, cmax: float, xmax: float):
+    def k(bound):
+        bound = float(bound)
+        if not math.isfinite(bound) or bound <= 0.0:
+            return 0
+        return max(-40, min(40, 12 - math.ceil(math.log2(bound))))
+    x_exp, c_exp = k(xmax), k(cmax)
+    i_exp = max(-14, min(12, c_exp))
+    shift = c_exp - i_exp
+    mgd, g0d = mg.detach().double(), g0.detach().double()
+    f_exp = min(k(float(mgd.abs().max())), k(float(mgd.abs().sum(1).max()) * xmax) - x_exp)
+    g0_exp = min(k(float(g0d.abs().max())), k(float(g0d.abs().sum(-1).max()) * xmax) - x_exp)
+    f_exp = min(f_exp, g0_exp - shift)
+    g0_exp = f_exp + shift
+    mv_exp = k(float(mv.detach().abs().max()))
+    if max(abs(e) for e in (x_exp, c_exp, f_exp, g0_exp, mv_exp)) > 60:
+        return None
+    return dict(x_exp=x_exp, c_exp=c_exp, i_exp=i_exp, f_exp=f_exp, g0_exp=g0_exp, mv_exp=mv_exp)
+
+
+def pack_cross_attn_cond(mg, mv, g0, v0, f_exp: int, g0_exp: int, mv_exp: int):
+    H, Cc, cd = mg.shape
+    assert Cc <= 16 and cd <= 8
+    dev = mg.device
+    F = torch.zeros(H, 12, 16, dtype=torch.float64)
+    F[:, :cd, :Cc] = mg.detach().double().cpu().transpose(1, 2) * 2.0 ** f_exp
+    F[:, 8, :Cc] = g0.detach().double().cpu() * 2.0 ** g0_exp
+    MV = torch.zeros(H, 16, 8, dtype=torch.float64)
+    MV[:, :Cc, :cd] = mv.detach().double().cpu() * 2.0 ** mv_exp
+    V0 = torch.zeros(H, 16, dtype=torch.float32)
+    V0[:, :Cc] = v0.detach().float().cpu()
+    lane = torch.arange(64)
+    lq, lg = lane & 15, lane >> 4
+    el = torch.arange(4)
+    a = 4 * lg[:, None] + el[None, :]
+    split = lambda t: (t.float().half(), (t - t.float().half().double()).float().half())
+    rows = []
+    for T in range(2):
+        e = 4 * T + (lq & 3)
+        lgp = lq >> 2
+        d = torch.where(e < 6, 3 * lgp + e % 3, 2 * lgp + e - 6)
+        hi, lo = split(F[:, d[:, None], a])
+        rows.append(torch.cat((hi, lo), -1))
+    hi, lo = split(MV[:, lq[:, None], a % 8])
+    rows.append(torch.cat((hi, hi), -1))
+    rows.append(torch.cat((lo, torch.zeros_like(lo)), -1))
+    rows.append(V0[:, a].contiguous().view(torch.float16))
+    tab = torch.stack(rows, 1).contiguous()
+    return tab.view(torch.float32).contiguous().to(dev)
+
+
 def layernorm_bound(weight, bias, n: int) -> float:
     with torch.no_grad():
         if bias is not None:
```
